# mratsim/laser

Hardware: NVIDIA H100
Metric: sgemm_tflops_m8192_n8192_k8192 (higher is better)
Workload: dtype f32

## Files before the change

### laser_b200/_build.py

```python
import concurrent.futures
import fcntl
import hashlib
import os
import shutil
import subprocess

_HERE = os.path.dirname(os.path.abspath(__file__))
CSRC = os.path.join(_HERE, "csrc")
LIB_DIR = os.path.join(_HERE, "lib")
OBJ_DIR = os.path.join(LIB_DIR, "obj")
LIB_PATH = os.path.join(LIB_DIR, "liblaser_b200.so")
SOURCES = ["capi.cu", "tc_f16x3.cu", "tc_tf32x3.cu", "tc_tf32x1.cu", "tc_bf16.cu"]
HEADERS = ["ptx.cuh", "f16_scale.cuh", "gemm_tc.cuh", "tc_params.h", "tc_launch.h", "tc_launch_impl.cuh", "gemm_simt.cuh", "gemm_dmma.cuh",
           "gemm_simt_kernel.inc", "split.cuh", "layers.cuh", "capi_layers.inc", "capi_multi.inc",
           "../../include/laser_b200.h"]

NVCC_FLAGS = [
    "-O3", "-std=c++17",
    "-gencode", "arch=compute_90a,code=sm_90a",
    "-lineinfo",
    "-Xcompiler", "-fPIC",
]
LINK_FLAGS = ["-shared", "-cudart", "static",
              "-gencode", "arch=compute_90a,code=sm_90a", "-Xcompiler", "-fPIC", "-ldl"]


def _nvcc():
    for cand in (shutil.which("nvcc"), "/usr/local/cuda/bin/nvcc"):
        if cand and os.path.exists(cand):
            return cand
    raise RuntimeError("nvcc not found: cannot build liblaser_b200.so")


def _sources():
    return [s for s in SOURCES if os.path.exists(os.path.join(CSRC, s))]


def _newest_header():
    return max((os.path.getmtime(os.path.join(CSRC, h)) for h in HEADERS if os.path.exists(os.path.join(CSRC, h))), default=0.0)


STAMP_PATH = LIB_PATH + ".srchash"


def _src_digest():
    h = hashlib.sha256(repr((NVCC_FLAGS, LINK_FLAGS)).encode())
    for name in _sources() + HEADERS:
        path = os.path.join(CSRC, name)
        if os.path.exists(path):
            h.update(name.encode() + b"\0")
            with open(path, "rb") as f:
                h.update(f.read())
    return h.hexdigest()


def _stamp():
    try:
        with open(STAMP_PATH) as f:
            return f.read().strip()
    except OSError:
        return None


def _write_stamp():
    tmp = "%s.tmp%d" % (STAMP_PATH, os.getpid())
    with open(tmp, "w") as f:
        f.write(_src_digest() + "\n")
    os.replace(tmp, STAMP_PATH)


def needs_build():
    if not os.path.exists(LIB_PATH):
        return True
    stamp = _stamp()
    if stamp is not None:
        return stamp != _src_digest()
    t = os.path.getmtime(LIB_PATH)
    return _newest_header() > t or any(os.path.getmtime(os.path.join(CSRC, s)) > t for s in _sources())


def build(force=False, verbose=False):
    if not force and not needs_build():
        if _stamp() is None:
            try:
                _write_stamp()
            except OSError:
                pass
        return LIB_PATH
    os.makedirs(OBJ_DIR, exist_ok=True)
    with open(os.path.join(LIB_DIR, ".build.lock"), "w") as lock:
        fcntl.flock(lock, fcntl.LOCK_EX)
        try:
            if not force and not needs_build():
                return LIB_PATH
            return _build_locked(force, verbose)
        finally:
            fcntl.flock(lock, fcntl.LOCK_UN)


def _build_locked(force, verbose):
    env = dict(os.environ)
    env.pop("CC", None)
    env.pop("CXX", None)
    nvcc = _nvcc()
    hdr_t = _newest_header()
    tag = ".tmp%d" % os.getpid()

    def compile_one(src):
        obj = os.path.join(OBJ_DIR, os.path.splitext(src)[0] + ".o")
        path = os.path.join(CSRC, src)
        if not force and os.path.exists(obj) and os.path.getmtime(obj) >= max(hdr_t, os.path.getmtime(path)):
            return obj
        cmd = [nvcc] + NVCC_FLAGS + (["-Xptxas", "-v"] if verbose else []) + ["-c", path, "-o", obj + tag]
        subprocess.check_call(cmd, env=env)
        os.replace(obj + tag, obj)
        return obj

    srcs = _sources()
    with concurrent.futures.ThreadPoolExecutor(max_workers=min(len(srcs), os.cpu_count() or 1)) as pool:
        objs = list(pool.map(compile_one, srcs))
    subprocess.check_call([nvcc] + LINK_FLAGS + ["-o", LIB_PATH + tag] + objs, env=env)
    os.replace(LIB_PATH + tag, LIB_PATH)
    _write_stamp()
    return LIB_PATH


if __name__ == "__main__":
    print(build(force=True, verbose=True))
```

### laser_b200/csrc/capi.cu

```cuda
#include "../../include/laser_b200.h"

#include <cuda.h>
#include <cuda_runtime.h>
#include <cudaTypedefs.h>

#include <atomic>
#include <cstdarg>
#include <cstdio>
#include <cstdlib>
#include <cstring>
#include <map>
#include <mutex>
#include <string>
#include <type_traits>
#include <utility>
#include <vector>

#include "gemm_simt.cuh"
#include "gemm_dmma.cuh"
#include "layers.cuh"
#include "split.cuh"
#include "tc_launch.h"

namespace {

using namespace lb200;

thread_local std::string g_last_error;
thread_local int g_last_path = 0;
std::atomic<int64_t> g_launches{0};
std::atomic<int64_t> g_dmma_launches{0};
std::atomic<int> g_f32_mode{-1};
constexpr int kDefaultF32Mode = LASER_B200_PATH_F16X3;
void multi_shutdown();

int set_error(int code, const char *fmt, ...) {
  char buf[512];
  va_list ap;
  va_start(ap, fmt);
  vsnprintf(buf, sizeof buf, fmt, ap);
  va_end(ap);
  g_last_error = buf;
  return code;
}

#define CUDA_TRY(expr)                                                                      \
  do {                                                                                      \
    cudaError_t _e = (expr);                                                                \
    if (_e != cudaSuccess) {                                                                \
      cudaGetLastError();                                                                   \
      return set_error(_e == cudaErrorMemoryAllocation ? LASER_B200_ENOMEM : LASER_B200_ECUDA, \
                       "%s failed: %s (%s:%d)", #expr, cudaGetErrorString(_e), __FILE__,   \
                       __LINE__);                                                           \
    }                                                                                       \
  } while (0)

struct Buffer {
  void *ptr = nullptr;
  size_t bytes = 0;
};

struct EventPair {
  cudaEvent_t a, b;
  int kind;
  int launches;
};

struct MapKey {
  const void *base;
  int64_t inner, outer, stride;
  int esz, box_inner, box_outer, swz;
  int64_t depth, depth_stride;
  bool operator==(const MapKey &o) const {
    return base == o.base && inner == o.inner && outer == o.outer && stride == o.stride && esz == o.esz &&
           box_inner == o.box_inner && box_outer == o.box_outer && swz == o.swz && depth == o.depth &&
           depth_stride == o.depth_stride;
  }
};
struct MapCacheEntry {
  MapKey key;
  CUtensorMap map;
  bool valid = false;
};
constexpr int kMapCacheSize = 64;

constexpr int kSchedSlots = 256;

struct Ctx {
  MapCacheEntry map_cache[kMapCacheSize];
  int map_cache_next = 0;
  int raster_g = 0;
  bool splitk_enabled = true;
  bool f64_dmma = true;
  bool ring_attr_set = false, dmma_attr_set = false;
  int64_t panel_rows = 1024;
  bool panel_taper = false;
  int kc_faithful = 128;
  bool dyn_sched = true;
  bool pdl = true;
  int64_t batch_ws_bytes = static_cast<int64_t>(1024) << 20;
  bool profiling = false;
  std::vector<EventPair> prof;
  int dev = -1;
  int sm_count = 0;
  cudaStream_t stream = nullptr;
  cudaStream_t up = nullptr, down = nullptr;
  std::vector<cudaEvent_t> panel_ev;
  PFN_cuTensorMapEncodeTiled_v12000 encode = nullptr;
  Buffer ws[4];
  Buffer gather[2];
  Buffer stage[3];
  Buffer splitk;
  Buffer bpanels;
  Buffer layer_ws;
  Buffer tfilt;
  Buffer f16s;
  Buffer sched;
  int sched_next = 0;
  cudaEvent_t ws_free = nullptr;
  std::mutex mu;
  std::mutex host_mu;
  std::mutex tfilt_mu;
  std::atomic<bool> ready{false};
};

constexpr int kMaxDevices = 32;
Ctx g_ctx[kMaxDevices];
std::mutex g_ctx_mu;

int parse_f32_mode(const char *mode) {
  if (!mode) return kDefaultF32Mode;
  if (!strcmp(mode, "f16x3")) return LASER_B200_PATH_F16X3;
  else if (!strcmp(mode, "tf32x3")) return LASER_B200_PATH_TF32X3;
  else if (!strcmp(mode, "tf32x1")) return LASER_B200_PATH_TF32X1;
  else if (!strcmp(mode, "simt")) return LASER_B200_PATH_SIMT;
  return kDefaultF32Mode;
}

int get_ctx(Ctx **out) {
  int dev = 0;
  cudaError_t e = cudaGetDevice(&dev);
  if (e != cudaSuccess) {
    cudaGetLastError();
    return set_error(LASER_B200_ENODEVICE, "no CUDA device: %s", cudaGetErrorString(e));
  }
  if (dev < 0 || dev >= kMaxDevices) return set_error(LASER_B200_ENODEVICE, "device index %d", dev);
  Ctx &c = g_ctx[dev];
  if (!c.ready) {
    std::lock_guard<std::mutex> lk(g_ctx_mu);
    if (!c.ready) {
      cudaDeviceProp prop;
      CUDA_TRY(cudaGetDeviceProperties(&prop, dev));
      if (prop.major != 9 || prop.minor != 0)
        return set_error(LASER_B200_ENODEVICE,
                         "device %d is sm_%d%d; this library is built for sm_90a only (no fallback)",
                         dev, prop.major, prop.minor);
      c.dev = dev;
      c.sm_count = prop.multiProcessorCount;
      CUDA_TRY(cudaStreamCreateWithFlags(&c.stream, cudaStreamNonBlocking));
      CUDA_TRY(cudaStreamCreateWithFlags(&c.up, cudaStreamNonBlocking));
      CUDA_TRY(cudaStreamCreateWithFlags(&c.down, cudaStreamNonBlocking));
      CUDA_TRY(cudaEventCreateWithFlags(&c.ws_free, cudaEventDisableTiming));
      void *fn = nullptr;
      cudaDriverEntryPointQueryResult qres;
      CUDA_TRY(cudaGetDriverEntryPoint("cuTensorMapEncodeTiled", &fn, cudaEnableDefault, &qres));
      if (!fn || qres != cudaDriverEntryPointSuccess)
        return set_error(LASER_B200_ECUDA, "cuTensorMapEncodeTiled not available from the driver");
      c.encode = reinterpret_cast<PFN_cuTensorMapEncodeTiled_v12000>(fn);
      CUDA_TRY(cudaMalloc(&c.sched.ptr, kSchedSlots * 2 * sizeof(unsigned int)));
      c.sched.bytes = kSchedSlots * 2 * sizeof(unsigned int);
      CUDA_TRY(cudaMemset(c.sched.ptr, 0, c.sched.bytes));
      if (const char *kc = getenv("LASER_B200_KC")) {
        const int v = atoi(kc);
        if (v >= 32) c.kc_faithful = v;
      }
      if (const char *rg = getenv("LASER_B200_RASTER")) c.raster_g = atoi(rg);
      if (const char *sk = getenv("LASER_B200_SPLITK")) c.splitk_enabled = atoi(sk) != 0;
      if (const char *dm = getenv("LASER_B200_F64_DMMA")) c.f64_dmma = atoi(dm) != 0;
      if (const char *pt = getenv("LASER_B200_PANEL_TAPER")) c.panel_taper = atoi(pt) != 0;
      if (const char *ds = getenv("LASER_B200_DYNSCHED")) c.dyn_sched = atoi(ds) != 0;
      if (const char *pd = getenv("LASER_B200_PDL")) c.pdl = atoi(pd) != 0;
      if (const char *bw = getenv("LASER_B200_BATCH_WS_MB")) {
        const int64_t v = atoll(bw);
        if (v >= 1) c.batch_ws_bytes = v << 20;
      }
      if (const char *pr = getenv("LASER_B200_PANEL_ROWS")) {
        const int64_t v = atoll(pr) / 256 * 256;
        if (v >= 256) c.panel_rows = v;
      }
      if (g_f32_mode.load() < 0) g_f32_mode.store(parse_f32_mode(getenv("LASER_B200_F32_MODE")));
      c.ready = true;
    }
  }
  *out = &c;
  return LASER_B200_OK;
}

int ensure(Buffer &b, size_t bytes) {
  if (b.bytes >= bytes) return LASER_B200_OK;
  if (b.ptr) CUDA_TRY(cudaFree(b.ptr));
  b.ptr = nullptr;
  b.bytes = 0;
  size_t want = bytes + (bytes >> 3);
  want = (want + 255) & ~static_cast<size_t>(255);
  CUDA_TRY(cudaMalloc(&b.ptr, want));
  b.bytes = want;
  return LASER_B200_OK;
}

struct ProfBracket {
  Ctx *c = nullptr;
  cudaStream_t s = nullptr;
  EventPair ep{};
  int64_t before = 0;

  int open(Ctx &ctx, cudaStream_t stream, int kind) {
    before = g_launches.load();
    if (!ctx.profiling) return LASER_B200_OK;
    c = &ctx;
    s = stream;
    ep.kind = kind;
    CUDA_TRY(cudaEventCreate(&ep.a));
    CUDA_TRY(cudaEventCreate(&ep.b));
    CUDA_TRY(cudaEventRecord(ep.a, s));
    return LASER_B200_OK;
  }
  int launches() const { return static_cast<int>(g_launches.load() - before); }
  int close() {
    if (!c) return LASER_B200_OK;
    ep.launches = launches();
    CUDA_TRY(cudaEventRecord(ep.b, s));
    c->prof.push_back(ep);
    c = nullptr;
    return LASER_B200_OK;
  }
  ~ProfBracket() {
    if (!c) return;
    if (ep.a) cudaEventDestroy(ep.a);
    if (ep.b) cudaEventDestroy(ep.b);
  }
};

inline int64_t round_up(int64_t x, int64_t m) { return (x + m - 1) / m * m; }
inline int grid_for(const Ctx &c, int64_t work_items, int per_sm) {
  int64_t g = static_cast<int64_t>(c.sm_count) * per_sm;
  if (work_items < g) g = work_items > 0 ? work_items : 1;
  return static_cast<int>(g);
}
#define COUNT_LAUNCH() g_launches.fetch_add(1, std::memory_order_relaxed)
#define CHECK_LAUNCH() CUDA_TRY(cudaGetLastError())

template <typename T, int TM, int TN, int BK>
int launch_simt(Ctx &c, int64_t M, int64_t N, int64_t K, T alpha, const T *A, int64_t rsA,
                int64_t csA, const T *B, int64_t rsB, int64_t csB, T beta, T *C, int64_t rsC,
                int64_t csC, cudaStream_t s, const Epilogue &epi, int64_t batch = 1, int64_t bsA = 0, int64_t bsB = 0,
                int64_t bsC = 0) {
  SimtParams<T> p;
  const int64_t tiles = simt_plan<T, TM, TN>(p, M, N, K, alpha, A, rsA, csA, B, rsB, csB, beta, C, rsC, csC);
  if constexpr (std::is_same<T, float>::value) { p.bias = epi.bias; p.bias_per_row = epi.bias_per_row; p.act = epi.act; }
  if (tiles > 0x7fffffff) return set_error(LASER_B200_EINVAL, "too many tiles");
  p.batch = batch; p.bsA = bsA; p.bsB = bsB; p.bsC = bsC;
  const int grid = grid_for(c, tiles * batch, 2);
  if (batch > 1) gemm_simt_batched_kernel<T, TM, TN, BK><<<grid, 256, 0, s>>>(p);
  else gemm_simt_kernel<T, TM, TN, BK><<<grid, 256, 0, s>>>(p);
  COUNT_LAUNCH();
  CHECK_LAUNCH();
  return LASER_B200_OK;
}

template <typename T>
int gemm_simt(Ctx &c, int64_t M, int64_t N, int64_t K, T alpha, const T *A, int64_t rsA,
              int64_t csA, const T *B, int64_t rsB, int64_t csB, T beta, T *C, int64_t rsC,
              int64_t csC, cudaStream_t s, const Epilogue &epi = Epilogue(), int64_t batch = 1, int64_t bsA = 0,
              int64_t bsB = 0, int64_t bsC = 0) {
#ifndef LB200_SIMT_BK
#define LB200_SIMT_BK 16
#endif
  if constexpr (std::is_same<T, double>::value) {
    const int64_t tiles128 = ((M + DMMA_BM - 1) / DMMA_BM) * ((N + DMMA_BN - 1) / DMMA_BN) * batch;
    if (c.f64_dmma && 2 * tiles128 >= c.sm_count) {
      SimtParams<double> p;
      const int64_t tiles = dmma_plan(p, M, N, K, alpha, A, rsA, csA, B, rsB, csB, beta, C, rsC, csC);
      if (tiles * batch > 0x7fffffff) return set_error(LASER_B200_EINVAL, "too many tiles");
      p.batch = batch; p.bsA = bsA; p.bsB = bsB; p.bsC = bsC;
      if (!c.dmma_attr_set) {
        CUDA_TRY(cudaFuncSetAttribute(gemm_dmma_kernel, cudaFuncAttributeMaxDynamicSharedMemorySize, static_cast<int>(DMMA_SMEM_BYTES)));
        c.dmma_attr_set = true;
      }
      gemm_dmma_kernel<<<grid_for(c, tiles * batch, 1), 256, DMMA_SMEM_BYTES, s>>>(p);
      g_dmma_launches.fetch_add(1);
      COUNT_LAUNCH();
      CHECK_LAUNCH();
      return LASER_B200_OK;
    }
  }
  if constexpr (std::is_same<T, float>::value) {
    if (M <= 32 && N >= 1024) {
      SimtParams<float> p;
      simt_plan<float, 8, 8>(p, M, N, K, alpha, A, rsA, csA, B, rsB, csB, beta, C, rsC, csC);
      p.bias = epi.bias; p.bias_per_row = epi.bias_per_row; p.act = epi.act;
      p.batch = batch; p.bsA = bsA; p.bsB = bsB; p.bsC = bsC;
      const bool async_ok = csB == 1 && rsB % 4 == 0 && (batch == 1 || bsB % 4 == 0) && (reinterpret_cast<uintptr_t>(B) & 15) == 0;
      if (async_ok) {
        const int grid = grid_for(c, ((N + 1023) / 1024) * batch, 1);
#define LB200_SKA(MT)                                                                                                  \
  do {                                                                                                                 \
    static std::atomic<uint32_t> attr_set{0};                                                                          \
    if (!(attr_set.load(std::memory_order_acquire) & (1u << c.dev))) {                                                 \
      CUDA_TRY(cudaFuncSetAttribute(gemm_skinny_m_async_kernel<MT>, cudaFuncAttributeMaxDynamicSharedMemorySize,       \
                                    static_cast<int>(ska_smem_bytes<MT>())));                                          \
      attr_set.fetch_or(1u << c.dev, std::memory_order_release);                                                       \
    }                                                                                                                  \
    gemm_skinny_m_async_kernel<MT><<<grid, 256, ska_smem_bytes<MT>(), s>>>(p);                                         \
  } while (0)
        if (M <= 8) LB200_SKA(8); else if (M <= 16) LB200_SKA(16); else if (M <= 24) LB200_SKA(24); else LB200_SKA(32);
#undef LB200_SKA
        COUNT_LAUNCH();
        CHECK_LAUNCH();
        return LASER_B200_OK;
      }
      const int nc = M <= 16 ? 4 : 2;
      const int grid = grid_for(c, ((N + 256 * nc - 1) / (256 * nc)) * batch, 2);
      if (M <= 8) gemm_skinny_m_kernel<8, 4><<<grid, 256, 0, s>>>(p);
      else if (M <= 16) gemm_skinny_m_kernel<16, 4><<<grid, 256, 0, s>>>(p);
      else if (M <= 24) gemm_skinny_m_kernel<24, 2><<<grid, 256, 0, s>>>(p);
      else gemm_skinny_m_kernel<32, 2><<<grid, 256, 0, s>>>(p);
      COUNT_LAUNCH();
      CHECK_LAUNCH();
      return LASER_B200_OK;
    }
  }
  if constexpr (sizeof(T) == 4)
    return launch_simt<T, 8, 8, LB200_SIMT_BK>(c, M, N, K, alpha, A, rsA, csA, B, rsB, csB, beta, C, rsC, csC, s, epi, batch,
                                               bsA, bsB, bsC);
  else
    return launch_simt<T, 4, 4, 16>(c, M, N, K, alpha, A, rsA, csA, B, rsB, csB, beta, C, rsC, csC, s, epi, batch, bsA, bsB,
                                    bsC);
}

struct Operand {
  const void *ptr;
  int64_t mn, k, s_mn, s_k;
  int64_t batch = 0, s_b = 0, aux_sb = 0;
  const ConvGeom *conv = nullptr;
  bool concat = false;
};
enum Major { K_MAJOR = 0, MN_MAJOR = 1, GENERAL = 2 };

Major classify(const Operand &o, int esz) {
  const bool aligned = (reinterpret_cast<uintptr_t>(o.ptr) & 15) == 0;
  if (!aligned) return GENERAL;
  const int64_t lim = (static_cast<int64_t>(1) << 40) / esz;
  if (o.s_k == 1 && o.s_mn > 0 && (o.s_mn * esz) % 16 == 0 && o.s_mn < lim) return K_MAJOR;
  if (o.s_mn == 1 && o.s_k > 0 && (o.s_k * esz) % 16 == 0 && o.s_k < lim) return MN_MAJOR;
  return GENERAL;
}

int encode_map(Ctx &c, CUtensorMap *map, int esz, const void *base, int64_t inner, int64_t outer,
               int64_t outer_stride_elems, int box_inner, int box_outer, CUtensorMapSwizzle swz, int64_t depth = 0,
               int64_t depth_stride = 0) {
  const MapKey key{base, inner, outer, outer_stride_elems, esz, box_inner, box_outer, static_cast<int>(swz), depth, depth_stride};
  for (int i = 0; i < kMapCacheSize; ++i)
    if (c.map_cache[i].valid && c.map_cache[i].key == key) {
      *map = c.map_cache[i].map;
      return LASER_B200_OK;
    }
  const cuuint64_t dims[3] = {static_cast<cuuint64_t>(inner), static_cast<cuuint64_t>(outer), static_cast<cuuint64_t>(depth)};
  const cuuint64_t strides[2] = {static_cast<cuuint64_t>(outer_stride_elems) * esz, static_cast<cuuint64_t>(depth_stride) * esz};
  const cuuint32_t box[3] = {static_cast<cuuint32_t>(box_inner), static_cast<cuuint32_t>(box_outer), 1};
  const cuuint32_t estr[3] = {1, 1, 1};
  const CUtensorMapDataType dt = esz == 4 ? CU_TENSOR_MAP_DATA_TYPE_FLOAT32 : CU_TENSOR_MAP_DATA_TYPE_BFLOAT16;
  CUresult r = c.encode(map, dt, depth > 0 ? 3 : 2, const_cast<void *>(base), dims, strides, box, estr,
                        CU_TENSOR_MAP_INTERLEAVE_NONE, swz,
                        CU_TENSOR_MAP_L2_PROMOTION_L2_256B, CU_TENSOR_MAP_FLOAT_OOB_FILL_NONE);
  if (r != CUDA_SUCCESS)
    return set_error(LASER_B200_ECUDA,
                     "cuTensorMapEncodeTiled failed (%d): base=%p inner=%lld outer=%lld stride=%lld box=%dx%d",
                     static_cast<int>(r), base, (long long)inner, (long long)outer,
                     (long long)outer_stride_elems, box_inner, box_outer);
  MapCacheEntry &e = c.map_cache[c.map_cache_next];
  c.map_cache_next = (c.map_cache_next + 1) % kMapCacheSize;
  e.key = key;
  e.map = *map;
  e.valid = true;
  return LASER_B200_OK;
}

int operand_map(Ctx &c, CUtensorMap *map, int esz, const void *base, Major major, int64_t mn,
                int64_t k, int64_t ld, int block_mn, int64_t depth = 0, int64_t depth_stride = 0) {
  const int block_k = TC_ROW_BYTES / esz;
  const int mn_atom = TC_ROW_BYTES / esz;
  if (major == K_MAJOR)
    return encode_map(c, map, esz, base, k, mn, ld, block_k, block_mn, CU_TENSOR_MAP_SWIZZLE_128B, depth, depth_stride);
  return encode_map(c, map, esz, base, mn, k, ld, mn_atom, block_k,
                    esz == 4 ? CU_TENSOR_MAP_SWIZZLE_128B_ATOM_32B : CU_TENSOR_MAP_SWIZZLE_128B, depth, depth_stride);
}

struct OperandMaps {
  CUtensorMap p0, p1;
  bool mn_major = false;
};
struct OperandWs {
  Buffer *p0, *p1, *gather;
  int64_t amax_off;
};
enum SplitMode {
  SPLIT_NONE = 0,
  SPLIT_TF32 = 1,
  SPLIT_F16X2 = 2,
};

inline OperandOp kernel_op(const OperandOp &op, bool rows_along_k) {
  OperandOp k = op;
  if (rows_along_k) { k.aux_sr = op.aux_sc; k.aux_sc = op.aux_sr; }
  return k;
}
inline bool op_same_layout(const Operand &o, const OperandOp &op) {
  return !op.aux || (op.aux_sr == o.s_mn && op.aux_sc == o.s_k && (reinterpret_cast<uintptr_t>(op.aux) & 15) == 0);
}

template <typename Launch>
int launch_prep(const OperandOp *op, const Batch &bt, Launch launch, bool concat = false) {
  auto with_op = [&](auto batched, auto cat) {
    if (op) launch(std::true_type(), *op, batched, cat);
    else launch(std::false_type(), OperandOp(), batched, cat);
  };
  if (concat) with_op(std::true_type(), std::true_type());
  else if (bt.n > 1) with_op(std::true_type(), std::false_type());
  else with_op(std::false_type(), std::false_type());
  COUNT_LAUNCH();
  CHECK_LAUNCH();
  return LASER_B200_OK;
}
inline Batch batch_of(const Operand &o) { return Batch{o.batch > 1 ? o.batch : 1, o.s_b, o.aux_sb}; }

template <typename T, int MODE = 0>
int gather(Ctx &c, const Operand &o, Buffer &dst, Buffer *lo, cudaStream_t s, const OperandOp *op = nullptr) {
  const Batch bt = batch_of(o);
  const int64_t ld = round_up(o.concat ? bt.n * o.k : o.k, 16 / static_cast<int64_t>(sizeof(T)));
  const size_t bytes = static_cast<size_t>((o.concat ? 1 : bt.n) * o.mn) * ld * sizeof(T);
  int rc;
  if ((rc = ensure(dst, bytes))) return rc;
  if (MODE == 1 && (rc = ensure(*lo, bytes))) return rc;
  const int64_t tiles = ((o.mn + 31) / 32) * ((o.k + 31) / 32) * bt.n;
  const int read_along_r = (llabs(o.s_mn) < llabs(o.s_k)) ? 1 : 0;
  T *d0 = static_cast<T *>(dst.ptr), *d1 = MODE == 1 ? static_cast<T *>(lo->ptr) : nullptr;
  return launch_prep(op, bt, [&](auto has_op, const OperandOp &k, auto batched, auto cat) {
    constexpr bool HAS_OP = decltype(has_op)::value && sizeof(T) == 4, BATCHED = decltype(batched)::value && sizeof(T) == 4,
                   CONCAT = decltype(cat)::value && sizeof(T) == 4;
    pack_general_kernel<T, MODE, HAS_OP, BATCHED, CONCAT><<<grid_for(c, tiles, 8), 256, 0, s>>>(
        static_cast<const T *>(o.ptr), o.mn, o.k, o.s_mn, o.s_k, d0, d1, ld, read_along_r, k, bt);
  }, o.concat);
}

int tf32_split(Ctx &c, const float *src, int64_t R, int64_t Cc, int64_t src_ld, float *hi, float *lo, int64_t ld, cudaStream_t s,
               const OperandOp *op, const Batch &bt = Batch(), bool concat = false) {
  const int64_t items = concat ? R * ((bt.n * Cc + 3) / 4) : bt.n * R * ((Cc + 3) / 4);
  return launch_prep(op, bt, [&](auto has_op, const OperandOp &k, auto batched, auto cat) {
    constexpr bool HAS_OP = decltype(has_op)::value, BATCHED = decltype(batched)::value, CONCAT = decltype(cat)::value;
    split_rows_tf32_kernel<HAS_OP, BATCHED, CONCAT><<<grid_for(c, (items + 255) / 256, 8), 256, 0, s>>>(src, R, Cc, src_ld, hi, lo,
                                                                                                       ld, k, bt);
  }, concat);
}

int f16x2_rows(Ctx &c, const float *src, int64_t R, int64_t Cc, int64_t src_ld, uint16_t *hb, uint16_t *lb, int64_t ld_b,
               uint32_t *words, cudaStream_t s, const OperandOp *op = nullptr, const Batch &bt = Batch(), bool concat = false) {
  const bool ring = !op && bt.n == 1 && f16x2_rows_ring_ok(src, Cc, src_ld);
  if (ring && !c.ring_attr_set) {
    CUDA_TRY(cudaFuncSetAttribute(f16x2_rows_ring_kernel, cudaFuncAttributeMaxDynamicSharedMemorySize,
                                  static_cast<int>(f16x2_rows_ring_smem(4 * 256 * F16ROWS_MAXV))));
    c.ring_attr_set = true;
  }
  const int64_t rows = concat ? R : bt.n * R, row_len = concat ? bt.n * Cc : Cc;
  return launch_prep(op, bt, [&](auto has_op, const OperandOp &k, auto batched, auto cat) {
    constexpr bool HAS_OP = decltype(has_op)::value, BATCHED = decltype(batched)::value, CONCAT = decltype(cat)::value;
    if (row_len <= 4 * 32 * F16ROWS_MAXV)
      f16x2_rows_fused_kernel<32, HAS_OP, BATCHED, CONCAT><<<grid_for(c, (rows + 7) / 8, 4), 256, 0, s>>>(src, R, Cc, src_ld, hb, lb,
                                                                                                     ld_b, words, k, bt);
    else if (ring)
      f16x2_rows_ring_kernel<<<grid_for(c, R, 2), 256, f16x2_rows_ring_smem(Cc), s>>>(src, R, Cc, src_ld, hb, lb, ld_b, words);
    else
      f16x2_rows_fused_kernel<256, HAS_OP, BATCHED, CONCAT><<<grid_for(c, rows, 4), 256, 0, s>>>(src, R, Cc, src_ld, hb, lb, ld_b,
                                                                                                words, k, bt);
  }, concat);
}

int f16x2_col_scales(Ctx &c, const float *src, int64_t R, int64_t Cc, int64_t src_ld, uint32_t *words, cudaStream_t s,
                     const OperandOp *op = nullptr, const Batch &bt = Batch(), bool concat = false) {
  CUDA_TRY(cudaMemsetAsync(words, 0, static_cast<size_t>((concat ? 1 : bt.n) * Cc) * sizeof(uint32_t), s));
  const int64_t items = ((Cc + 3) / 4) * ((R + ABSMAX_COL_ROWS - 1) / ABSMAX_COL_ROWS) * bt.n;
  return launch_prep(op, bt, [&](auto has_op, const OperandOp &k, auto batched, auto cat) {
    constexpr bool HAS_OP = decltype(has_op)::value, BATCHED = decltype(batched)::value, CONCAT = decltype(cat)::value;
    absmax_mn_kernel<true, HAS_OP, BATCHED, CONCAT><<<grid_for(c, (items + 255) / 256, 8), 256, 0, s>>>(src, R, Cc, src_ld, words, k,
                                                                                                       bt);
  }, concat);
}
int f16x2_col_split(Ctx &c, const float *src, int64_t R, int64_t Cc, int64_t src_ld, uint16_t *hb, uint16_t *lb, int64_t ld_b,
                    const uint32_t *words, cudaStream_t s, const OperandOp *op = nullptr, const Batch &bt = Batch(),
                    bool concat = false) {
  const int64_t items = ((Cc + 255) / 256) * ((R + SPLIT_ROWS - 1) / SPLIT_ROWS) * bt.n;
  return launch_prep(op, bt, [&](auto has_op, const OperandOp &k, auto batched, auto cat) {
    constexpr bool HAS_OP = decltype(has_op)::value, BATCHED = decltype(batched)::value, CONCAT = decltype(cat)::value;
    split_rows_f16x2_kernel<true, HAS_OP, BATCHED, CONCAT><<<grid_for(c, items, 8), 256, 0, s>>>(src, R, Cc, src_ld, hb, lb, ld_b,
                                                                                                words, k, bt);
  }, concat);
}

int im2col_rows(Ctx &c, const Operand &o, SplitMode mode, float *dst, float *dst_lo, uint16_t *hb, uint16_t *lb, int64_t ld,
                uint32_t *words, cudaStream_t s, const OperandOp *op = nullptr) {
  const Im2colSrc q = im2col_src(*o.conv);
  const Batch bt = batch_of(o);
  const int64_t images = o.conv->taps ? o.k / q.outHW : o.concat ? bt.n : bt.n * (o.mn / q.outHW), rows = bt.n * o.mn;
  const int64_t tiles = o.conv->taps ? ((o.mn + NHWC_TAPS - 1) / NHWC_TAPS) * ((ld + NHWC_PIX - 1) / NHWC_PIX)
                                     : o.mn * ((ld + TAP_SEG - 1) / TAP_SEG);
  const float *in = static_cast<const float *>(o.ptr);
  const bool dil = o.conv->dH != 1 || o.conv->dW != 1;
  if (o.concat && (dil || op)) return set_error(LASER_B200_ECUDA, "internal: a concatenated im2col source has no dilation or op");
  if (o.conv->nhwc && o.concat) return set_error(LASER_B200_ECUDA, "internal: a channels-last im2col source is not concatenated");
  if (o.conv->taps && (!o.conv->nhwc || dil || op))
    return set_error(LASER_B200_ECUDA, "internal: only a channels-last source without dilation or op has tap rows");
  auto launch = [&](auto m, auto absmax) {
    constexpr int MODE = decltype(m)::value, PER_SM = MODE == IM2COL_F16X2 ? 3 : 4;
    auto rows_kernel = [&](auto d, auto has_op, const auto &src) {
      constexpr bool DIL = decltype(d)::value, HAS_OP = decltype(has_op)::value;
      constexpr bool NHWC = std::is_base_of<Im2colNhwcSrc, typename std::decay<decltype(src)>::type>::value;
      if (ld <= 4 * 32 * F16ROWS_MAXV)
        im2col_rows_kernel<MODE, 32, DIL, HAS_OP, NHWC><<<grid_for(c, (rows + 7) / 8, PER_SM), 256, 0, s>>>(in, src, images, dst,
                                                                                                         dst_lo, hb, lb, ld, words);
      else
        im2col_rows_kernel<MODE, 256, DIL, HAS_OP, NHWC><<<grid_for(c, rows, PER_SM), 256, 0, s>>>(in, src, images, dst, dst_lo, hb,
                                                                                                lb, ld, words);
    };
    if (o.conv->taps) {
      im2col_nhwc_tap_rows_kernel<MODE, decltype(absmax)::value><<<grid_for(c, tiles, NHWC_PER_SM), 256, 0, s>>>(
          in, im2col_nhwc_src(*o.conv, in), images, dst, dst_lo, hb, lb, ld, words);
    } else if (o.conv->nhwc && (dil || op)) {
      Im2colNhwcGradSrc gq{};
      static_cast<Im2colNhwcSrc &>(gq) = im2col_nhwc_src(*o.conv, in);
      gq.vec = gq.vec && (!op || !op->aux || (reinterpret_cast<uintptr_t>(op->aux) & 15) == 0);
      gq.dH = static_cast<int>(o.conv->dH);
      gq.dW = static_cast<int>(o.conv->dW);
      if (op) gq.op = *op;
      if (dil && op) rows_kernel(std::true_type(), std::true_type(), gq);
      else if (dil) rows_kernel(std::true_type(), std::false_type(), gq);
      else rows_kernel(std::false_type(), std::true_type(), gq);
    } else if (o.conv->nhwc) {
      rows_kernel(std::false_type(), std::false_type(), im2col_nhwc_src(*o.conv, in));
    } else if (o.concat) {
      im2col_tap_rows_kernel<MODE, decltype(absmax)::value><<<grid_for(c, tiles, 8), 256, 0, s>>>(in, q, images, dst, dst_lo, hb, lb,
                                                                                                 ld, words);
    } else if (dil || op) {
      Im2colGradSrc gq{};
      static_cast<Im2colSrc &>(gq) = q;
      gq.dH = static_cast<int>(o.conv->dH);
      gq.dW = static_cast<int>(o.conv->dW);
      if (op) gq.op = *op;
      if (dil && op) rows_kernel(std::true_type(), std::true_type(), gq);
      else if (dil) rows_kernel(std::true_type(), std::false_type(), gq);
      else rows_kernel(std::false_type(), std::true_type(), gq);
    } else {
      rows_kernel(std::false_type(), std::false_type(), q);
    }
    COUNT_LAUNCH();
    CHECK_LAUNCH();
    return LASER_B200_OK;
  };
  if (mode == SPLIT_F16X2 && (o.concat || o.conv->taps)) {
    CUDA_TRY(cudaMemsetAsync(words, 0, static_cast<size_t>(o.mn) * sizeof(uint32_t), s));
    const int rc = launch(std::integral_constant<int, IM2COL_F16X2>(), std::true_type());
    if (rc) return rc;
  }
  if (mode == SPLIT_F16X2) return launch(std::integral_constant<int, IM2COL_F16X2>(), std::false_type());
  if (mode == SPLIT_TF32) return launch(std::integral_constant<int, IM2COL_TF32>(), std::false_type());
  return launch(std::integral_constant<int, IM2COL_F32>(), std::false_type());
}

int f32_rows(Ctx &c, const Operand &o, SplitMode mode, Buffer &dst, Buffer *lo, cudaStream_t s, const OperandOp *op) {
  if (!o.conv) return mode == SPLIT_TF32 ? gather<float, 1>(c, o, dst, lo, s, op) : gather<float>(c, o, dst, nullptr, s, op);
  const Batch bt = batch_of(o);
  const int64_t ld = round_up(o.concat ? bt.n * o.k : o.k, 4);
  const size_t bytes = static_cast<size_t>((o.concat ? 1 : bt.n) * o.mn) * ld * sizeof(float);
  int rc;
  if ((rc = ensure(dst, bytes))) return rc;
  if (mode == SPLIT_TF32 && (rc = ensure(*lo, bytes))) return rc;
  return im2col_rows(c, o, mode, static_cast<float *>(dst.ptr), mode == SPLIT_TF32 ? static_cast<float *>(lo->ptr) : nullptr,
                     nullptr, nullptr, ld, nullptr, s, op);
}

template <int ESZ>
int prepare_operand(Ctx &c, const Operand &o, SplitMode mode, const OperandWs &w, int block_mn,
                    OperandMaps *m, bool *used_ws, cudaStream_t s, const OperandOp *op = nullptr) {
  const bool conv = o.conv != nullptr;
  const Major mj = conv ? K_MAJOR : classify(o, ESZ);
  const Batch bt = batch_of(o);
  const bool cat = o.concat;
  const int64_t kk = cat ? bt.n * o.k : o.k;
  const bool rows_ok = bt.n == 1 || ((o.s_b * ESZ) % 16 == 0 && (!op || !op->aux || o.aux_sb % 4 == 0));
  const bool map_ok = bt.n == 1 || (o.s_b > 0 && o.s_b < (static_cast<int64_t>(1) << 40) / ESZ);
  const bool tma_layout = (mj == K_MAJOR || (mj == MN_MAJOR && (ESZ == 2 || mode == SPLIT_F16X2))) && rows_ok;
  const bool in_place = !conv && tma_layout && (mode == SPLIT_NONE ? !op && map_ok && !cat : !op || op_same_layout(o, *op));
  const Major out_mj = in_place ? mj : K_MAJOR;
  const int64_t R = (out_mj == K_MAJOR) ? o.mn : o.k;
  const int64_t Cc = (out_mj == K_MAJOR) ? o.k : o.mn;
  const int64_t src_ld = (mj == K_MAJOR) ? o.s_mn : o.s_k;
  const bool cat_rows = cat && out_mj == K_MAJOR;
  const int64_t rows_p = cat_rows ? R : bt.n * R, row_len = cat_rows ? bt.n * Cc : Cc;
  const int64_t ld = round_up(row_len, 16 / ESZ);
  const int64_t depth = o.batch > 0 && !cat ? bt.n : 0;
  auto d_stride = [&](int64_t pitch) { return bt.n > 1 ? (in_place && mode == SPLIT_NONE ? o.s_b : R * pitch) : R * pitch; };
  m->mn_major = (out_mj == MN_MAJOR);
  int rc;
  if (mode == SPLIT_NONE && in_place) {
    if ((rc = operand_map(c, &m->p0, ESZ, o.ptr, mj, o.mn, o.k, src_ld, block_mn, depth, d_stride(src_ld)))) return rc;
    m->p1 = m->p0;
    return LASER_B200_OK;
  }
  *used_ws = true;
  if constexpr (ESZ == 2) {
    if ((rc = gather<uint16_t>(c, o, *w.p0, nullptr, s))) return rc;
  } else {
    const float *src = static_cast<const float *>(o.ptr);
    const OperandOp kop = op ? kernel_op(*op, out_mj == MN_MAJOR) : OperandOp();
    const OperandOp *on_load = (in_place && op) ? &kop : nullptr;
    if (mode == SPLIT_F16X2) {
      const int64_t ld_b = round_up(row_len, 8);
      const size_t bytes_b = static_cast<size_t>(rows_p) * ld_b * 2;
      if ((rc = ensure(*w.p0, bytes_b))) return rc;
      if ((rc = ensure(*w.p1, bytes_b))) return rc;
      if (c.f16s.bytes < static_cast<size_t>(w.amax_off + (cat ? 1 : bt.n) * o.mn) * sizeof(uint32_t))
        return set_error(LASER_B200_ECUDA, "internal: F16X3 scale buffer not sized for this operand");
      uint16_t *hb = static_cast<uint16_t *>(w.p0->ptr), *lb = static_cast<uint16_t *>(w.p1->ptr);
      uint32_t *words = static_cast<uint32_t *>(c.f16s.ptr) + w.amax_off;
      if (conv) {
        rc = im2col_rows(c, o, mode, nullptr, nullptr, hb, lb, ld_b, words, s, op);
      } else if (!in_place) {
        if ((rc = gather<float>(c, o, *w.gather, nullptr, s, op))) return rc;
        rc = f16x2_rows(c, static_cast<const float *>(w.gather->ptr), rows_p, row_len, ld, hb, lb, ld_b, words, s);
      } else if (out_mj == K_MAJOR) {
        rc = f16x2_rows(c, src, R, Cc, src_ld, hb, lb, ld_b, words, s, on_load, bt, cat);
      } else {
        if ((rc = f16x2_col_scales(c, src, R, Cc, src_ld, words, s, on_load, bt, cat))) return rc;
        rc = f16x2_col_split(c, src, R, Cc, src_ld, hb, lb, ld_b, words, s, on_load, bt, cat);
      }
      if (rc) return rc;
      if ((rc = operand_map(c, &m->p0, 2, w.p0->ptr, out_mj, o.mn, kk, ld_b, block_mn, depth, d_stride(ld_b)))) return rc;
      return operand_map(c, &m->p1, 2, w.p1->ptr, out_mj, o.mn, kk, ld_b, block_mn, depth, d_stride(ld_b));
    }
    if (!in_place || conv) {
      rc = f32_rows(c, o, mode, *w.p0, w.p1, s, op);
    } else {
      const size_t bytes = static_cast<size_t>(rows_p) * ld * sizeof(float);
      if ((rc = ensure(*w.p0, bytes))) return rc;
      if ((rc = ensure(*w.p1, bytes))) return rc;
      rc = tf32_split(c, src, R, Cc, src_ld, static_cast<float *>(w.p0->ptr), static_cast<float *>(w.p1->ptr), ld, s, on_load, bt, cat);
    }
    if (rc) return rc;
  }
  if ((rc = operand_map(c, &m->p0, ESZ, w.p0->ptr, out_mj, o.mn, kk, ld, block_mn, depth, d_stride(ld)))) return rc;
  m->p1 = m->p0;
  if (mode == SPLIT_TF32) return operand_map(c, &m->p1, ESZ, w.p1->ptr, out_mj, o.mn, kk, ld, block_mn, depth, d_stride(ld));
  return LASER_B200_OK;
}

inline OperandWs ws_of_A(Ctx &c) { return OperandWs{&c.ws[0], &c.ws[1], &c.gather[0], 0}; }
inline OperandWs ws_of_B(Ctx &c, int64_t amax_off = 0) { return OperandWs{&c.ws[2], &c.ws[3], &c.gather[1], amax_off}; }
inline int f16_scales(Ctx &c, int64_t M, int64_t N, int64_t *b_off) {
  *b_off = round_up(M, 64);
  return ensure(c.f16s, static_cast<size_t>(*b_off + N) * sizeof(uint32_t));
}
struct F16Scales {
  const uint32_t *a = nullptr, *b = nullptr;
};

enum TcKind { TC_TF32X1, TC_TF32X3, TC_BF16, TC_F16X3 };
inline TcKind tc_kind_of_path(int path) {
  return path == LASER_B200_PATH_TF32X1 ? TC_TF32X1 : path == LASER_B200_PATH_TF32X3 ? TC_TF32X3 : TC_F16X3;
}
inline SplitMode split_mode(TcKind k) { return k == TC_TF32X3 ? SPLIT_TF32 : k == TC_F16X3 ? SPLIT_F16X2 : SPLIT_NONE; }

struct BatchArgs {
  int64_t batch, C, bias = 0;
};

template <typename OutT>
int tc_run(Ctx &c, TcKind kind, int64_t M, int64_t N, int64_t K, float alpha, const OperandMaps &ma,
           const OperandMaps &mb, float beta, OutT *C, int64_t rsC, int64_t csC, cudaStream_t s,
           const Epilogue &epi, const F16Scales *f16 = nullptr, bool after_prep = false, const BatchArgs *bat = nullptr,
           int64_t period_a = 1, int64_t period_b = 1) {
  TcLaunch l;
  l.a0 = ma.p0; l.a1 = ma.p1; l.b0 = mb.p0; l.b1 = mb.p1;
  l.a_mn = ma.mn_major; l.b_mn = mb.mn_major;
  l.pdl = c.pdl && after_prep;
  l.dev = c.dev; l.sm_count = c.sm_count; l.stream = s;
  TcParams &p = l.p;
  p.M = M; p.N = N; p.K = K; p.alpha = alpha; p.beta = beta;
  p.C = C; p.rsC = rsC; p.csC = csC; p.epi = epi;
  if (f16) { p.amax_a = f16->a; p.amax_b = f16->b; }
  if (bat) {
    l.batched = true;
    p.batch = static_cast<int>(bat->batch);
    p.period_a = static_cast<int>(period_a);
    p.period_b = static_cast<int>(period_b);
    p.bsC = bat->C;
    p.amax_bs_a = M;
    p.amax_bs_b = N;
    p.bias_bs = bat->bias;
  }
  const int npass = (kind == TC_TF32X3 || kind == TC_F16X3) ? 3 : 1;
  const TcPlanCfg cfg{c.kc_faithful, c.raster_g, c.splitk_enabled, c.sm_count};
  if (kind == TC_BF16 || kind == TC_F16X3) tc_plan<2, std::is_same<OutT, float>::value>(p, npass, cfg);
  else tc_plan<4, std::is_same<OutT, float>::value>(p, npass, cfg);
  if (c.dyn_sched) {
    p.sched = static_cast<unsigned int *>(c.sched.ptr) + 2 * c.sched_next;
    c.sched_next = (c.sched_next + 1) % kSchedSlots;
  }
  auto launch = [&](const TcLaunch &q) -> int {
    int e;
    switch (kind) {
      case TC_TF32X1: e = launch_tc_tf32x1(q); break;
      case TC_TF32X3: e = launch_tc_tf32x3(q); break;
      case TC_BF16: e = launch_tc_bf16(q); break;
      default: e = launch_tc_f16x3(q); break;
    }
    COUNT_LAUNCH();
    if (e != 0) {
      cudaGetLastError();
      return set_error(e == static_cast<int>(cudaErrorMemoryAllocation) ? LASER_B200_ENOMEM : LASER_B200_ECUDA,
                       "tensor-core kernel launch failed: %s", cudaGetErrorString(static_cast<cudaError_t>(e)));
    }
    CHECK_LAUNCH();
    return LASER_B200_OK;
  };
  ProfBracket prof;
  int rc = prof.open(c, s, 0);
  if (rc) return rc;
  if (p.k_splits > 1) {
    if constexpr (std::is_same<OutT, float>::value) {
      const int64_t ws_floats = tc_split_ws_floats(p);
      if ((rc = ensure(c.splitk, static_cast<size_t>(ws_floats) * sizeof(float)))) return rc;
      p.split_ws = static_cast<float *>(c.splitk.ptr);
      if ((rc = launch(l))) return rc;
      const int n_tail = p.num_m_blocks * p.num_n_blocks * p.batch - p.n_direct;
      const int64_t items = (static_cast<int64_t>(n_tail) * TC_BLOCK_M * (TC_BLOCK_N / 4) + 255) / 256;
      auto reduce = [&](auto batched) {
        splitk_tail_reduce_kernel<decltype(batched)::value><<<grid_for(c, items, 8), 256, 0, s>>>(
            static_cast<const float *>(c.splitk.ptr), p.k_splits, n_tail, p.n_direct, p.num_m_blocks, p.num_n_blocks, p.raster_g,
            M, N, alpha, beta, C, rsC, csC, p.epi.bias, p.epi.bias_per_row, p.epi.act, p.bsC, p.period_a, p.bias_bs);
      };
      if (bat) reduce(std::true_type());
      else reduce(std::false_type());
      COUNT_LAUNCH();
      CHECK_LAUNCH();
      CUDA_TRY(cudaEventRecord(c.ws_free, s));
      return prof.close();
    }
  }
  if ((rc = launch(l))) return rc;
  return prof.close();
}

inline bool batch_shares(int64_t stride, const OperandOp *op, int64_t aux_stride) {
  return stride == 0 && (!op || !op->aux || aux_stride == 0);
}

template <int SRC_ESZ, typename OutT>
int gemm_tc(Ctx &c, TcKind kind, const Operand &oa, const Operand &ob, float alpha, float beta, OutT *C, int64_t rsC, int64_t csC,
            cudaStream_t s, const Epilogue &epi, cudaEvent_t b_ready = nullptr, const OperandOp *opA = nullptr,
            const OperandOp *opB = nullptr, const BatchArgs *bat = nullptr) {
  const int64_t M = oa.mn, N = ob.mn, K = oa.k;
  const bool cat = oa.concat;
  const int64_t Kt = cat ? batch_of(oa).n * K : K;
  if (M > 0x7fffffffLL || N > 0x7fffffffLL || Kt > 0x7fffffffLL)
    return set_error(LASER_B200_EUNSUPPORTED, "tensor-core path: extents must fit in int32");
  std::lock_guard<std::mutex> lk(c.mu);
  const SplitMode mode = split_mode(kind);
  OperandMaps ma, mb;
  bool used_ws = false;
  CUDA_TRY(cudaStreamWaitEvent(s, c.ws_free, 0));
  ProfBracket prep;
  int rc = prep.open(c, s, 1);
  if (rc) return rc;
  int64_t f16_b_off = 0;
  if (mode == SPLIT_F16X2 &&
      (rc = f16_scales(c, (cat ? 1 : batch_of(oa).n) * M, (cat ? 1 : batch_of(ob).n) * N, &f16_b_off)))
    return rc;
  if ((rc = prepare_operand<SRC_ESZ>(c, oa, mode, ws_of_A(c), TC_BLOCK_M, &ma, &used_ws, s, opA))) return rc;
  if (b_ready) CUDA_TRY(cudaStreamWaitEvent(s, b_ready, 0));
  if ((rc = prepare_operand<SRC_ESZ>(c, ob, mode, ws_of_B(c, f16_b_off), TC_BLOCK_N, &mb, &used_ws, s, opB))) return rc;
  const int prep_launches = prep.launches();
  if ((rc = prep.close())) return rc;
  const F16Scales f16{static_cast<const uint32_t *>(c.f16s.ptr), static_cast<const uint32_t *>(c.f16s.ptr) + f16_b_off};
  rc = tc_run<OutT>(c, kind, M, N, Kt, alpha, ma, mb, beta, C, rsC, csC, s, epi, mode == SPLIT_F16X2 ? &f16 : nullptr,
                    prep_launches > 0 && !c.profiling, bat, batch_of(oa).n, batch_of(ob).n);
  if (rc) return rc;
  if (used_ws) CUDA_TRY(cudaEventRecord(c.ws_free, s));
  return LASER_B200_OK;
}

int finish(Ctx &c, cudaStream_t user, cudaStream_t s);

struct PackedLayout {
  int64_t ld_b;
  size_t off_h, off_l, off_amax, bytes;
};
inline PackedLayout packed_layout(int64_t mn, int64_t k) {
  PackedLayout L;
  L.ld_b = round_up(k, 8);
  auto al = [](size_t x) { return (x + 255) & ~static_cast<size_t>(255); };
  L.off_h = 0;
  L.off_l = al(static_cast<size_t>(mn) * L.ld_b * 2);
  L.off_amax = L.off_l + al(static_cast<size_t>(mn) * L.ld_b * 2);
  L.bytes = L.off_amax + al(static_cast<size_t>(mn) * sizeof(uint32_t));
  return L;
}

int prepack_dev(int which, void *dst, int64_t mn, int64_t k, const float *src, int64_t s_mn, int64_t s_k,
                void *stream) {
  if (mn < 0 || k < 0) return set_error(LASER_B200_EINVAL, "negative extent");
  if (mn == 0 || k == 0) return LASER_B200_OK;
  if (!dst || !src) return set_error(LASER_B200_EINVAL, "null pointer");
  if (reinterpret_cast<uintptr_t>(dst) & 255) return set_error(LASER_B200_EINVAL, "packed buffer must be 256-byte aligned");
  Ctx *c;
  int rc = get_ctx(&c);
  if (rc) return rc;
  cudaStream_t s = stream ? static_cast<cudaStream_t>(stream) : c->stream;
  const PackedLayout L = packed_layout(mn, k);
  uint8_t *base = static_cast<uint8_t *>(dst);
  uint16_t *h = reinterpret_cast<uint16_t *>(base + L.off_h), *l = reinterpret_cast<uint16_t *>(base + L.off_l);
  uint32_t *amax = reinterpret_cast<uint32_t *>(base + L.off_amax);
  {
    std::lock_guard<std::mutex> lk(c->mu);
    Operand o{src, mn, k, s_mn, s_k};
    const float *rows = src;
    int64_t rows_ld = s_mn;
    if (classify(o, 4) != K_MAJOR) {
      CUDA_TRY(cudaStreamWaitEvent(s, c->ws_free, 0));
      Buffer &g = c->gather[which];
      if ((rc = gather<float>(*c, o, g, nullptr, s))) return rc;
      rows = static_cast<const float *>(g.ptr);
      rows_ld = round_up(k, 4);
    }
    if ((rc = f16x2_rows(*c, rows, mn, k, rows_ld, h, l, L.ld_b, amax, s))) return rc;
    CUDA_TRY(cudaEventRecord(c->ws_free, s));
  }
  return finish(*c, static_cast<cudaStream_t>(stream), s);
}

int packed_maps(Ctx &c, const void *packed, int64_t mn, int64_t k, int block_mn, OperandMaps *m, const uint32_t **amax) {
  const PackedLayout L = packed_layout(mn, k);
  const uint8_t *base = static_cast<const uint8_t *>(packed);
  int rc;
  m->mn_major = false;
  *amax = reinterpret_cast<const uint32_t *>(base + L.off_amax);
  if ((rc = operand_map(c, &m->p0, 2, base + L.off_h, K_MAJOR, mn, k, L.ld_b, block_mn))) return rc;
  return operand_map(c, &m->p1, 2, base + L.off_l, K_MAJOR, mn, k, L.ld_b, block_mn);
}

int gemm_packed_dev(int64_t M, int64_t N, int64_t K, float alpha, const float *A, int64_t rsA,
                    int64_t csA, const void *packedA, const void *packedB, float beta, float *C,
                    int64_t rsC, int64_t csC, void *stream) {
  if (M < 0 || N < 0 || K < 0) return set_error(LASER_B200_EINVAL, "negative extent");
  if (M == 0 || N == 0 || K == 0) return LASER_B200_OK;
  if ((!A && !packedA) || !packedB || !C) return set_error(LASER_B200_EINVAL, "null pointer");
  if (M > 0x7fffffffLL || N > 0x7fffffffLL || K > 0x7fffffffLL)
    return set_error(LASER_B200_EUNSUPPORTED, "extents must fit in int32");
  Ctx *cp;
  int rc = get_ctx(&cp);
  if (rc) return rc;
  Ctx &c = *cp;
  cudaStream_t s = stream ? static_cast<cudaStream_t>(stream) : c.stream;
  {
    std::lock_guard<std::mutex> lk(c.mu);
    OperandMaps ma, mb;
    F16Scales f16;
    bool used_ws = false;
    int prep_launches = 0;
    CUDA_TRY(cudaStreamWaitEvent(s, c.ws_free, 0));
    if (packedA) {
      if ((rc = packed_maps(c, packedA, M, K, TC_BLOCK_M, &ma, &f16.a))) return rc;
    } else {
      Operand oa{A, M, K, rsA, csA};
      int64_t b_off = 0;
      if ((rc = f16_scales(c, M, 0, &b_off))) return rc;
      ProfBracket prep;
      if ((rc = prep.open(c, s, 1))) return rc;
      if ((rc = prepare_operand<4>(c, oa, SPLIT_F16X2, ws_of_A(c), TC_BLOCK_M, &ma, &used_ws, s))) return rc;
      prep_launches = prep.launches();
      if ((rc = prep.close())) return rc;
      f16.a = static_cast<const uint32_t *>(c.f16s.ptr);
    }
    if ((rc = packed_maps(c, packedB, N, K, TC_BLOCK_N, &mb, &f16.b))) return rc;
    if ((rc = tc_run<float>(c, TC_F16X3, M, N, K, alpha, ma, mb, beta, C, rsC, csC, s, Epilogue(), &f16,
                            prep_launches > 0 && !c.profiling)))
      return rc;
    if (used_ws) CUDA_TRY(cudaEventRecord(c.ws_free, s));
  }
  g_last_path = LASER_B200_PATH_F16X3;
  return finish(c, static_cast<cudaStream_t>(stream), s);
}

int check_args(int64_t M, int64_t N, int64_t K, const void *A, const void *B, const void *C) {
  if (M < 0 || N < 0 || K < 0) return set_error(LASER_B200_EINVAL, "negative extent M=%lld N=%lld K=%lld",
                                                (long long)M, (long long)N, (long long)K);
  if (M == 0 || N == 0 || K == 0) return -1;
  if (!A || !B || !C) return set_error(LASER_B200_EINVAL, "null matrix pointer");
  return LASER_B200_OK;
}

int finish(Ctx &, cudaStream_t user, cudaStream_t s) {
  if (!user) CUDA_TRY(cudaStreamSynchronize(s));
  return LASER_B200_OK;
}

inline bool is_tc_mode(int mode) {
  return mode == LASER_B200_PATH_F16X3 || mode == LASER_B200_PATH_TF32X3 || mode == LASER_B200_PATH_TF32X1;
}
int resolve_auto(int64_t M, int64_t N, int64_t K, const Epilogue &epi, bool operand_op = false) {
  const double work = static_cast<double>(M) * N * K;
  if (work <= 128.0 * 128.0 * 128.0) return LASER_B200_PATH_SIMT;
  const int mode = g_f32_mode.load();
  if (mode == LASER_B200_PATH_SIMT) return LASER_B200_PATH_SIMT;
  if (N <= 4 && M >= 1024 && !epi.bias && !epi.act && !operand_op) return -1;
  if (M <= 32 && N >= 1024) return LASER_B200_PATH_SIMT;
  return mode < 0 ? kDefaultF32Mode : mode;
}

int check_f32_path(int path) {
  if (path == LASER_B200_PATH_AUTO || path == LASER_B200_PATH_SIMT || is_tc_mode(path)) return LASER_B200_OK;
  return set_error(LASER_B200_EINVAL, "unknown path %d for float32", path);
}

int simt_run(Ctx &c, const Operand &oa, const Operand &ob, float alpha, float beta, float *C, int64_t rsC, int64_t csC,
             cudaStream_t s, const Epilogue &epi, const OperandOp *opA, const OperandOp *opB, int64_t batch, int64_t bsC) {
  struct Rows {
    const float *p;
    int64_t s_mn, s_k, s_b;
  };
  const bool copy_a = opA || oa.concat || oa.conv, copy_b = opB || ob.concat || ob.conv;
  std::unique_lock<std::mutex> lk(c.mu, std::defer_lock);
  if (copy_a || copy_b) {
    lk.lock();
    CUDA_TRY(cudaStreamWaitEvent(s, c.ws_free, 0));
  }
  auto rows = [&](const Operand &o, const OperandOp *op, bool copy, Buffer &g, Rows *r) {
    *r = Rows{static_cast<const float *>(o.ptr), o.s_mn, o.s_k, o.s_b};
    if (!copy) return LASER_B200_OK;
    const int rc = f32_rows(c, o, SPLIT_NONE, g, nullptr, s, op);
    const int64_t ld = round_up(o.concat ? batch_of(o).n * o.k : o.k, 4);
    *r = Rows{static_cast<const float *>(g.ptr), ld, 1, !o.concat && !batch_shares(o.s_b, op, o.aux_sb) ? o.mn * ld : 0};
    return rc;
  };
  Rows a, b;
  int rc;
  if ((rc = rows(oa, opA, copy_a, c.gather[0], &a))) return rc;
  if ((rc = rows(ob, opB, copy_b, c.gather[1], &b))) return rc;
  const int64_t K = oa.concat ? batch_of(oa).n * oa.k : oa.k;
  if ((rc = gemm_simt<float>(c, oa.mn, ob.mn, K, alpha, a.p, a.s_mn, a.s_k, b.p, b.s_k, b.s_mn, beta, C, rsC, csC, s, epi, batch,
                             a.s_b, b.s_b, bsC)))
    return rc;
  if (copy_a || copy_b) CUDA_TRY(cudaEventRecord(c.ws_free, s));
  return LASER_B200_OK;
}

int run_f32(Ctx &c, int path, int64_t M, int64_t N, int64_t K, float alpha, const float *A, int64_t rsA, int64_t csA, const float *B,
            int64_t rsB, int64_t csB, float beta, float *C, int64_t rsC, int64_t csC, cudaStream_t s, const Epilogue &epi,
            const OperandOp *opA, const OperandOp *opB, int64_t batch = 0, const laser_b200_batch_strides *bs = nullptr,
            bool concat = false, const ConvGeom *convB = nullptr, cudaEvent_t b_ready = nullptr, const ConvGeom *convA = nullptr,
            int64_t periodA = 0) {
  Operand oa{A, M, K, rsA, csA}, ob{B, N, K, csB, rsB};
  if (batch > 0) {
    oa.batch = periodA > 0 ? periodA : !concat && batch_shares(bs->A, opA, bs->auxA) ? 1 : batch; oa.s_b = bs->A; oa.aux_sb = bs->auxA; oa.concat = concat;
    ob.batch = !concat && batch_shares(bs->B, opB, bs->auxB) ? 1 : batch; ob.s_b = bs->B; ob.aux_sb = bs->auxB; ob.concat = concat;
  }
  oa.conv = convA;
  ob.conv = convB;
  const bool batched = batch > 0 && !concat;
  if (periodA > 0 && (!batched || opA || path == LASER_B200_PATH_SIMT))
    return set_error(LASER_B200_ECUDA, "internal: a periodic A is a batched tensor-core operand without op");
  if (path == LASER_B200_PATH_SIMT)
    return simt_run(c, oa, ob, alpha, beta, C, rsC, csC, s, epi, opA, opB, batched ? batch : 1, batched ? bs->C : 0);
  const BatchArgs bat{batch, batched ? bs->C : 0, periodA > 0 ? M : 0};
  return gemm_tc<4, float>(c, tc_kind_of_path(path), oa, ob, alpha, beta, C, rsC, csC, s, epi, b_ready, opA, opB,
                           batched ? &bat : nullptr);
}

int f32_dev(int64_t M, int64_t N, int64_t K, float alpha, const float *A, int64_t rsA, int64_t csA,
            const float *B, int64_t rsB, int64_t csB, float beta, float *C, int64_t rsC, int64_t csC,
            int path, void *stream, const Epilogue &epi = Epilogue(), cudaEvent_t b_ready = nullptr,
            const OperandOp *opA = nullptr, const OperandOp *opB = nullptr) {
  int rc = check_args(M, N, K, A, B, C);
  if (rc == -1) return LASER_B200_OK;
  if (rc) return rc;
  const bool has_op = opA || opB;
  if ((has_op || path != -1) && (rc = check_f32_path(path))) return rc;
  Ctx *c;
  rc = get_ctx(&c);
  if (rc) return rc;
  cudaStream_t s = stream ? static_cast<cudaStream_t>(stream) : c->stream;
  if (path == LASER_B200_PATH_AUTO) path = resolve_auto(M, N, K, epi, has_op);
  if (b_ready && !is_tc_mode(path)) CUDA_TRY(cudaStreamWaitEvent(s, b_ready, 0));
  switch (path) {
    case -1: {
      const int grid = grid_for(*c, (M + 7) / 8, 8);
      const bool vec = (csA == 1) && (rsA % 4 == 0) && (K % 4 == 0) && ((reinterpret_cast<uintptr_t>(A) & 15) == 0);
      const size_t bsmem = static_cast<size_t>(N) * K * sizeof(float);
      const bool use_smem = vec && bsmem <= 96 * 1024;
#define LB200_GEMV(NV)                                                                                         \
  do {                                                                                                         \
    if (use_smem) {                                                                                            \
      static std::atomic<uint32_t> attr_set{0};                                                                \
      if (!(attr_set.load(std::memory_order_acquire) & (1u << c->dev))) {                                      \
        CUDA_TRY(cudaFuncSetAttribute(gemv_warp_smem_kernel<NV>, cudaFuncAttributeMaxDynamicSharedMemorySize, 96 * 1024)); \
        attr_set.fetch_or(1u << c->dev, std::memory_order_release);                                            \
      }                                                                                                        \
      gemv_warp_smem_kernel<NV><<<grid_for(*c, (M + 7) / 8, 2), 256, bsmem, s>>>(M, K, alpha, A, rsA, B, rsB, csB, beta, C, rsC, csC); \
    } else if (vec) gemv_warp_kernel<NV, true><<<grid, 256, 0, s>>>(M, K, alpha, A, rsA, csA, B, rsB, csB, beta, C, rsC, csC);  \
    else gemv_warp_kernel<NV, false><<<grid, 256, 0, s>>>(M, K, alpha, A, rsA, csA, B, rsB, csB, beta, C, rsC, csC);     \
  } while (0)
      if (N == 1) LB200_GEMV(1); else if (N == 2) LB200_GEMV(2); else if (N == 3) LB200_GEMV(3); else LB200_GEMV(4);
#undef LB200_GEMV
      COUNT_LAUNCH();
      CHECK_LAUNCH();
      g_last_path = LASER_B200_PATH_SIMT;
      break;
    }
    default:
      rc = run_f32(*c, path, M, N, K, alpha, A, rsA, csA, B, rsB, csB, beta, C, rsC, csC, s, epi, opA, opB, 0, nullptr, false,
                   nullptr, b_ready);
      if (rc) return rc;
      g_last_path = path;
      break;
  }
  return finish(*c, static_cast<cudaStream_t>(stream), s);
}

template <typename T>
int simt_dev(int64_t M, int64_t N, int64_t K, T alpha, const T *A, int64_t rsA, int64_t csA,
             const T *B, int64_t rsB, int64_t csB, T beta, T *C, int64_t rsC, int64_t csC,
             void *stream) {
  int rc = check_args(M, N, K, A, B, C);
  if (rc == -1) return LASER_B200_OK;
  if (rc) return rc;
  Ctx *c;
  rc = get_ctx(&c);
  if (rc) return rc;
  cudaStream_t s = stream ? static_cast<cudaStream_t>(stream) : c->stream;
  rc = gemm_simt<T>(*c, M, N, K, alpha, A, rsA, csA, B, rsB, csB, beta, C, rsC, csC, s);
  if (rc) return rc;
  g_last_path = LASER_B200_PATH_SIMT;
  return finish(*c, static_cast<cudaStream_t>(stream), s);
}

int bf16_dev(int64_t M, int64_t N, int64_t K, float alpha, const uint16_t *A, int64_t rsA,
             int64_t csA, const uint16_t *B, int64_t rsB, int64_t csB, float beta, uint16_t *C,
             int64_t rsC, int64_t csC, void *stream) {
  int rc = check_args(M, N, K, A, B, C);
  if (rc == -1) return LASER_B200_OK;
  if (rc) return rc;
  Ctx *c;
  rc = get_ctx(&c);
  if (rc) return rc;
  cudaStream_t s = stream ? static_cast<cudaStream_t>(stream) : c->stream;
  rc = gemm_tc<2, uint16_t>(*c, TC_BF16, Operand{A, M, K, rsA, csA}, Operand{B, N, K, csB, rsB}, alpha, beta, C, rsC, csC, s,
                            Epilogue());
  if (rc) return rc;
  g_last_path = LASER_B200_PATH_BF16;
  return finish(*c, static_cast<cudaStream_t>(stream), s);
}

int epilogue_of(const laser_b200_epilogue *epi, Epilogue *e) {
  if (!epi) return LASER_B200_OK;
  if (epi->activation < 0 || epi->activation > 3) return set_error(LASER_B200_EINVAL, "unknown activation %d", epi->activation);
  e->bias = epi->bias;
  e->bias_per_row = epi->bias_per_row ? 1 : 0;
  e->act = epi->activation;
  return LASER_B200_OK;
}
int operand_op_of(const laser_b200_operand_op *in, bool is_b, OperandOp *op, const OperandOp **out) {
  *out = nullptr;
  if (!in || in->op == LASER_B200_OP_NONE) return LASER_B200_OK;
  if (in->op < LASER_B200_OP_NONE || in->op > LASER_B200_OP_SIGMOID_GRAD)
// ... 886 lines not shown
```

### laser_b200/csrc/f16_scale.cuh

```cuda
#pragma once

#include <stdint.h>
#ifdef LB200_HOST_EMULATION
#include <cmath>
#include <limits>
#endif

namespace lb200 {

__device__ __forceinline__ int f16x2_scale_exp(uint32_t absmax_bits) {
  const int e = static_cast<int>(absmax_bits >> 23);
  if (e == 0) return 0;
  int s = 14 - (e - 127);
  if (s > 126) s = 126;
  if (s < -126) s = -126;
  return s;
}
__device__ __forceinline__ float f16x2_pow2(int s) { return __uint_as_float(static_cast<uint32_t>(127 + s) << 23); }
__device__ __forceinline__ float f16x2_scale(uint32_t absmax_bits) { return f16x2_pow2(f16x2_scale_exp(absmax_bits)); }
__device__ __forceinline__ float f16x2_unscale(uint32_t absmax_bits) { return f16x2_pow2(-f16x2_scale_exp(absmax_bits)); }

#ifndef LB200_HOST_EMULATION
__device__ __forceinline__ uint16_t f16_rn_bits(float x) {
  uint16_t h;
  asm("cvt.rn.f16.f32 %0, %1;" : "=h"(h) : "f"(x));
  return h;
}
__device__ __forceinline__ float f16_bits_to_f32(uint16_t h) {
  float f;
  asm("cvt.f32.f16 %0, %1;" : "=f"(f) : "h"(h));
  return f;
}
#else
inline uint16_t f16_rn_bits(float x) {
  const uint32_t u = __float_as_uint(x);
  const uint16_t sign = static_cast<uint16_t>((u >> 16) & 0x8000u);
  const uint32_t a = u & 0x7fffffffu;
  if (a > 0x7f800000u) return static_cast<uint16_t>(sign | 0x7e00u);
  if (a == 0x7f800000u) return static_cast<uint16_t>(sign | 0x7c00u);
  const double ax = static_cast<double>(__uint_as_float(a));
  if (ax == 0.0) return sign;
  int e;
  std::frexp(ax, &e);
  int E = e - 1;
  if (E < -14) E = -14;
  const double q = std::ldexp(1.0, E - 10);
  const double r = std::nearbyint(ax / q) * q;
  if (r >= 65520.0) return static_cast<uint16_t>(sign | 0x7c00u);
  if (r < std::ldexp(1.0, -14)) return static_cast<uint16_t>(sign | static_cast<uint16_t>(r / std::ldexp(1.0, -24)));
  int e2;
  const double m = std::frexp(r, &e2);
  const uint32_t mant = static_cast<uint32_t>(m * 2048.0) - 1024u;
  return static_cast<uint16_t>(sign | (static_cast<uint32_t>(e2 - 1 + 15) << 10) | mant);
}
inline float f16_bits_to_f32(uint16_t h) {
  const int e = (h >> 10) & 31;
  const int m = h & 1023;
  double v;
  if (e == 0) v = std::ldexp(static_cast<double>(m), -24);
  else if (e == 31) v = m ? std::numeric_limits<double>::quiet_NaN() : std::numeric_limits<double>::infinity();
  else v = std::ldexp(static_cast<double>(1024 + m), e - 25);
  return static_cast<float>((h & 0x8000) ? -v : v);
}
#endif

__device__ __forceinline__ float f16_bits_to_f32_alu(uint32_t v) {
  const uint32_t u = v & 0x7fffu;
  const float normal = __uint_as_float((u << 13) + 0x38000000u);
  const float subnormal = __uint_as_float(0x38800000u + (u << 13)) - __uint_as_float(0x38800000u);
  const float mag = (u < 0x0400u) ? subnormal : normal;
  return (v & 0x8000u) ? -mag : mag;
}
__device__ __forceinline__ void f16x2_pieces2(float x0, float x1, uint32_t &h2, uint32_t &l2) {
#ifndef LB200_HOST_EMULATION
  asm("cvt.rn.f16x2.f32 %0, %1, %2;" : "=r"(h2) : "f"(x1), "f"(x0));
  const uint32_t v0 = h2 & 0xffffu, v1 = h2 >> 16;
  float d0 = __fsub_rn(x0, f16_bits_to_f32_alu(v0)), d1 = __fsub_rn(x1, f16_bits_to_f32_alu(v1));
  if ((v0 & 0x7c00u) == 0x7c00u) d0 = 0.0f;
  if ((v1 & 0x7c00u) == 0x7c00u) d1 = 0.0f;
  asm("cvt.rn.f16x2.f32 %0, %1, %2;" : "=r"(l2) : "f"(d1), "f"(d0));
#else
  const uint16_t a0 = f16_rn_bits(x0), a1 = f16_rn_bits(x1);
  const uint16_t b0 = ((a0 & 0x7c00u) == 0x7c00u) ? static_cast<uint16_t>(0) : f16_rn_bits(__fsub_rn(x0, f16_bits_to_f32_alu(a0)));
  const uint16_t b1 = ((a1 & 0x7c00u) == 0x7c00u) ? static_cast<uint16_t>(0) : f16_rn_bits(__fsub_rn(x1, f16_bits_to_f32_alu(a1)));
  h2 = a0 | (static_cast<uint32_t>(a1) << 16);
  l2 = b0 | (static_cast<uint32_t>(b1) << 16);
#endif
}

}
```

### laser_b200/csrc/gemm_tc.cuh

```cuda
#pragma once

#include <type_traits>

#include "f16_scale.cuh"
#include "ptx.cuh"
#include "tc_params.h"

namespace lb200 {

#ifndef LB200_HOST_EMULATION
static __device__ __noinline__ float epi_act(float v, int act) {
#else
inline float epi_act(float v, int act) {
#endif
  if (act == 1) return fmaxf(v, 0.0f);
  if (act == 2) return tanhf(v);
  if (act == 3) return 1.0f / (1.0f + expf(-v));
  return v;
}

__device__ __forceinline__ float bf16_bits_to_f32(uint16_t h) {
  return __uint_as_float(static_cast<uint32_t>(h) << 16);
}
__device__ __forceinline__ uint16_t f32_to_bf16_bits(float f) {
  uint32_t u = __float_as_uint(f);
  if ((u & 0x7fffffffu) > 0x7f800000u) return static_cast<uint16_t>((u >> 16) | 0x40);
  u += 0x7fffu + ((u >> 16) & 1u);
  return static_cast<uint16_t>(u >> 16);
}

template <int ESZ, uint32_t FMT16, int NPASS, bool A_MN, bool B_MN, typename OutT, bool SCALED, bool BATCHED>
__global__ void __launch_bounds__(TC_THREADS, 1)
gemm_tc_kernel(const __grid_constant__ CUtensorMap mapA0, const __grid_constant__ CUtensorMap mapA1,
               const __grid_constant__ CUtensorMap mapB0, const __grid_constant__ CUtensorMap mapB1,
               const TcParams p) {
  static_assert(NPASS == 1 || NPASS == 3, "one pass, or the three passes of a two-piece product");
  static_assert(ESZ == 2 || (!A_MN && !B_MN), "wgmma reads tf32 operands K-major only (capi.cu transposes MN-major fp32)");
  using Cfg = TcCfg<NPASS>;
  constexpr int STAGES = Cfg::STAGES;
  constexpr int BLOCK_K = TC_ROW_BYTES / ESZ;
  const int sched_id = static_cast<int>(blockIdx.x);
  const int sched_stride = static_cast<int>(gridDim.x);

  LB200_DYN_SMEM(uint8_t, smem_raw);
  uint8_t *smem = reinterpret_cast<uint8_t *>((reinterpret_cast<uintptr_t>(smem_raw) + 1023) &
                                              ~static_cast<uintptr_t>(1023));
  uint64_t *bars = reinterpret_cast<uint64_t *>(smem + STAGES * Cfg::STAGE_BYTES);
  uint64_t *full_bar = bars;
  uint64_t *empty_bar = bars + STAGES;
  uint64_t *sched_full = bars + 2 * STAGES;
  uint64_t *sched_empty = sched_full + 1;
  int *sched_unit = reinterpret_cast<int *>(sched_empty + 1);

  const int warp_idx = threadIdx.x >> 5;
  const int lane = threadIdx.x & 31;
  const int tiles_pp = p.num_m_blocks * p.num_n_blocks;
  const int num_tiles = BATCHED ? tiles_pp * p.batch : tiles_pp;
  const int num_kb = static_cast<int>((p.K + BLOCK_K - 1) / BLOCK_K);
  const int num_units = p.n_direct + (num_tiles - p.n_direct) * p.k_splits;
  auto decode_unit = [&](int u, int &t, int &sp, int &kb_lo, int &kb_hi) {
    if (u < p.n_direct) {
      t = u; sp = -1; kb_lo = 0; kb_hi = num_kb;
    } else {
      const int v = u - p.n_direct;
      const int i = v / p.k_splits;
      t = p.n_direct + i;
      sp = v - i * p.k_splits;
      kb_lo = min(num_kb, sp * p.kb_per_split);
      kb_hi = min(num_kb, kb_lo + p.kb_per_split);
    }
  };
  constexpr int SCHED_CONSUMERS = 1 + TC_EPI_WARPS;
  auto next_unit = [&](uint32_t &ph) -> int {
    ptx::mbar_wait(sched_full, ph);
    const int u = *reinterpret_cast<volatile int *>(sched_unit);
    ptx::mbar_arrive(sched_empty);
    ph ^= 1u;
    return u;
  };

  if (threadIdx.x == 0) {
    ptx::prefetch_tensormap(&mapA0);
    ptx::prefetch_tensormap(&mapB0);
    if constexpr (NPASS == 3) {
      ptx::prefetch_tensormap(&mapA1);
      ptx::prefetch_tensormap(&mapB1);
    }
  }
  if (threadIdx.x == 32) {
    for (int i = 0; i < STAGES; ++i) {
      ptx::mbar_init(&full_bar[i], 1);
      ptx::mbar_init(&empty_bar[i], TC_EPI_WARPS);
    }
    ptx::mbar_init(sched_full, 1);
    ptx::mbar_init(sched_empty, SCHED_CONSUMERS);
    ptx::fence_barrier_init();
  }
  __syncthreads();
  ptx::griddep_wait();

  if (warp_idx < 4) {
    ptx::setmaxnreg_dec<TC_REGS_CTRL>();
    if (warp_idx == 3 && lane == 0) {
      uint32_t phase = 0;
      int next_static = sched_id;
      for (;;) {
        ptx::mbar_wait(sched_empty, phase ^ 1);
        int u;
        if (p.sched) {
          u = static_cast<int>(atomicAdd(p.sched, 1u));
        } else {
          u = next_static;
          next_static += sched_stride;
        }
        if (u >= num_units) u = -1;
        *reinterpret_cast<volatile int *>(sched_unit) = u;
        ptx::mbar_arrive(sched_full);
        phase ^= 1u;
        if (u < 0) {
          if (p.sched) {
            __threadfence();
            if (atomicAdd(p.sched + 1, 1u) == static_cast<unsigned int>(sched_stride - 1)) {
              p.sched[0] = 0u;
              p.sched[1] = 0u;
              __threadfence();
            }
          }
          break;
        }
      }
    } else if (warp_idx == 0 && lane == 0) {
      int stage = 0;
      uint32_t phase = 0, sched_phase = 0;
      constexpr int MN_ATOM = TC_ROW_BYTES / ESZ;
      constexpr int MN_BOX_BYTES = BLOCK_K * TC_ROW_BYTES;
      auto load_a = [&](uint8_t *dst, const CUtensorMap *m, uint64_t *bar, int m0, int k0, int z) {
        if constexpr (!A_MN) {
          if constexpr (BATCHED) ptx::tma_load_3d(dst, m, bar, k0, m0, z);
          else ptx::tma_load_2d(dst, m, bar, k0, m0);
        } else {
#pragma unroll
          for (int c = 0; c < TC_BLOCK_M / MN_ATOM; ++c) {
            if constexpr (BATCHED) ptx::tma_load_3d(dst + c * MN_BOX_BYTES, m, bar, m0 + c * MN_ATOM, k0, z);
            else ptx::tma_load_2d(dst + c * MN_BOX_BYTES, m, bar, m0 + c * MN_ATOM, k0);
          }
        }
      };
      auto load_b = [&](uint8_t *dst, const CUtensorMap *m, uint64_t *bar, int n0, int k0, int z) {
        if constexpr (!B_MN) {
          if constexpr (BATCHED) ptx::tma_load_3d(dst, m, bar, k0, n0, z);
          else ptx::tma_load_2d(dst, m, bar, k0, n0);
        } else {
#pragma unroll
          for (int c = 0; c < TC_BLOCK_N / MN_ATOM; ++c) {
            if constexpr (BATCHED) ptx::tma_load_3d(dst + c * MN_BOX_BYTES, m, bar, n0 + c * MN_ATOM, k0, z);
            else ptx::tma_load_2d(dst + c * MN_BOX_BYTES, m, bar, n0 + c * MN_ATOM, k0);
          }
        }
      };
      for (;;) {
        const int u = next_unit(sched_phase);
        if (u < 0) break;
        int t, sp, mb, nb, kb_lo, kb_hi;
        decode_unit(u, t, sp, kb_lo, kb_hi);
        int za = 0, zb = 0;
        if constexpr (BATCHED) {
          const int bz = t / tiles_pp;
          t -= bz * tiles_pp;
          za = bz % p.period_a;
          zb = bz % p.period_b;
        }
        tile_coords(t, p.num_m_blocks, p.num_n_blocks, p.raster_g, mb, nb);
        const int m0 = mb * TC_BLOCK_M;
        const int n0 = nb * TC_BLOCK_N;
        for (int kb = kb_lo; kb < kb_hi; ++kb) {
          ptx::mbar_wait(&empty_bar[stage], phase ^ 1);
          ptx::mbar_arrive_expect_tx(&full_bar[stage], Cfg::STAGE_BYTES);
          uint8_t *sa = smem + stage * Cfg::STAGE_BYTES;
          uint8_t *sb = sa + Cfg::A_STAGE_BYTES;
          const int k0 = kb * BLOCK_K;
          load_a(sa, &mapA0, &full_bar[stage], m0, k0, za);
          if constexpr (NPASS == 3) load_a(sa + TC_A_TILE_BYTES, &mapA1, &full_bar[stage], m0, k0, za);
          load_b(sb, &mapB0, &full_bar[stage], n0, k0, zb);
          if constexpr (NPASS == 3) load_b(sb + Cfg::B_TILE_BYTES, &mapB1, &full_bar[stage], n0, k0, zb);
          if (++stage == STAGES) { stage = 0; phase ^= 1; }
        }
      }
    }
  } else {
    ptx::setmaxnreg_inc<TC_REGS_EPI>();
    const int g = (warp_idx - 4) >> 2;
    const int wq = warp_idx & 3;
    const int lr = lane >> 2;
    const int lc = 2 * (lane & 3);
    constexpr int MMA_K = 32 / ESZ;
    constexpr int K_STEPS = BLOCK_K / MMA_K;
    constexpr int MN_BOX_BYTES = BLOCK_K * TC_ROW_BYTES;
    constexpr uint32_t A_WG_BYTES = 64 * TC_ROW_BYTES;
    int stage = 0;
    uint32_t phase = 0, sched_phase = 0;
    const bool vec_ok_c = (p.csC == 1) && ((p.rsC & 1) == 0) && ((reinterpret_cast<uintptr_t>(p.C) & (2 * sizeof(OutT) - 1)) == 0) &&
                          (!BATCHED || (p.bsC & 1) == 0);
    float acc[TC_ACC_REGS];
#pragma unroll
    for (int j = 0; j < TC_ACC_REGS; ++j) acc[j] = 0.0f;
    for (;;) {
      int u = 0;
      if (lane == 0) u = next_unit(sched_phase);
      u = __shfl_sync(0xffffffffu, u, 0);
      if (u < 0) break;
      int t, sp, mb, nb, kb_lo, kb_hi;
      decode_unit(u, t, sp, kb_lo, kb_hi);
      int bz = 0, za = 0, zb = 0;
      if constexpr (BATCHED) {
        bz = t / tiles_pp;
        za = bz % p.period_a;
        zb = bz % p.period_b;
        int tl = t - bz * tiles_pp;
        tile_coords(tl, p.num_m_blocks, p.num_n_blocks, p.raster_g, mb, nb);
      } else {
        tile_coords(t, p.num_m_blocks, p.num_n_blocks, p.raster_g, mb, nb);
      }
      const int num_blocks = (kb_hi - kb_lo + p.kb_per_block - 1) / p.kb_per_block;
      const int r_tile = 64 * g + 16 * wq + lr;
      const int64_t row0 = static_cast<int64_t>(mb) * TC_BLOCK_M + r_tile;
      const int64_t col0 = static_cast<int64_t>(nb) * TC_BLOCK_N + lc;
      const bool split_unit = sp >= 0;
      uint32_t amax_row[2] = {0u, 0u}, amax_col[2 * TC_BLOCK_N / 8];
      if constexpr (SCALED) {
#pragma unroll
        for (int h = 0; h < 2; ++h)
          if (row0 + 8 * h < p.M) amax_row[h] = p.amax_a[(BATCHED ? za * p.amax_bs_a : 0) + row0 + 8 * h];
#pragma unroll
        for (int j = 0; j < 2 * TC_BLOCK_N / 8; ++j) {
          const int64_t c = col0 + 8 * (j >> 1) + (j & 1);
          amax_col[j] = c < p.N ? p.amax_b[(BATCHED ? zb * p.amax_bs_b : 0) + c] : 0u;
        }
      }
      float run[TC_ACC_REGS];
#pragma unroll
      for (int j = 0; j < TC_ACC_REGS; ++j) run[j] = 0.0f;
      for (int blk = 0; blk < num_blocks; ++blk) {
        const int kb0 = kb_lo + blk * p.kb_per_block;
        const int kb1 = min(kb_hi, kb0 + p.kb_per_block);
        int prev_stage = -1;
        for (int kb = kb0; kb < kb1; ++kb) {
          ptx::mbar_wait(&full_bar[stage], phase);
          ptx::wgmma_fence();
          const uint32_t a_addr = ptx::smem_u32(smem + stage * Cfg::STAGE_BYTES) + g * A_WG_BYTES;
          const uint32_t b_addr = ptx::smem_u32(smem + stage * Cfg::STAGE_BYTES + Cfg::A_STAGE_BYTES);
#pragma unroll
          for (int pass = 0; pass < NPASS; ++pass) {
            const uint32_t a_tile = a_addr + ((NPASS == 3 && pass == 1) ? TC_A_TILE_BYTES : 0);
            const uint32_t b_tile = b_addr + ((NPASS == 3 && pass == 0) ? Cfg::B_TILE_BYTES : 0);
#pragma unroll
            for (int k = 0; k < K_STEPS; ++k) {
              const uint64_t ad = A_MN ? ptx::make_smem_desc(a_tile + k * MMA_K * TC_ROW_BYTES, MN_BOX_BYTES, 1024, ptx::kLayoutSw128)
                                       : ptx::make_smem_desc(a_tile + k * 32, 0, 1024, ptx::kLayoutSw128);
              const uint64_t bd = B_MN ? ptx::make_smem_desc(b_tile + k * MMA_K * TC_ROW_BYTES, MN_BOX_BYTES, 1024, ptx::kLayoutSw128)
                                       : ptx::make_smem_desc(b_tile + k * 32, 0, 1024, ptx::kLayoutSw128);
              const uint32_t accum = (kb == kb0 && pass == 0 && k == 0) ? 0u : 1u;
              if constexpr (ESZ == 4) ptx::wgmma_m64n128k8_tf32(acc, ad, bd, accum);
              else if constexpr (FMT16 == ptx::kFmtF16) ptx::wgmma_m64n128k16_f16<A_MN ? 1 : 0, B_MN ? 1 : 0>(acc, ad, bd, accum);
              else ptx::wgmma_m64n128k16_bf16<A_MN ? 1 : 0, B_MN ? 1 : 0>(acc, ad, bd, accum);
            }
          }
          ptx::wgmma_commit();
          ptx::wgmma_wait<1>();
          if (prev_stage >= 0 && lane == 0) ptx::mbar_arrive(&empty_bar[prev_stage]);
          prev_stage = stage;
          if (++stage == STAGES) { stage = 0; phase ^= 1; }
        }
        ptx::wgmma_wait<0>();
        ptx::wgmma_hold(acc);
        if (prev_stage >= 0 && lane == 0) ptx::mbar_arrive(&empty_bar[prev_stage]);
#pragma unroll
        for (int j = 0; j < TC_ACC_REGS; ++j) run[j] = __fadd_rn(run[j], acc[j]);
      }
      float alpha_r[2] = {split_unit ? 1.0f : p.alpha, split_unit ? 1.0f : p.alpha};
      if constexpr (SCALED) {
#pragma unroll
        for (int h = 0; h < 2; ++h) alpha_r[h] *= f16x2_unscale(amax_row[h]);
      }
      const float beta_u = split_unit ? 0.0f : p.beta;
      const bool has_epi = !split_unit && ((p.epi.bias != nullptr) || (p.epi.act != 0));
      float *ws_base = nullptr;
      if (split_unit) {
        const int64_t plane = static_cast<int64_t>(sp) * (num_tiles - p.n_direct) + (t - p.n_direct);
        ws_base = p.split_ws + (plane * TC_BLOCK_M + r_tile) * TC_BLOCK_N + lc;
      }
#pragma unroll
      for (int h = 0; h < 2; ++h) {
        const int64_t row = row0 + 8 * h;
        if (!split_unit && row >= p.M) continue;
        const float row_bias =
            (has_epi && p.epi.bias && p.epi.bias_per_row) ? p.epi.bias[(BATCHED ? za * p.bias_bs : 0) + row] : 0.0f;
        OutT *crow = split_unit ? nullptr : reinterpret_cast<OutT *>(p.C) + (BATCHED ? bz * p.bsC : 0) + row * p.rsC;
#pragma unroll
        for (int i = 0; i < TC_BLOCK_N / 8; ++i) {
          float v[2];
#pragma unroll
          for (int e = 0; e < 2; ++e) {
            v[e] = alpha_r[h] * run[4 * i + 2 * h + e];
            if constexpr (SCALED) v[e] *= f16x2_unscale(amax_col[2 * i + e]);
          }
          if (split_unit) {
            *reinterpret_cast<float2 *>(ws_base + 8 * h * TC_BLOCK_N + 8 * i) = make_float2(v[0], v[1]);
            continue;
          }
          const int64_t c = col0 + 8 * i;
          if (c >= p.N) continue;
          const bool pair_ok = vec_ok_c && c + 1 < p.N;
          OutT *dst = crow + c * p.csC;
          if (beta_u != 0.0f) {
            float o[2] = {0.0f, 0.0f};
            if constexpr (sizeof(OutT) == 4) {
              if (pair_ok) { const float2 w = *reinterpret_cast<const float2 *>(dst); o[0] = w.x; o[1] = w.y; }
              else { o[0] = dst[0]; if (c + 1 < p.N) o[1] = dst[p.csC]; }
            } else {
              o[0] = bf16_bits_to_f32(dst[0]);
              if (c + 1 < p.N) o[1] = bf16_bits_to_f32(dst[pair_ok ? 1 : p.csC]);
            }
#pragma unroll
            for (int e = 0; e < 2; ++e) v[e] = fmaf(beta_u, o[e], v[e]);
          }
          if (has_epi) {
#pragma unroll
            for (int e = 0; e < 2; ++e) {
              const float bv = (p.epi.bias && !p.epi.bias_per_row) ? (c + e < p.N ? p.epi.bias[c + e] : 0.0f) : row_bias;
              v[e] = epi_act(v[e] + bv, p.epi.act);
            }
          }
          if constexpr (sizeof(OutT) == 4) {
            if (pair_ok) *reinterpret_cast<float2 *>(dst) = make_float2(v[0], v[1]);
            else { dst[0] = v[0]; if (c + 1 < p.N) dst[p.csC] = v[1]; }
          } else {
            if (pair_ok) *reinterpret_cast<uint32_t *>(dst) = f32_to_bf16_bits(v[0]) | (static_cast<uint32_t>(f32_to_bf16_bits(v[1])) << 16);
            else { dst[0] = f32_to_bf16_bits(v[0]); if (c + 1 < p.N) dst[p.csC] = f32_to_bf16_bits(v[1]); }
          }
        }
      }
    }
  }

  __syncthreads();
}

}
```

### laser_b200/csrc/ptx.cuh

```cuda
#pragma once

#include <cuda.h>
#include <cuda_runtime.h>
#include <stdint.h>

#ifdef LB200_HOST_EMULATION
#include "ptx_emu.h"
#else

#define LB200_DYN_SMEM(T, name) extern __shared__ T name[]

namespace lb200 {
namespace ptx {

__device__ __forceinline__ uint32_t smem_u32(const void *p) {
  return static_cast<uint32_t>(__cvta_generic_to_shared(p));
}

__device__ __forceinline__ bool elect_one() {
  uint32_t pred = 0;
  asm volatile(
      "{\n\t"
      ".reg .pred P;\n\t"
      "elect.sync _|P, 0xffffffff;\n\t"
      "selp.u32 %0, 1, 0, P;\n\t"
      "}\n"
      : "=r"(pred));
  return pred != 0;
}

__device__ __forceinline__ void mbar_init(uint64_t *bar, uint32_t count) {
  asm volatile("mbarrier.init.shared::cta.b64 [%0], %1;" ::"r"(smem_u32(bar)), "r"(count));
}
__device__ __forceinline__ void fence_barrier_init() {
  asm volatile("fence.mbarrier_init.release.cluster;" ::: "memory");
}
__device__ __forceinline__ void fence_proxy_async_smem() {
  asm volatile("fence.proxy.async.shared::cta;" ::: "memory");
}
__device__ __forceinline__ void mbar_arrive_expect_tx(uint64_t *bar, uint32_t bytes) {
  asm volatile("mbarrier.arrive.expect_tx.shared::cta.b64 _, [%0], %1;" ::"r"(smem_u32(bar)),
               "r"(bytes)
               : "memory");
}
__device__ __forceinline__ void mbar_arrive(uint64_t *bar) {
  asm volatile("mbarrier.arrive.shared::cta.b64 _, [%0];" ::"r"(smem_u32(bar)) : "memory");
}
__device__ __forceinline__ bool mbar_try_wait(uint64_t *bar, uint32_t parity) {
  uint32_t ok;
  asm volatile(
      "{\n\t"
      ".reg .pred P;\n\t"
      "mbarrier.try_wait.parity.shared::cta.b64 P, [%1], %2;\n\t"
      "selp.u32 %0, 1, 0, P;\n\t"
      "}\n"
      : "=r"(ok)
      : "r"(smem_u32(bar)), "r"(parity)
      : "memory");
  return ok != 0;
}
__device__ __forceinline__ void mbar_wait(uint64_t *bar, uint32_t parity) {
  while (!mbar_try_wait(bar, parity)) {
  }
}

__device__ __forceinline__ void prefetch_tensormap(const CUtensorMap *m) {
  asm volatile("prefetch.tensormap [%0];" ::"l"(reinterpret_cast<uint64_t>(m)) : "memory");
}
__device__ __forceinline__ void tma_load_2d(void *smem_dst, const CUtensorMap *map, uint64_t *bar,
                                            int32_t c0, int32_t c1) {
  asm volatile(
      "cp.async.bulk.tensor.2d.shared::cluster.global.mbarrier::complete_tx::bytes"
      " [%0], [%1, {%3, %4}], [%2];"
      ::"r"(smem_u32(smem_dst)), "l"(reinterpret_cast<uint64_t>(map)), "r"(smem_u32(bar)),
        "r"(c0), "r"(c1)
      : "memory");
}
__device__ __forceinline__ void tma_load_3d(void *smem_dst, const CUtensorMap *map, uint64_t *bar,
                                            int32_t c0, int32_t c1, int32_t c2) {
  asm volatile(
      "cp.async.bulk.tensor.3d.shared::cluster.global.mbarrier::complete_tx::bytes"
      " [%0], [%1, {%3, %4, %5}], [%2];"
      ::"r"(smem_u32(smem_dst)), "l"(reinterpret_cast<uint64_t>(map)), "r"(smem_u32(bar)),
        "r"(c0), "r"(c1), "r"(c2)
      : "memory");
}
__device__ __forceinline__ void cp_async_8(void *smem_dst, const void *gsrc, bool valid) {
  asm volatile("cp.async.ca.shared.global [%0], [%1], 8, %2;"
               ::"r"(smem_u32(smem_dst)), "l"(reinterpret_cast<uint64_t>(gsrc)), "r"(valid ? 8u : 0u) : "memory");
}
__device__ __forceinline__ void cp_async_16(void *smem_dst, const void *gsrc, uint32_t src_bytes) {
  asm volatile("cp.async.cg.shared.global [%0], [%1], 16, %2;"
               ::"r"(smem_u32(smem_dst)), "l"(reinterpret_cast<uint64_t>(gsrc)), "r"(src_bytes) : "memory");
}
__device__ __forceinline__ void cp_async_commit() { asm volatile("cp.async.commit_group;" ::: "memory"); }
template <int N>
__device__ __forceinline__ void cp_async_wait() { asm volatile("cp.async.wait_group %0;" ::"n"(N) : "memory"); }
__device__ __forceinline__ void bulk_load_1d(void *smem_dst, const void *gsrc, uint32_t bytes, uint64_t *bar) {
  asm volatile("cp.async.bulk.shared::cluster.global.mbarrier::complete_tx::bytes [%0], [%1], %2, [%3];"
               ::"r"(smem_u32(smem_dst)), "l"(reinterpret_cast<uint64_t>(gsrc)), "r"(bytes), "r"(smem_u32(bar))
               : "memory");
}
__device__ __forceinline__ void prefetch_l2(const void *p) {
  asm volatile("prefetch.global.L2 [%0];" ::"l"(p));
}
template <int N>
__device__ __forceinline__ void setmaxnreg_inc() {
  asm volatile("setmaxnreg.inc.sync.aligned.u32 %0;" ::"n"(N));
}
template <int N>
__device__ __forceinline__ void setmaxnreg_dec() {
  asm volatile("setmaxnreg.dec.sync.aligned.u32 %0;" ::"n"(N));
}

__device__ __forceinline__ void wgmma_fence() { asm volatile("wgmma.fence.sync.aligned;" ::: "memory"); }
__device__ __forceinline__ void wgmma_commit() { asm volatile("wgmma.commit_group.sync.aligned;" ::: "memory"); }
template <int N>
__device__ __forceinline__ void wgmma_wait() { asm volatile("wgmma.wait_group.sync.aligned %0;" ::"n"(N) : "memory"); }
__device__ __forceinline__ void wgmma_hold(float (&d)[64]) {
#pragma unroll
  for (int i = 0; i < 64; ++i) asm volatile("" : "+f"(d[i])::"memory");
}
template <int TA, int TB>
__device__ __forceinline__ void wgmma_m64n128k16_f16(float (&d)[64], uint64_t a_desc, uint64_t b_desc, uint32_t scale_d) {
  asm volatile(
      "{\n\t"
      ".reg .pred p;\n\t"
      "setp.ne.b32 p, %66, 0;\n\t"
      "wgmma.mma_async.sync.aligned.m64n128k16.f32.f16.f16 "
      "{%0, %1, %2, %3, %4, %5, %6, %7, %8, %9, %10, %11, %12, %13, %14, %15, %16, %17, %18, %19, %20, %21, %22, %23, %24, %25, %26, %27, %28, %29, %30, %31, %32, %33, %34, %35, %36, %37, %38, %39, %40, %41, %42, %43, %44, %45, %46, %47, %48, %49, %50, %51, %52, %53, %54, %55, %56, %57, %58, %59, %60, %61, %62, %63}, "
      "%64, %65, p, 1, 1, %67, %68;\n\t"
      "}\n"
      : "+f"(d[0]), "+f"(d[1]), "+f"(d[2]), "+f"(d[3]), "+f"(d[4]), "+f"(d[5]), "+f"(d[6]), "+f"(d[7]),
        "+f"(d[8]), "+f"(d[9]), "+f"(d[10]), "+f"(d[11]), "+f"(d[12]), "+f"(d[13]), "+f"(d[14]), "+f"(d[15]),
        "+f"(d[16]), "+f"(d[17]), "+f"(d[18]), "+f"(d[19]), "+f"(d[20]), "+f"(d[21]), "+f"(d[22]), "+f"(d[23]),
        "+f"(d[24]), "+f"(d[25]), "+f"(d[26]), "+f"(d[27]), "+f"(d[28]), "+f"(d[29]), "+f"(d[30]), "+f"(d[31]),
        "+f"(d[32]), "+f"(d[33]), "+f"(d[34]), "+f"(d[35]), "+f"(d[36]), "+f"(d[37]), "+f"(d[38]), "+f"(d[39]),
        "+f"(d[40]), "+f"(d[41]), "+f"(d[42]), "+f"(d[43]), "+f"(d[44]), "+f"(d[45]), "+f"(d[46]), "+f"(d[47]),
        "+f"(d[48]), "+f"(d[49]), "+f"(d[50]), "+f"(d[51]), "+f"(d[52]), "+f"(d[53]), "+f"(d[54]), "+f"(d[55]),
        "+f"(d[56]), "+f"(d[57]), "+f"(d[58]), "+f"(d[59]), "+f"(d[60]), "+f"(d[61]), "+f"(d[62]), "+f"(d[63])
      : "l"(a_desc), "l"(b_desc), "r"(scale_d), "n"(TA), "n"(TB));
}
template <int TA, int TB>
__device__ __forceinline__ void wgmma_m64n128k16_bf16(float (&d)[64], uint64_t a_desc, uint64_t b_desc, uint32_t scale_d) {
  asm volatile(
      "{\n\t"
      ".reg .pred p;\n\t"
      "setp.ne.b32 p, %66, 0;\n\t"
      "wgmma.mma_async.sync.aligned.m64n128k16.f32.bf16.bf16 "
      "{%0, %1, %2, %3, %4, %5, %6, %7, %8, %9, %10, %11, %12, %13, %14, %15, %16, %17, %18, %19, %20, %21, %22, %23, %24, %25, %26, %27, %28, %29, %30, %31, %32, %33, %34, %35, %36, %37, %38, %39, %40, %41, %42, %43, %44, %45, %46, %47, %48, %49, %50, %51, %52, %53, %54, %55, %56, %57, %58, %59, %60, %61, %62, %63}, "
      "%64, %65, p, 1, 1, %67, %68;\n\t"
      "}\n"
      : "+f"(d[0]), "+f"(d[1]), "+f"(d[2]), "+f"(d[3]), "+f"(d[4]), "+f"(d[5]), "+f"(d[6]), "+f"(d[7]),
        "+f"(d[8]), "+f"(d[9]), "+f"(d[10]), "+f"(d[11]), "+f"(d[12]), "+f"(d[13]), "+f"(d[14]), "+f"(d[15]),
        "+f"(d[16]), "+f"(d[17]), "+f"(d[18]), "+f"(d[19]), "+f"(d[20]), "+f"(d[21]), "+f"(d[22]), "+f"(d[23]),
        "+f"(d[24]), "+f"(d[25]), "+f"(d[26]), "+f"(d[27]), "+f"(d[28]), "+f"(d[29]), "+f"(d[30]), "+f"(d[31]),
        "+f"(d[32]), "+f"(d[33]), "+f"(d[34]), "+f"(d[35]), "+f"(d[36]), "+f"(d[37]), "+f"(d[38]), "+f"(d[39]),
        "+f"(d[40]), "+f"(d[41]), "+f"(d[42]), "+f"(d[43]), "+f"(d[44]), "+f"(d[45]), "+f"(d[46]), "+f"(d[47]),
        "+f"(d[48]), "+f"(d[49]), "+f"(d[50]), "+f"(d[51]), "+f"(d[52]), "+f"(d[53]), "+f"(d[54]), "+f"(d[55]),
        "+f"(d[56]), "+f"(d[57]), "+f"(d[58]), "+f"(d[59]), "+f"(d[60]), "+f"(d[61]), "+f"(d[62]), "+f"(d[63])
      : "l"(a_desc), "l"(b_desc), "r"(scale_d), "n"(TA), "n"(TB));
}
__device__ __forceinline__ void wgmma_m64n128k8_tf32(float (&d)[64], uint64_t a_desc, uint64_t b_desc, uint32_t scale_d) {
  asm volatile(
      "{\n\t"
      ".reg .pred p;\n\t"
      "setp.ne.b32 p, %66, 0;\n\t"
      "wgmma.mma_async.sync.aligned.m64n128k8.f32.tf32.tf32 "
      "{%0, %1, %2, %3, %4, %5, %6, %7, %8, %9, %10, %11, %12, %13, %14, %15, %16, %17, %18, %19, %20, %21, %22, %23, %24, %25, %26, %27, %28, %29, %30, %31, %32, %33, %34, %35, %36, %37, %38, %39, %40, %41, %42, %43, %44, %45, %46, %47, %48, %49, %50, %51, %52, %53, %54, %55, %56, %57, %58, %59, %60, %61, %62, %63}, "
      "%64, %65, p, 1, 1;\n\t"
      "}\n"
      : "+f"(d[0]), "+f"(d[1]), "+f"(d[2]), "+f"(d[3]), "+f"(d[4]), "+f"(d[5]), "+f"(d[6]), "+f"(d[7]),
        "+f"(d[8]), "+f"(d[9]), "+f"(d[10]), "+f"(d[11]), "+f"(d[12]), "+f"(d[13]), "+f"(d[14]), "+f"(d[15]),
        "+f"(d[16]), "+f"(d[17]), "+f"(d[18]), "+f"(d[19]), "+f"(d[20]), "+f"(d[21]), "+f"(d[22]), "+f"(d[23]),
        "+f"(d[24]), "+f"(d[25]), "+f"(d[26]), "+f"(d[27]), "+f"(d[28]), "+f"(d[29]), "+f"(d[30]), "+f"(d[31]),
        "+f"(d[32]), "+f"(d[33]), "+f"(d[34]), "+f"(d[35]), "+f"(d[36]), "+f"(d[37]), "+f"(d[38]), "+f"(d[39]),
        "+f"(d[40]), "+f"(d[41]), "+f"(d[42]), "+f"(d[43]), "+f"(d[44]), "+f"(d[45]), "+f"(d[46]), "+f"(d[47]),
        "+f"(d[48]), "+f"(d[49]), "+f"(d[50]), "+f"(d[51]), "+f"(d[52]), "+f"(d[53]), "+f"(d[54]), "+f"(d[55]),
        "+f"(d[56]), "+f"(d[57]), "+f"(d[58]), "+f"(d[59]), "+f"(d[60]), "+f"(d[61]), "+f"(d[62]), "+f"(d[63])
      : "l"(a_desc), "l"(b_desc), "r"(scale_d));
}

__device__ __forceinline__ void griddep_wait() { asm volatile("griddepcontrol.wait;" ::: "memory"); }
__device__ __forceinline__ void griddep_launch_dependents() { asm volatile("griddepcontrol.launch_dependents;" ::: "memory"); }
constexpr uint32_t kLayoutSw128 = 1;
__device__ __forceinline__ uint64_t make_smem_desc(uint32_t smem_addr, uint32_t lbo_bytes, uint32_t sbo_bytes, uint32_t layout) {
  uint64_t d = 0;
  d |= static_cast<uint64_t>((smem_addr & 0x3FFFF) >> 4);
  d |= static_cast<uint64_t>((lbo_bytes >> 4) & 0x3FFF) << 16;
  d |= static_cast<uint64_t>((sbo_bytes >> 4) & 0x3FFF) << 32;
  d |= static_cast<uint64_t>(layout) << 62;
  return d;
}
constexpr uint32_t kFmtF16 = 0, kFmtBF16 = 1, kFmtTF32 = 2;

}
}

#endif
```

### laser_b200/csrc/split.cuh

```cuda
#pragma once

#include <cuda_runtime.h>
#include <stdint.h>

#include <type_traits>

#include "f16_scale.cuh"
#include "layers.cuh"
#include "ptx.cuh"
#include "tc_params.h"

namespace lb200 {

#ifndef LB200_HOST_EMULATION
__device__ __forceinline__ float tf32_rna(float x) {
  uint32_t u;
  asm("cvt.rna.tf32.f32 %0, %1;" : "=r"(u) : "f"(x));
  return __uint_as_float(u);
}
#else
inline float tf32_rna(float x) {
  uint32_t u = __float_as_uint(x);
  if ((u & 0x7f800000u) != 0x7f800000u) u = (u + 0x1000u) & 0xffffe000u;
  return __uint_as_float(u);
}
#endif

__device__ __forceinline__ float tf32_lo(float x, float hi) {
  return ((__float_as_uint(hi) & 0x7f800000u) == 0x7f800000u) ? 0.0f : tf32_rna(x - hi);
}

struct OperandOp {
  int op = 0;
  const float *aux = nullptr;
  int64_t aux_sr = 0, aux_sc = 0;
};
#ifndef LB200_HOST_EMULATION
static __device__ __noinline__ float operand_act(int op, float x) {
#else
inline float operand_act(int op, float x) {
#endif
  return op == 2 ? tanhf(x) : 1.0f / (1.0f + expf(-x));
}
__device__ __forceinline__ float operand_op(int op, float x, float y) {
  switch (op) {
    case 1: return fmaxf(x, 0.0f);
    case 2:
    case 3: return operand_act(op, x);
    case 4: return y > 0.0f ? x : 0.0f;
    case 5: return __fmul_rn(x, __fsub_rn(1.0f, __fmul_rn(y, y)));
    case 6: return __fmul_rn(x, __fmul_rn(y, __fsub_rn(1.0f, y)));
    default: return x;
  }
}
__device__ __forceinline__ float4 load_row_vec(const float *row, int64_t c, int64_t Cc) {
  float4 v;
  if (c + 4 <= Cc) {
    v = *reinterpret_cast<const float4 *>(row + c);
  } else {
    v.x = row[c];
    v.y = (c + 1 < Cc) ? row[c + 1] : 0.0f;
    v.z = (c + 2 < Cc) ? row[c + 2] : 0.0f;
    v.w = 0.0f;
  }
  return v;
}
__device__ __forceinline__ float4 op_vec(const OperandOp &op, float4 v, int64_t r, int64_t c, int64_t Cc) {
  const float4 y = op.aux ? load_row_vec(op.aux + r * op.aux_sr, c, Cc) : make_float4(0.0f, 0.0f, 0.0f, 0.0f);
  v.x = operand_op(op.op, v.x, y.x);
  v.y = (c + 1 < Cc) ? operand_op(op.op, v.y, y.y) : 0.0f;
  v.z = (c + 2 < Cc) ? operand_op(op.op, v.z, y.z) : 0.0f;
  v.w = (c + 3 < Cc) ? operand_op(op.op, v.w, y.w) : 0.0f;
  return v;
}

struct Batch {
  int64_t n = 1;
  int64_t bs = 0, aux_bs = 0;
};
template <bool BATCHED>
__device__ __forceinline__ int64_t batch_row(int64_t g, int64_t R, const Batch &bt, const float *&src, OperandOp &op) {
  if constexpr (BATCHED) {
    const int64_t b = g / R;
    src += b * bt.bs;
    if (op.aux) op.aux += b * bt.aux_bs;
    return g - b * R;
  } else {
    return g;
  }
}

template <bool HAS_OP>
__device__ __forceinline__ float4 concat_vec(const float *src, int64_t src_ld, const OperandOp &op, const Batch &bt, int64_t r,
                                             int64_t c, int64_t Cc) {
  const int seg = static_cast<int>(Cc);
  int b = static_cast<int>(c) / seg;
  int k = static_cast<int>(c) - b * seg;
  if ((k & 3) == 0 && k + 4 <= seg) {
    float4 v = *reinterpret_cast<const float4 *>(src + b * bt.bs + r * src_ld + k);
    if constexpr (HAS_OP) {
      float4 y = make_float4(0.0f, 0.0f, 0.0f, 0.0f);
      if (op.aux) y = *reinterpret_cast<const float4 *>(op.aux + b * bt.aux_bs + r * op.aux_sr + k);
      v.x = operand_op(op.op, v.x, y.x); v.y = operand_op(op.op, v.y, y.y);
      v.z = operand_op(op.op, v.z, y.z); v.w = operand_op(op.op, v.w, y.w);
    }
    return v;
  }
  float e[4];
#pragma unroll
  for (int i = 0; i < 4; ++i) {
    while (k >= seg) { k -= seg; ++b; }
    float x = 0.0f;
    if (b < bt.n) {
      x = src[b * bt.bs + r * src_ld + k];
      if constexpr (HAS_OP) x = operand_op(op.op, x, op.aux ? op.aux[b * bt.aux_bs + r * op.aux_sr + k] : 0.0f);
    }
    e[i] = x;
    ++k;
  }
  return make_float4(e[0], e[1], e[2], e[3]);
}

template <bool HAS_OP = false, bool BATCHED = false, bool CONCAT = false>
__global__ void __launch_bounds__(256)
split_rows_tf32_kernel(const float *__restrict__ src, int64_t R, int64_t Cc, int64_t src_ld,
                       float *__restrict__ hi, float *__restrict__ lo, int64_t dst_ld, OperandOp op = OperandOp(),
                       Batch bt = Batch()) {
  static_assert(!CONCAT || BATCHED, "a concatenation is of a batch");
  ptx::griddep_launch_dependents();
  const int64_t vec_per_row = ((CONCAT ? bt.n * Cc : Cc) + 3) >> 2;
  const int64_t total = (BATCHED && !CONCAT ? bt.n * R : R) * vec_per_row;
  for (int64_t i = blockIdx.x * static_cast<int64_t>(blockDim.x) + threadIdx.x; i < total;
       i += static_cast<int64_t>(gridDim.x) * blockDim.x) {
    const int64_t r = i / vec_per_row;
    const int64_t c = (i - r * vec_per_row) << 2;
    float4 v;
    if constexpr (CONCAT) {
      v = concat_vec<HAS_OP>(src, src_ld, op, bt, r, c, Cc);
    } else {
      const float *sp = src;
      OperandOp o = op;
      const int64_t rl = batch_row<BATCHED>(r, R, bt, sp, o);
      const float *s = sp + rl * src_ld + c;
      if (c + 4 <= Cc) {
        v = *reinterpret_cast<const float4 *>(s);
      } else {
        v.x = s[0];
        v.y = (c + 1 < Cc) ? s[1] : 0.0f;
        v.z = (c + 2 < Cc) ? s[2] : 0.0f;
        v.w = 0.0f;
      }
      if constexpr (HAS_OP && BATCHED) v = op_vec(o, v, rl, c, Cc);
      else if constexpr (HAS_OP) v = op_vec(op, v, r, c, Cc);
    }
    float4 h, l;
    h.x = tf32_rna(v.x); l.x = tf32_lo(v.x, h.x);
    h.y = tf32_rna(v.y); l.y = tf32_lo(v.y, h.y);
    h.z = tf32_rna(v.z); l.z = tf32_lo(v.z, h.z);
    h.w = tf32_rna(v.w); l.w = tf32_lo(v.w, h.w);
    *reinterpret_cast<float4 *>(hi + r * dst_ld + c) = h;
    *reinterpret_cast<float4 *>(lo + r * dst_ld + c) = l;
  }
}

__device__ __forceinline__ uint32_t finite_abs_bits(float f) {
  const uint32_t a = __float_as_uint(f) & 0x7fffffffu;
  return a < 0x7f800000u ? a : 0u;
}
constexpr int ABSMAX_ROW_CHUNK = 1024;
constexpr int ABSMAX_COL_ROWS = 64;
template <bool PER_COL, bool HAS_OP = false, bool BATCHED = false, bool CONCAT = false>
__global__ void __launch_bounds__(256)
absmax_mn_kernel(const float *__restrict__ src, int64_t R, int64_t Cc, int64_t src_ld, uint32_t *__restrict__ out,
                 OperandOp op = OperandOp(), Batch bt = Batch()) {
  static_assert(PER_COL || !HAS_OP, "a K-major operand with an op takes the fused row kernel");
  static_assert(PER_COL || !BATCHED, "a K-major operand takes the fused row kernel");
  static_assert(!CONCAT || BATCHED, "a concatenation is of a batch");
  if constexpr (!PER_COL) {
    const int lane = threadIdx.x & 31;
    const int64_t chunks = (Cc + ABSMAX_ROW_CHUNK - 1) / ABSMAX_ROW_CHUNK;
    const int64_t items = R * chunks;
    const int64_t warps = (static_cast<int64_t>(gridDim.x) * blockDim.x) >> 5;
    for (int64_t it = (blockIdx.x * static_cast<int64_t>(blockDim.x) + threadIdx.x) >> 5; it < items; it += warps) {
      const int64_t r = it / chunks;
      const int64_t c0 = (it - r * chunks) * ABSMAX_ROW_CHUNK;
      const float *row = src + r * src_ld;
      uint32_t m = 0u;
#pragma unroll
      for (int i = 0; i < ABSMAX_ROW_CHUNK / 128; ++i) {
        const int64_t c = c0 + i * 128 + lane * 4;
        if (c + 4 <= Cc) {
          const float4 v = *reinterpret_cast<const float4 *>(row + c);
          m = max(max(m, finite_abs_bits(v.x)), max(finite_abs_bits(v.y), max(finite_abs_bits(v.z), finite_abs_bits(v.w))));
        } else if (c < Cc) {
          m = max(m, finite_abs_bits(row[c]));
          if (c + 1 < Cc) m = max(m, finite_abs_bits(row[c + 1]));
          if (c + 2 < Cc) m = max(m, finite_abs_bits(row[c + 2]));
        }
      }
      float mf = __uint_as_float(m);
#pragma unroll
      for (int o = 16; o > 0; o >>= 1) mf = fmaxf(mf, __shfl_xor_sync(0xffffffffu, mf, o));
      if (lane == 0) atomicMax(out + r, __float_as_uint(mf));
    }
  } else {
    const int64_t strips = (Cc + 3) >> 2;
    const int64_t rblocks = (R + ABSMAX_COL_ROWS - 1) / ABSMAX_COL_ROWS;
    const int64_t items = strips * (BATCHED ? bt.n * rblocks : rblocks);
    for (int64_t it = blockIdx.x * static_cast<int64_t>(blockDim.x) + threadIdx.x; it < items;
         it += static_cast<int64_t>(gridDim.x) * blockDim.x) {
      int64_t rb = it / strips;
      const int64_t c = (it - rb * strips) << 2;
      const float *src_b = src;
      OperandOp o = op;
      uint32_t *out_b = out;
      if constexpr (BATCHED) {
        const int64_t b = rb / rblocks;
        rb -= b * rblocks;
        batch_row<true>(b * R, R, bt, src_b, o);
        if constexpr (!CONCAT) out_b += b * Cc;
      }
      const int64_t r1 = (rb + 1) * ABSMAX_COL_ROWS < R ? (rb + 1) * ABSMAX_COL_ROWS : R;
      uint32_t m0 = 0u, m1 = 0u, m2 = 0u, m3 = 0u;
      for (int64_t r = rb * ABSMAX_COL_ROWS; r < r1; ++r) {
        const float *s = src_b + r * src_ld + c;
        if constexpr (HAS_OP) {
          const float4 v = op_vec(BATCHED ? o : op, load_row_vec(src_b + r * src_ld, c, Cc), r, c, Cc);
          m0 = max(m0, finite_abs_bits(v.x)); m1 = max(m1, finite_abs_bits(v.y));
          m2 = max(m2, finite_abs_bits(v.z)); m3 = max(m3, finite_abs_bits(v.w));
        } else if (c + 4 <= Cc) {
          const float4 v = *reinterpret_cast<const float4 *>(s);
          m0 = max(m0, finite_abs_bits(v.x)); m1 = max(m1, finite_abs_bits(v.y));
          m2 = max(m2, finite_abs_bits(v.z)); m3 = max(m3, finite_abs_bits(v.w));
        } else {
          m0 = max(m0, finite_abs_bits(s[0]));
          if (c + 1 < Cc) m1 = max(m1, finite_abs_bits(s[1]));
          if (c + 2 < Cc) m2 = max(m2, finite_abs_bits(s[2]));
        }
      }
      atomicMax(out_b + c, m0);
      if (c + 1 < Cc) atomicMax(out_b + c + 1, m1);
      if (c + 2 < Cc) atomicMax(out_b + c + 2, m2);
      if (c + 3 < Cc) atomicMax(out_b + c + 3, m3);
    }
  }
}

__device__ __forceinline__ void store_f16x2_vec4(float4 v, float sx, float sy, float sz, float sw, uint16_t *hrow, uint16_t *lrow,
                                                 int64_t c) {
  uint2 h, l;
  f16x2_pieces2(__fmul_rn(v.x, sx), __fmul_rn(v.y, sy), h.x, l.x);
  f16x2_pieces2(__fmul_rn(v.z, sz), __fmul_rn(v.w, sw), h.y, l.y);
  *reinterpret_cast<uint2 *>(hrow + c) = h;
  *reinterpret_cast<uint2 *>(lrow + c) = l;
}
__device__ __forceinline__ void store_f16x2_vec(float4 v, float s, uint16_t *hrow, uint16_t *lrow, int64_t c) {
  store_f16x2_vec4(v, s, s, s, s, hrow, lrow, c);
}

constexpr int F16ROWS_MAXV = 8;
template <int GROUP, bool HAS_OP = false, bool BATCHED = false, bool CONCAT = false>
__global__ void __launch_bounds__(256, 4)
f16x2_rows_fused_kernel(const float *__restrict__ src, int64_t R, int64_t Cc, int64_t src_ld, uint16_t *__restrict__ hb,
                        uint16_t *__restrict__ lb, int64_t ld_b, uint32_t *__restrict__ absmax, OperandOp op = OperandOp(),
                        Batch bt = Batch()) {
  static_assert(GROUP == 32 || GROUP == 256, "a warp or the CTA per row");
  static_assert(!CONCAT || BATCHED, "a concatenation is of a batch");
  __shared__ uint32_t red[2][8];
  ptx::griddep_launch_dependents();
  const int tid = static_cast<int>(threadIdx.x) % GROUP;
  const int64_t per_cta = 256 / GROUP;
  const int64_t first = static_cast<int64_t>(blockIdx.x) * per_cta + static_cast<int64_t>(threadIdx.x) / GROUP;
  const int64_t step = static_cast<int64_t>(gridDim.x) * per_cta;
  const int64_t nvec = ((CONCAT ? bt.n * Cc : Cc) + 3) >> 2;
  int parity = 0;
  const int64_t rows = BATCHED && !CONCAT ? bt.n * R : R;
  for (int64_t r = first; r < rows; r += step) {
    const float *sp = src;
    OperandOp o = op;
    const int64_t rl = batch_row<BATCHED && !CONCAT>(r, R, bt, sp, o);
    const float *row = sp + rl * src_ld;
    float4 v[F16ROWS_MAXV];
    uint32_t m = 0u;
#pragma unroll
    for (int i = 0; i < F16ROWS_MAXV; ++i) {
      const int64_t idx = tid + static_cast<int64_t>(i) * GROUP;
      if (idx < nvec) {
        if constexpr (CONCAT) {
          v[i] = concat_vec<HAS_OP>(src, src_ld, op, bt, r, idx << 2, Cc);
        } else {
          v[i] = load_row_vec(row, idx << 2, Cc);
          if constexpr (HAS_OP) v[i] = op_vec(o, v[i], rl, idx << 2, Cc);
        }
        m = max(max(m, finite_abs_bits(v[i].x)), max(finite_abs_bits(v[i].y), max(finite_abs_bits(v[i].z), finite_abs_bits(v[i].w))));
      }
    }
    for (int64_t idx = tid + static_cast<int64_t>(F16ROWS_MAXV) * GROUP; idx < nvec; idx += GROUP) {
      float4 t;
      if constexpr (CONCAT) {
        t = concat_vec<HAS_OP>(src, src_ld, op, bt, r, idx << 2, Cc);
      } else {
        t = load_row_vec(row, idx << 2, Cc);
        if constexpr (HAS_OP) t = op_vec(o, t, rl, idx << 2, Cc);
      }
      m = max(max(m, finite_abs_bits(t.x)), max(finite_abs_bits(t.y), max(finite_abs_bits(t.z), finite_abs_bits(t.w))));
    }
    float mf = __uint_as_float(m);
#pragma unroll
    for (int o = 16; o > 0; o >>= 1) mf = fmaxf(mf, __shfl_xor_sync(0xffffffffu, mf, o));
    m = __float_as_uint(mf);
    if constexpr (GROUP == 256) {
      if ((threadIdx.x & 31) == 0) red[parity][threadIdx.x >> 5] = m;
      __syncthreads();
#pragma unroll
      for (int w = 0; w < 8; ++w) m = max(m, red[parity][w]);
      parity ^= 1;
    }
    if (tid == 0) absmax[r] = m;
    const float s = f16x2_scale(m);
    uint16_t *hrow = hb + r * ld_b, *lrow = lb + r * ld_b;
#pragma unroll
    for (int i = 0; i < F16ROWS_MAXV; ++i) {
      const int64_t idx = tid + static_cast<int64_t>(i) * GROUP;
      if (idx < nvec) store_f16x2_vec(v[i], s, hrow, lrow, idx << 2);
    }
    for (int64_t idx = tid + static_cast<int64_t>(F16ROWS_MAXV) * GROUP; idx < nvec; idx += GROUP) {
      if constexpr (CONCAT) store_f16x2_vec(concat_vec<HAS_OP>(src, src_ld, op, bt, r, idx << 2, Cc), s, hrow, lrow, idx << 2);
      else if constexpr (HAS_OP) store_f16x2_vec(op_vec(o, load_row_vec(row, idx << 2, Cc), rl, idx << 2, Cc), s, hrow, lrow, idx << 2);
      else store_f16x2_vec(load_row_vec(row, idx << 2, Cc), s, hrow, lrow, idx << 2);
    }
  }
}

constexpr int F16RING_BUFS = 3;
__global__ void __launch_bounds__(256, 2)
f16x2_rows_ring_kernel(const float *__restrict__ src, int64_t R, int64_t Cc, int64_t src_ld, uint16_t *__restrict__ hb,
                       uint16_t *__restrict__ lb, int64_t ld_b, uint32_t *__restrict__ absmax) {
  LB200_DYN_SMEM(uint8_t, ring_raw);
  __shared__ uint32_t red[2][8];
  __shared__ uint64_t full[F16RING_BUFS];
  ptx::griddep_launch_dependents();
  uint8_t *ring = reinterpret_cast<uint8_t *>((reinterpret_cast<uintptr_t>(ring_raw) + 127) & ~static_cast<uintptr_t>(127));
  const uint32_t row_bytes = static_cast<uint32_t>(Cc) * 4u;
  const uint32_t buf_bytes = (row_bytes + 127u) & ~127u;
  const int tid = static_cast<int>(threadIdx.x);
  const int64_t first = blockIdx.x, step = gridDim.x;
  const int nvec = static_cast<int>(Cc >> 2);
  if (tid == 0) {
    for (int i = 0; i < F16RING_BUFS; ++i) ptx::mbar_init(&full[i], 1);
    ptx::fence_barrier_init();
    for (int i = 0; i < F16RING_BUFS; ++i) {
      const int64_t r = first + i * step;
      if (r < R) {
        ptx::mbar_arrive_expect_tx(&full[i], row_bytes);
        ptx::bulk_load_1d(ring + i * buf_bytes, src + r * src_ld, row_bytes, &full[i]);
      }
    }
  }
  __syncthreads();
  int b = 0, parity = 0;
  uint32_t phase = 0;
  for (int64_t r = first; r < R; r += step) {
    ptx::mbar_wait(&full[b], phase);
    const float4 *row = reinterpret_cast<const float4 *>(ring + b * buf_bytes);
    float4 v[F16ROWS_MAXV];
    uint32_t m = 0u;
#pragma unroll
    for (int i = 0; i < F16ROWS_MAXV; ++i) {
      const int idx = tid + i * 256;
      if (idx < nvec) {
        v[i] = row[idx];
        m = max(max(m, finite_abs_bits(v[i].x)), max(finite_abs_bits(v[i].y), max(finite_abs_bits(v[i].z), finite_abs_bits(v[i].w))));
      }
    }
    float mf = __uint_as_float(m);
#pragma unroll
    for (int o = 16; o > 0; o >>= 1) mf = fmaxf(mf, __shfl_xor_sync(0xffffffffu, mf, o));
    if ((tid & 31) == 0) red[parity][tid >> 5] = __float_as_uint(mf);
    __syncthreads();
    if (tid == 0) {
      const int64_t rn = r + F16RING_BUFS * step;
      if (rn < R) {
        ptx::mbar_arrive_expect_tx(&full[b], row_bytes);
        ptx::bulk_load_1d(ring + b * buf_bytes, src + rn * src_ld, row_bytes, &full[b]);
      }
    }
    m = 0u;
#pragma unroll
    for (int w = 0; w < 8; ++w) m = max(m, red[parity][w]);
    parity ^= 1;
    if (tid == 0) absmax[r] = m;
    const float s = f16x2_scale(m);
    uint16_t *hrow = hb + r * ld_b, *lrow = lb + r * ld_b;
#pragma unroll
    for (int i = 0; i < F16ROWS_MAXV; ++i) {
      const int idx = tid + i * 256;
      if (idx < nvec) store_f16x2_vec(v[i], s, hrow, lrow, static_cast<int64_t>(idx) << 2);
    }
    if (++b == F16RING_BUFS) { b = 0; phase ^= 1u; }
  }
}
inline size_t f16x2_rows_ring_smem(int64_t Cc) { return static_cast<size_t>(F16RING_BUFS) * ((Cc * 4 + 127) / 128 * 128) + 128; }
inline bool f16x2_rows_ring_ok(const float *src, int64_t Cc, int64_t src_ld) {
  return Cc % 4 == 0 && src_ld % 4 == 0 && Cc > 4 * 32 * F16ROWS_MAXV && Cc <= 4 * 256 * F16ROWS_MAXV &&
         (reinterpret_cast<uintptr_t>(src) & 15) == 0;
}

constexpr int SPLIT_ROWS = 64;
template <bool PER_COL, bool HAS_OP = false, bool BATCHED = false, bool CONCAT = false>
__global__ void __launch_bounds__(256)
split_rows_f16x2_kernel(const float *__restrict__ src, int64_t R, int64_t Cc, int64_t src_ld,
                        uint16_t *__restrict__ hb, uint16_t *__restrict__ lb, int64_t ld_b,
                        const uint32_t *__restrict__ absmax, OperandOp op = OperandOp(), Batch bt = Batch()) {
  static_assert(PER_COL || !BATCHED, "a K-major operand takes the fused row kernel");
  static_assert(!CONCAT || BATCHED, "a concatenation is of a batch");
  ptx::griddep_launch_dependents();
  const int tx = static_cast<int>(threadIdx.x) & 63, ty = static_cast<int>(threadIdx.x) >> 6;
  const int64_t strips = (Cc + 255) >> 8;
  const int64_t rblocks = (R + SPLIT_ROWS - 1) / SPLIT_ROWS;
  for (int64_t it = blockIdx.x; it < strips * (BATCHED ? bt.n * rblocks : rblocks); it += gridDim.x) {
    int64_t rb = it / strips;
    const int64_t c = ((it - rb * strips) << 8) + (tx << 2);
    if (c >= Cc) continue;
    const float *src_b = src;
    OperandOp o = op;
    const uint32_t *absmax_b = absmax;
    uint16_t *hb_b = hb, *lb_b = lb;
    if constexpr (BATCHED) {
      const int64_t b = rb / rblocks;
      rb -= b * rblocks;
      batch_row<true>(b * R, R, bt, src_b, o);
      if constexpr (!CONCAT) absmax_b += b * Cc;
      hb_b += b * R * ld_b;
      lb_b += b * R * ld_b;
    }
    float sx = 1.0f, sy = 1.0f, sz = 1.0f, sw = 1.0f;
    if constexpr (PER_COL) {
      sx = f16x2_scale(absmax_b[c]);
      sy = (c + 1 < Cc) ? f16x2_scale(absmax_b[c + 1]) : 1.0f;
      sz = (c + 2 < Cc) ? f16x2_scale(absmax_b[c + 2]) : 1.0f;
      sw = (c + 3 < Cc) ? f16x2_scale(absmax_b[c + 3]) : 1.0f;
    }
    const int64_t r1 = (rb + 1) * SPLIT_ROWS < R ? (rb + 1) * SPLIT_ROWS : R;
#pragma unroll 4
    for (int64_t r = rb * SPLIT_ROWS + ty; r < r1; r += 4) {
      float4 v = load_row_vec(src_b + r * src_ld, c, Cc);
      if constexpr (HAS_OP) v = op_vec(o, v, r, c, Cc);
      if constexpr (!PER_COL) sx = sy = sz = sw = f16x2_scale(absmax_b[r]);
      store_f16x2_vec4(v, sx, sy, sz, sw, hb_b + r * ld_b, lb_b + r * ld_b, c);
    }
  }
}

enum Im2colMode { IM2COL_F32 = 0, IM2COL_TF32 = 1, IM2COL_F16X2 = 2 };
struct Im2colSrc {
  int C, H, W, kH, kW, pH, pW, sH, sW, outW, K;
  int64_t outHW, image;
};
inline Im2colSrc im2col_src(const ConvGeom &g) {
  return Im2colSrc{static_cast<int>(g.C), static_cast<int>(g.H), static_cast<int>(g.W), static_cast<int>(g.kH),
                   static_cast<int>(g.kW), static_cast<int>(g.pH), static_cast<int>(g.pW), static_cast<int>(g.sH),
                   static_cast<int>(g.sW), static_cast<int>(g.outW), static_cast<int>(g.K()), g.outHW(), g.C * g.H * g.W};
}
__device__ __forceinline__ float4 window_vec(const float *__restrict__ img, const Im2colSrc &q, int oh, int ow, int k) {
  const int khw = q.kH * q.kW;
  int c = k / khw;
  int kr = (k - c * khw) / q.kW;
  int kc = k - c * khw - kr * q.kW;
  float v[4];
#pragma unroll
  for (int e = 0; e < 4; ++e) {
    const int h = oh * q.sH - q.pH + kr, w = ow * q.sW - q.pW + kc;
    const bool inside = k + e < q.K && static_cast<unsigned>(h) < static_cast<unsigned>(q.H) &&
                        static_cast<unsigned>(w) < static_cast<unsigned>(q.W);
    v[e] = inside ? img[(static_cast<int64_t>(c) * q.H + h) * q.W + w] : 0.0f;
    if (++kc == q.kW) { kc = 0; if (++kr == q.kH) { kr = 0; ++c; } }
  }
  return make_float4(v[0], v[1], v[2], v[3]);
}

struct Im2colGradSrc : Im2colSrc {
  int dH, dW;
  OperandOp op;
};
struct Im2colNhwcSrc : Im2colSrc {
  int vec;
};
inline Im2colNhwcSrc im2col_nhwc_src(const ConvGeom &g, const float *in) {
  Im2colNhwcSrc q{};
  static_cast<Im2colSrc &>(q) = im2col_src(g);
  q.vec = g.C % 4 == 0 && (reinterpret_cast<uintptr_t>(in) & 15) == 0;
  return q;
}
__device__ __forceinline__ float4 nhwc_window_vec(const float *__restrict__ img, const Im2colNhwcSrc &q, int oh, int ow, int k) {
  const int tap = k / q.C;
  int ci = k - tap * q.C;
  int kr = tap / q.kW, kc = tap - kr * q.kW;
  if (q.vec) {
    const int h = oh * q.sH - q.pH + kr, w = ow * q.sW - q.pW + kc;
    if (k < q.K && static_cast<unsigned>(h) < static_cast<unsigned>(q.H) && static_cast<unsigned>(w) < static_cast<unsigned>(q.W))
      return *reinterpret_cast<const float4 *>(img + (static_cast<int64_t>(h) * q.W + w) * q.C + ci);
    return make_float4(0.0f, 0.0f, 0.0f, 0.0f);
  }
  float v[4];
#pragma unroll
  for (int e = 0; e < 4; ++e) {
    const int h = oh * q.sH - q.pH + kr, w = ow * q.sW - q.pW + kc;
    const bool inside = k + e < q.K && static_cast<unsigned>(h) < static_cast<unsigned>(q.H) &&
                        static_cast<unsigned>(w) < static_cast<unsigned>(q.W);
    v[e] = inside ? img[(static_cast<int64_t>(h) * q.W + w) * q.C + ci] : 0.0f;
    if (++ci == q.C) { ci = 0; if (++kc == q.kW) { kc = 0; ++kr; } }
  }
  return make_float4(v[0], v[1], v[2], v[3]);
}

struct Im2colNhwcGradSrc : Im2colNhwcSrc {
  int dH, dW;
  OperandOp op;
};
template <bool DIL>
__device__ __forceinline__ bool dilated_source(const Im2colNhwcGradSrc &q, int &h, int &w) {
  if constexpr (DIL) {
    const unsigned hq = static_cast<unsigned>(h) / static_cast<unsigned>(q.dH), wq = static_cast<unsigned>(w) / static_cast<unsigned>(q.dW);
    const bool inside = h >= 0 && w >= 0 && hq * q.dH == static_cast<unsigned>(h) && wq * q.dW == static_cast<unsigned>(w) &&
                        hq < static_cast<unsigned>(q.H) && wq < static_cast<unsigned>(q.W);
    h = static_cast<int>(hq);
    w = static_cast<int>(wq);
    return inside;
  } else {
    return static_cast<unsigned>(h) < static_cast<unsigned>(q.H) && static_cast<unsigned>(w) < static_cast<unsigned>(q.W);
  }
}
template <bool DIL, bool HAS_OP>
__device__ __forceinline__ float4 nhwc_grad_window_vec(const float *__restrict__ img, const float *__restrict__ aux,
                                                       const Im2colNhwcGradSrc &q, int oh, int ow, int k) {
  const int tap = k / q.C;
  int co = k - tap * q.C;
  int kr = tap / q.kW, kc = tap - kr * q.kW;
  if (q.vec) {
    int h = oh - q.pH + kr, w = ow - q.pW + kc;
    if (k < q.K && dilated_source<DIL>(q, h, w)) {
      const int64_t off = (static_cast<int64_t>(h) * q.W + w) * q.C + co;
      float4 v = *reinterpret_cast<const float4 *>(img + off);
      if constexpr (HAS_OP) {
        const float4 y = aux ? *reinterpret_cast<const float4 *>(aux + off) : make_float4(0.0f, 0.0f, 0.0f, 0.0f);
        v = make_float4(operand_op(q.op.op, v.x, y.x), operand_op(q.op.op, v.y, y.y), operand_op(q.op.op, v.z, y.z),
                        operand_op(q.op.op, v.w, y.w));
      }
      return v;
    }
    return make_float4(0.0f, 0.0f, 0.0f, 0.0f);
  }
  float v[4];
#pragma unroll
  for (int e = 0; e < 4; ++e) {
    int h = oh - q.pH + kr, w = ow - q.pW + kc;
    float x = 0.0f;
    if (k + e < q.K && dilated_source<DIL>(q, h, w)) {
// ... 451 lines not shown
```

### laser_b200/csrc/tc_launch.h

```cpp
#pragma once

#include <cuda.h>
#include <cuda_runtime.h>

#include "tc_params.h"

namespace lb200 {

struct TcLaunch {
  CUtensorMap a0, a1, b0, b1;
  TcParams p;
  bool a_mn = false, b_mn = false;
  bool batched = false;
  bool pdl = false;
  int dev = 0, sm_count = 0;
  cudaStream_t stream = nullptr;
};

int launch_tc_tf32x1(const TcLaunch &l);
int launch_tc_tf32x3(const TcLaunch &l);
int launch_tc_bf16(const TcLaunch &l);
int launch_tc_f16x3(const TcLaunch &l);

}
```

### laser_b200/csrc/tc_launch_impl.cuh

```cuda
#pragma once

#include <atomic>

#include "gemm_tc.cuh"
#include "tc_launch.h"

#ifndef LB200_LAUNCH_EX
#define LB200_LAUNCH_EX cudaLaunchKernelEx
#endif

namespace lb200 {

template <int ESZ, uint32_t FMT16, int NPASS, typename OutT, bool SCALED, bool A_MN, bool B_MN, bool BATCHED>
int launch_tc_one(const TcLaunch &l) {
  using Cfg = TcCfg<NPASS>;
  const int64_t units_total = tc_units(l.p);
  cudaLaunchConfig_t cfg{};
  cfg.gridDim = dim3(static_cast<int>(units_total < l.sm_count ? units_total : l.sm_count));
  cfg.blockDim = dim3(TC_THREADS);
  cfg.dynamicSmemBytes = Cfg::SMEM_BYTES;
  cfg.stream = l.stream;
  cudaLaunchAttribute attr[1];
  if (l.pdl) {
    attr[0].id = cudaLaunchAttributeProgrammaticStreamSerialization;
    attr[0].val.programmaticStreamSerializationAllowed = 1;
    cfg.attrs = attr;
    cfg.numAttrs = 1;
  }
  auto kfn = gemm_tc_kernel<ESZ, FMT16, NPASS, A_MN, B_MN, OutT, SCALED, BATCHED>;
  static std::atomic<uint32_t> attr_set{0};
  if (!(attr_set.load(std::memory_order_acquire) & (1u << l.dev))) {
    const cudaError_t e = cudaFuncSetAttribute(kfn, cudaFuncAttributeMaxDynamicSharedMemorySize, Cfg::SMEM_BYTES);
    if (e != cudaSuccess) return static_cast<int>(e);
    attr_set.fetch_or(1u << l.dev, std::memory_order_release);
  }
  return static_cast<int>(LB200_LAUNCH_EX(&cfg, kfn, l.a0, l.a1, l.b0, l.b1, l.p));
}

template <int ESZ, uint32_t FMT16, int NPASS, typename OutT, bool SCALED>
int launch_tc_family(const TcLaunch &l) {
  if constexpr (ESZ == 4) {
    if (l.a_mn || l.b_mn) return static_cast<int>(cudaErrorNotSupported);
    if (l.batched) return launch_tc_one<ESZ, FMT16, NPASS, OutT, SCALED, false, false, true>(l);
    return launch_tc_one<ESZ, FMT16, NPASS, OutT, SCALED, false, false, false>(l);
  }
#define LB200_MAJORS(BATCHED)                                                                                  \
  do {                                                                                                         \
    if (!l.a_mn && !l.b_mn) return launch_tc_one<ESZ, FMT16, NPASS, OutT, SCALED, false, false, BATCHED>(l);   \
    if (!l.a_mn && l.b_mn) return launch_tc_one<ESZ, FMT16, NPASS, OutT, SCALED, false, true, BATCHED>(l);     \
    if (l.a_mn && !l.b_mn) return launch_tc_one<ESZ, FMT16, NPASS, OutT, SCALED, true, false, BATCHED>(l);     \
    return launch_tc_one<ESZ, FMT16, NPASS, OutT, SCALED, true, true, BATCHED>(l);                             \
  } while (0)
  if constexpr (ESZ == 2) {
    if constexpr (SCALED) {
      if (l.batched) LB200_MAJORS(true);
    }
    if (l.batched) return static_cast<int>(cudaErrorNotSupported);
    LB200_MAJORS(false);
  }
#undef LB200_MAJORS
}

}
```

### laser_b200/csrc/tc_params.h

```cpp
#pragma once

#include <stdint.h>

#if defined(__CUDACC__) || defined(LB200_HOST_EMULATION)
#define LB200_HD __host__ __device__
#else
#define LB200_HD
#endif

namespace lb200 {

constexpr int TC_BLOCK_M = 128;
constexpr int TC_BLOCK_N = 128;
constexpr int TC_ROW_BYTES = 128;
constexpr int TC_A_TILE_BYTES = TC_BLOCK_M * TC_ROW_BYTES;
template <int NPASS> struct TcCfg {
  static constexpr int PIECES = (NPASS == 3) ? 2 : 1;
  static constexpr int B_TILE_BYTES = TC_BLOCK_N * TC_ROW_BYTES;
  static constexpr int A_STAGE_BYTES = PIECES * TC_A_TILE_BYTES;
  static constexpr int B_STAGE_BYTES = PIECES * B_TILE_BYTES;
  static constexpr int STAGE_BYTES = A_STAGE_BYTES + B_STAGE_BYTES;
#ifdef TC_STAGES_OVERRIDE
  static constexpr int STAGES = TC_STAGES_OVERRIDE;
#else
  static constexpr int STAGES = (NPASS == 3) ? 3 : 6;
#endif
  static constexpr int SMEM_BYTES = STAGES * STAGE_BYTES + 1024  + 512 ;
};
constexpr int TC_THREADS = 384;
constexpr int TC_EPI_THREADS = 256;
constexpr int TC_EPI_WARPS = TC_EPI_THREADS / 32;
constexpr int TC_ACC_REGS = 64 * TC_BLOCK_N / 128;
constexpr int TC_REGS_CTRL = 40;
constexpr int TC_REGS_EPI = 232;

struct Epilogue {
  const float *bias = nullptr;
  int bias_per_row = 0;
  int act = 0;
};
struct TcParams {
  int64_t M, N, K;
  float alpha, beta;
  void *C;
  int64_t rsC, csC;
  int kb_per_block;
  int raster_g;
  Epilogue epi;
  int n_direct;
  int k_splits;
  int kb_per_split;
  float *split_ws = nullptr;
  int num_m_blocks, num_n_blocks;
  const uint32_t *amax_a = nullptr, *amax_b = nullptr;
  unsigned int *sched = nullptr;
  int batch = 1;
  int period_a = 1, period_b = 1;
  int64_t bsC = 0;
  int64_t amax_bs_a = 0, amax_bs_b = 0;
  int64_t bias_bs = 0;
};

LB200_HD inline void tile_coords(int t, int num_m, int num_n, int G, int &mb, int &nb) {
  const int per_group = G * num_n;
  const int g = t / per_group;
  const int first_m = g * G;
  const int gsz = (G < num_m - first_m) ? G : (num_m - first_m);
  const int r = t - g * per_group;
  mb = first_m + r % gsz;
  nb = r / gsz;
}

struct TcPlanCfg {
  int kc_faithful;
  int raster_g;
  bool splitk_enabled;
  int sm_count;
  int tail_min_k = 2048;
};
template <int ESZ, bool OUT_F32>
inline void tc_plan(TcParams &p, int npass, const TcPlanCfg &cfg) {
  const int block_k = TC_ROW_BYTES / ESZ;
  const int num_kb = static_cast<int>((p.K + block_k - 1) / block_k);
  {
    const int kc = (npass == 3) ? cfg.kc_faithful : 0;
    p.kb_per_block = (kc > 0) ? (kc + block_k - 1) / block_k : num_kb;
    if (p.kb_per_block < 1) p.kb_per_block = 1;
    if (p.kb_per_block > num_kb) p.kb_per_block = num_kb;
  }
  p.raster_g = cfg.raster_g > 0 ? cfg.raster_g : 16;
  p.num_m_blocks = static_cast<int>((p.M + TC_BLOCK_M - 1) / TC_BLOCK_M);
  p.num_n_blocks = static_cast<int>((p.N + TC_BLOCK_N - 1) / TC_BLOCK_N);
  const int64_t tiles = static_cast<int64_t>(p.num_m_blocks) * p.num_n_blocks * p.batch;
  p.k_splits = 1;
  p.kb_per_split = num_kb;
  p.n_direct = static_cast<int>(tiles);
  p.split_ws = nullptr;
  const int units = cfg.sm_count;
  if constexpr (OUT_F32) {
    const int blocks = (num_kb + p.kb_per_block - 1) / p.kb_per_block;
    const int min_tiles = 512 / block_k;
    const int min_blocks = (min_tiles + p.kb_per_block - 1) / p.kb_per_block;
    const int max_s = blocks / min_blocks < 16 ? blocks / min_blocks : 16;
    const int64_t rem = tiles < units ? tiles : tiles % units;
    int S = rem > 0 ? static_cast<int>(units / rem) : 1;
    if (S > max_s) S = max_s;
    const bool worth = S >= 2 && (tiles < units || p.K >= cfg.tail_min_k);
    if (cfg.splitk_enabled && worth && units > 0) {
      const int blocks_per_split = (blocks + S - 1) / S;
      p.k_splits = (blocks + blocks_per_split - 1) / blocks_per_split;
      p.kb_per_split = blocks_per_split * p.kb_per_block;
      if (p.k_splits >= 2) p.n_direct = static_cast<int>(tiles - rem);
      else { p.k_splits = 1; p.kb_per_split = num_kb; }
    }
  }
}
inline int64_t tc_units(const TcParams &p) {
  const int64_t tiles = static_cast<int64_t>(p.num_m_blocks) * p.num_n_blocks * p.batch;
  return p.n_direct + (tiles - p.n_direct) * p.k_splits;
}
inline int64_t tc_split_ws_floats(const TcParams &p) {
  const int64_t tiles = static_cast<int64_t>(p.num_m_blocks) * p.num_n_blocks * p.batch;
  return (tiles - p.n_direct) * p.k_splits * TC_BLOCK_M * TC_BLOCK_N;
}

}
```

Baseline: 209.1.

## Fuse f16x3 operand preparation into the persistent GEMM kernel via panel work units

Adds a fused path for fp32 f16x3 GEMMs in which the persistent tensor-core kernel also does the operand preparation. Panel-prep units (absmax scaling and hi/lo f16 splitting of A/B row or column panels) are interleaved into the dynamic schedule, and consumers wait on per-panel global ready flags using acquire/release. The aim is to remove the separate prep kernels and their extra global memory round trip and launch serialization, letting the prep overlap with the GEMM. In exchange it adds cross-CTA flag spinning, a host-computed unit sequence, and extra shared memory, which risks stalls if panels are not ready when tiles need them.

Result: slower. 188.1 (median of 6 runs) (-10.0%).

```diff
diff --git a/laser_b200/_build.py b/laser_b200/_build.py
--- a/laser_b200/_build.py
+++ b/laser_b200/_build.py
@@ -11,7 +11,7 @@
 OBJ_DIR = os.path.join(LIB_DIR, "obj")
 LIB_PATH = os.path.join(LIB_DIR, "liblaser_b200.so")
 SOURCES = ["capi.cu", "tc_f16x3.cu", "tc_tf32x3.cu", "tc_tf32x1.cu", "tc_bf16.cu"]
-HEADERS = ["ptx.cuh", "f16_scale.cuh", "gemm_tc.cuh", "tc_params.h", "tc_launch.h", "tc_launch_impl.cuh", "gemm_simt.cuh", "gemm_dmma.cuh",
+HEADERS = ["ptx.cuh", "f16_scale.cuh", "gemm_tc.cuh", "gemm_tc_kernel.inc", "tc_params.h", "tc_launch.h", "tc_launch_impl.cuh", "gemm_simt.cuh", "gemm_dmma.cuh",
            "gemm_simt_kernel.inc", "split.cuh", "layers.cuh", "capi_layers.inc", "capi_multi.inc",
            "../../include/laser_b200.h"]
 
diff --git a/laser_b200/csrc/capi.cu b/laser_b200/csrc/capi.cu
--- a/laser_b200/csrc/capi.cu
+++ b/laser_b200/csrc/capi.cu
@@ -98,6 +98,7 @@
   int kc_faithful = 128;
   bool dyn_sched = true;
   bool pdl = true;
+  bool fused_prep = true;
   int64_t batch_ws_bytes = static_cast<int64_t>(1024) << 20;
   bool profiling = false;
   std::vector<EventPair> prof;
@@ -117,6 +118,10 @@
   Buffer f16s;
   Buffer sched;
   int sched_next = 0;
+  Buffer prep_ready;
+  uint32_t prep_seq = 0;
+  Buffer prep_units;
+  int64_t prep_units_key[6] = {};
   cudaEvent_t ws_free = nullptr;
   std::mutex mu;
   std::mutex host_mu;
@@ -180,6 +185,7 @@
       if (const char *pt = getenv("LASER_B200_PANEL_TAPER")) c.panel_taper = atoi(pt) != 0;
       if (const char *ds = getenv("LASER_B200_DYNSCHED")) c.dyn_sched = atoi(ds) != 0;
       if (const char *pd = getenv("LASER_B200_PDL")) c.pdl = atoi(pd) != 0;
+      if (const char *fp = getenv("LASER_B200_FUSED_PREP")) c.fused_prep = atoi(fp) != 0;
       if (const char *bw = getenv("LASER_B200_BATCH_WS_MB")) {
         const int64_t v = atoll(bw);
         if (v >= 1) c.batch_ws_bytes = v << 20;
@@ -682,11 +688,16 @@
   int64_t batch, C, bias = 0;
 };
 
+struct FusedPrep {
+  CUtensorMap sa, sb;
+  TcParams::PrepOperand a, b;
+};
+
 template <typename OutT>
 int tc_run(Ctx &c, TcKind kind, int64_t M, int64_t N, int64_t K, float alpha, const OperandMaps &ma,
            const OperandMaps &mb, float beta, OutT *C, int64_t rsC, int64_t csC, cudaStream_t s,
            const Epilogue &epi, const F16Scales *f16 = nullptr, bool after_prep = false, const BatchArgs *bat = nullptr,
-           int64_t period_a = 1, int64_t period_b = 1) {
+           int64_t period_a = 1, int64_t period_b = 1, const FusedPrep *fused = nullptr) {
   TcLaunch l;
   l.a0 = ma.p0; l.a1 = ma.p1; l.b0 = mb.p0; l.b1 = mb.p1;
   l.a_mn = ma.mn_major; l.b_mn = mb.mn_major;
@@ -713,6 +724,34 @@
   if (c.dyn_sched) {
     p.sched = static_cast<unsigned int *>(c.sched.ptr) + 2 * c.sched_next;
     c.sched_next = (c.sched_next + 1) % kSchedSlots;
+  }
+  if (fused) {
+    if (!p.sched) return set_error(LASER_B200_ECUDA, "internal: the fused preparation needs the dynamic scheduler");
+    l.prep = true;
+    l.sa = fused->sa;
+    l.sb = fused->sb;
+    p.prep_a = fused->a;
+    p.prep_b = fused->b;
+    p.n_prep = p.num_m_blocks + p.num_n_blocks;
+    const size_t ready_bytes = static_cast<size_t>(p.n_prep) * sizeof(uint32_t);
+    if (c.prep_ready.bytes < ready_bytes) {
+      int rc;
+      if ((rc = ensure(c.prep_ready, ready_bytes))) return rc;
+      CUDA_TRY(cudaMemsetAsync(c.prep_ready.ptr, 0, c.prep_ready.bytes, s));
+    }
+    if (++c.prep_seq == 0) c.prep_seq = 1;
+    p.ready = static_cast<uint32_t *>(c.prep_ready.ptr);
+    p.ready_seq = c.prep_seq;
+    const int64_t key[6] = {p.num_m_blocks, p.num_n_blocks, p.raster_g, p.n_direct, p.k_splits, c.sm_count};
+    if (memcmp(key, c.prep_units_key, sizeof key) != 0) {
+      std::vector<int> seq(static_cast<size_t>(tc_units(p) + p.n_prep));
+      tc_prep_sequence(p, c.sm_count, seq.data());
+      int rc;
+      if ((rc = ensure(c.prep_units, seq.size() * sizeof(int)))) return rc;
+      CUDA_TRY(cudaMemcpyAsync(c.prep_units.ptr, seq.data(), seq.size() * sizeof(int), cudaMemcpyHostToDevice, s));
+      memcpy(c.prep_units_key, key, sizeof key);
+    }
+    p.unit_seq = static_cast<const int *>(c.prep_units.ptr);
   }
   auto launch = [&](const TcLaunch &q) -> int {
     int e;
@@ -763,6 +802,48 @@
   return stride == 0 && (!op || !op->aux || aux_stride == 0);
 }
 
+int gemm_tc_fused(Ctx &c, const Operand &oa, const Operand &ob, float alpha, float beta, float *C, int64_t rsC, int64_t csC,
+                  cudaStream_t s, const Epilogue &epi) {
+  int64_t f16_b_off = 0;
+  int rc;
+  if ((rc = f16_scales(c, oa.mn, ob.mn, &f16_b_off))) return rc;
+  FusedPrep fp;
+  OperandMaps ma, mb;
+  auto operand = [&](const Operand &o, const OperandWs &w, int block_mn, OperandMaps *m, CUtensorMap *src,
+                     TcParams::PrepOperand *po) {
+    const Major mj = classify(o, 4);
+    const int64_t R = mj == K_MAJOR ? o.mn : o.k, Cc = mj == K_MAJOR ? o.k : o.mn;
+    const int64_t ld_b = round_up(Cc, 8);
+    const size_t bytes_b = static_cast<size_t>(R) * ld_b * 2;
+    int e;
+    if ((e = ensure(*w.p0, bytes_b)) || (e = ensure(*w.p1, bytes_b))) return e;
+    m->mn_major = mj == MN_MAJOR;
+    if ((e = operand_map(c, &m->p0, 2, w.p0->ptr, mj, o.mn, o.k, ld_b, block_mn))) return e;
+    if ((e = operand_map(c, &m->p1, 2, w.p1->ptr, mj, o.mn, o.k, ld_b, block_mn))) return e;
+    if ((e = encode_map(c, src, 4, o.ptr, Cc, R, mj == K_MAJOR ? o.s_mn : o.s_k, TC_PREP_STRIP, TC_PREP_BOX,
+                        CU_TENSOR_MAP_SWIZZLE_NONE)))
+      return e;
+    po->h = static_cast<uint16_t *>(w.p0->ptr);
+    po->l = static_cast<uint16_t *>(w.p1->ptr);
+    po->ld = ld_b;
+    po->words = static_cast<uint32_t *>(c.f16s.ptr) + w.amax_off;
+    po->R = R;
+    po->Cc = Cc;
+    po->mn_major = mj == MN_MAJOR;
+    return LASER_B200_OK;
+  };
+  if ((rc = operand(oa, ws_of_A(c), TC_BLOCK_M, &ma, &fp.sa, &fp.a))) return rc;
+  if ((rc = operand(ob, ws_of_B(c, f16_b_off), TC_BLOCK_N, &mb, &fp.sb, &fp.b))) return rc;
+  ProfBracket prep;
+  if ((rc = prep.open(c, s, 1)) || (rc = prep.close())) return rc;
+  const F16Scales f16{static_cast<const uint32_t *>(c.f16s.ptr), static_cast<const uint32_t *>(c.f16s.ptr) + f16_b_off};
+  if ((rc = tc_run<float>(c, TC_F16X3, oa.mn, ob.mn, oa.k, alpha, ma, mb, beta, C, rsC, csC, s, epi, &f16, false, nullptr, 1, 1,
+                          &fp)))
+    return rc;
+  CUDA_TRY(cudaEventRecord(c.ws_free, s));
+  return LASER_B200_OK;
+}
+
 template <int SRC_ESZ, typename OutT>
 int gemm_tc(Ctx &c, TcKind kind, const Operand &oa, const Operand &ob, float alpha, float beta, OutT *C, int64_t rsC, int64_t csC,
             cudaStream_t s, const Epilogue &epi, cudaEvent_t b_ready = nullptr, const OperandOp *opA = nullptr,
@@ -777,6 +858,13 @@
   OperandMaps ma, mb;
   bool used_ws = false;
   CUDA_TRY(cudaStreamWaitEvent(s, c.ws_free, 0));
+  if constexpr (SRC_ESZ == 4 && std::is_same<OutT, float>::value) {
+    const int64_t tiles = ((M + TC_BLOCK_M - 1) / TC_BLOCK_M) * ((N + TC_BLOCK_N - 1) / TC_BLOCK_N);
+    if (kind == TC_F16X3 && c.fused_prep && c.dyn_sched && !bat && !b_ready && !opA && !opB && !oa.conv && !ob.conv &&
+        oa.batch == 0 && ob.batch == 0 && !cat && classify(oa, 4) != GENERAL && classify(ob, 4) != GENERAL &&
+        tiles >= 2 * static_cast<int64_t>(c.sm_count))
+      return gemm_tc_fused(c, oa, ob, alpha, beta, C, rsC, csC, s, epi);
+  }
   ProfBracket prep;
   int rc = prep.open(c, s, 1);
   if (rc) return rc;
diff --git a/laser_b200/csrc/f16_scale.cuh b/laser_b200/csrc/f16_scale.cuh
--- a/laser_b200/csrc/f16_scale.cuh
+++ b/laser_b200/csrc/f16_scale.cuh
@@ -88,4 +88,17 @@
 #endif
 }
 
+__device__ __forceinline__ uint32_t finite_abs_bits(float f) {
+  const uint32_t a = __float_as_uint(f) & 0x7fffffffu;
+  return a < 0x7f800000u ? a : 0u;
 }
+__device__ __forceinline__ void store_f16x2_vec4(float4 v, float sx, float sy, float sz, float sw, uint16_t *hrow, uint16_t *lrow,
+                                                 int64_t c) {
+  uint2 h, l;
+  f16x2_pieces2(__fmul_rn(v.x, sx), __fmul_rn(v.y, sy), h.x, l.x);
+  f16x2_pieces2(__fmul_rn(v.z, sz), __fmul_rn(v.w, sw), h.y, l.y);
+  *reinterpret_cast<uint2 *>(hrow + c) = h;
+  *reinterpret_cast<uint2 *>(lrow + c) = l;
+}
+
+}
diff --git a/laser_b200/csrc/gemm_tc.cuh b/laser_b200/csrc/gemm_tc.cuh
--- a/laser_b200/csrc/gemm_tc.cuh
+++ b/laser_b200/csrc/gemm_tc.cuh
@@ -29,321 +29,110 @@
   return static_cast<uint16_t>(u >> 16);
 }
 
-template <int ESZ, uint32_t FMT16, int NPASS, bool A_MN, bool B_MN, typename OutT, bool SCALED, bool BATCHED>
-__global__ void __launch_bounds__(TC_THREADS, 1)
-gemm_tc_kernel(const __grid_constant__ CUtensorMap mapA0, const __grid_constant__ CUtensorMap mapA1,
-               const __grid_constant__ CUtensorMap mapB0, const __grid_constant__ CUtensorMap mapB1,
-               const TcParams p) {
-  static_assert(NPASS == 1 || NPASS == 3, "one pass, or the three passes of a two-piece product");
-  static_assert(ESZ == 2 || (!A_MN && !B_MN), "wgmma reads tf32 operands K-major only (capi.cu transposes MN-major fp32)");
-  using Cfg = TcCfg<NPASS>;
-  constexpr int STAGES = Cfg::STAGES;
-  constexpr int BLOCK_K = TC_ROW_BYTES / ESZ;
-  const int sched_id = static_cast<int>(blockIdx.x);
-  const int sched_stride = static_cast<int>(gridDim.x);
-
-  LB200_DYN_SMEM(uint8_t, smem_raw);
-  uint8_t *smem = reinterpret_cast<uint8_t *>((reinterpret_cast<uintptr_t>(smem_raw) + 1023) &
-                                              ~static_cast<uintptr_t>(1023));
-  uint64_t *bars = reinterpret_cast<uint64_t *>(smem + STAGES * Cfg::STAGE_BYTES);
-  uint64_t *full_bar = bars;
-  uint64_t *empty_bar = bars + STAGES;
-  uint64_t *sched_full = bars + 2 * STAGES;
-  uint64_t *sched_empty = sched_full + 1;
-  int *sched_unit = reinterpret_cast<int *>(sched_empty + 1);
-
-  const int warp_idx = threadIdx.x >> 5;
-  const int lane = threadIdx.x & 31;
-  const int tiles_pp = p.num_m_blocks * p.num_n_blocks;
-  const int num_tiles = BATCHED ? tiles_pp * p.batch : tiles_pp;
-  const int num_kb = static_cast<int>((p.K + BLOCK_K - 1) / BLOCK_K);
-  const int num_units = p.n_direct + (num_tiles - p.n_direct) * p.k_splits;
-  auto decode_unit = [&](int u, int &t, int &sp, int &kb_lo, int &kb_hi) {
-    if (u < p.n_direct) {
-      t = u; sp = -1; kb_lo = 0; kb_hi = num_kb;
+template <int STAGES, int STAGE_BYTES>
+__device__ __forceinline__ void prep_panel(const TcParams &p, int i, uint8_t *smem, uint64_t *full_bar, uint64_t *empty_bar,
+                                           uint64_t *prep_bar, uint32_t *red, int &stage, uint32_t &phase, uint32_t &prep_phase) {
+  constexpr int V = TC_PREP_STRIP / 4;
+  const int ct = static_cast<int>(threadIdx.x) - (TC_THREADS - TC_EPI_THREADS);
+  const int w = ct >> 5, lane = ct & 31;
+  const bool is_a = i < p.num_m_blocks;
+  uint16_t *const hb = is_a ? p.prep_a.h : p.prep_b.h;
+  uint16_t *const lb = is_a ? p.prep_a.l : p.prep_b.l;
+  uint32_t *const words = is_a ? p.prep_a.words : p.prep_b.words;
+  const int64_t ld = is_a ? p.prep_a.ld : p.prep_b.ld;
+  const int64_t R = is_a ? p.prep_a.R : p.prep_b.R, Cc = is_a ? p.prep_a.Cc : p.prep_b.Cc;
+  const bool per_col = is_a ? p.prep_a.mn_major : p.prep_b.mn_major;
+  const int64_t panel0 = static_cast<int64_t>(is_a ? i : i - p.num_m_blocks) * TC_PREP_BOX;
+  const int chunks = static_cast<int>(((per_col ? R : Cc) + TC_PREP_BOX - 1) / TC_PREP_BOX);
+  auto consumers_sync = [&]() {
+    ptx::mbar_arrive(prep_bar);
+    ptx::mbar_wait(prep_bar, prep_phase);
+    prep_phase ^= 1u;
+  };
+  auto release_stage = [&]() {
+    __syncwarp();
+    if (lane == 0) ptx::mbar_arrive(&empty_bar[stage]);
+    if (++stage == STAGES) { stage = 0; phase ^= 1u; }
+  };
+  const int lane_off = (lane / V) * TC_PREP_BOX * V + lane % V;
+  uint32_t m[16];
+#pragma unroll
+  for (int k = 0; k < 16; ++k) m[k] = 0u;
+  for (int q = 0; q < chunks; ++q) {
+    ptx::mbar_wait(&full_bar[stage], phase);
+    const float4 *box = reinterpret_cast<const float4 *>(smem + stage * STAGE_BYTES) + lane_off + 16 * w * V;
+    if (per_col) {
+#pragma unroll
+      for (int k = 0; k < 16; ++k) {
+        const float4 v = box[k * V];
+        m[0] = max(m[0], finite_abs_bits(v.x)); m[1] = max(m[1], finite_abs_bits(v.y));
+        m[2] = max(m[2], finite_abs_bits(v.z)); m[3] = max(m[3], finite_abs_bits(v.w));
+      }
     } else {
-      const int v = u - p.n_direct;
-      const int i = v / p.k_splits;
-      t = p.n_direct + i;
-      sp = v - i * p.k_splits;
-      kb_lo = min(num_kb, sp * p.kb_per_split);
-      kb_hi = min(num_kb, kb_lo + p.kb_per_split);
+#pragma unroll
+      for (int k = 0; k < 16; ++k) {
+        const float4 v = box[k * V];
+        m[k] = max(max(m[k], finite_abs_bits(v.x)), max(finite_abs_bits(v.y), max(finite_abs_bits(v.z), finite_abs_bits(v.w))));
+      }
     }
-  };
-  constexpr int SCHED_CONSUMERS = 1 + TC_EPI_WARPS;
-  auto next_unit = [&](uint32_t &ph) -> int {
-    ptx::mbar_wait(sched_full, ph);
-    const int u = *reinterpret_cast<volatile int *>(sched_unit);
-    ptx::mbar_arrive(sched_empty);
-    ph ^= 1u;
-    return u;
-  };
-
-  if (threadIdx.x == 0) {
-    ptx::prefetch_tensormap(&mapA0);
-    ptx::prefetch_tensormap(&mapB0);
-    if constexpr (NPASS == 3) {
-      ptx::prefetch_tensormap(&mapA1);
-      ptx::prefetch_tensormap(&mapB1);
+    release_stage();
+  }
+  float s[16];
+  if (per_col) {
+#pragma unroll
+    for (int e = 0; e < 4; ++e) red[w * TC_PREP_BOX + 4 * lane + e] = m[e];
+    consumers_sync();
+    const int64_t c = panel0 + 4 * lane;
+#pragma unroll
+    for (int e = 0; e < 4; ++e) {
+      uint32_t mm = 0u;
+#pragma unroll
+      for (int v = 0; v < TC_EPI_WARPS; ++v) mm = max(mm, red[v * TC_PREP_BOX + 4 * lane + e]);
+      if (w == 0 && c + e < Cc) words[c + e] = mm;
+      s[e] = f16x2_scale(mm);
+    }
+  } else {
+#pragma unroll
+    for (int k = 0; k < 16; ++k) {
+      float mf = __uint_as_float(m[k]);
+#pragma unroll
+      for (int o = 16; o > 0; o >>= 1) mf = fmaxf(mf, __shfl_xor_sync(0xffffffffu, mf, o));
+      const int64_t r = panel0 + 16 * w + k;
+      if (lane == 0 && r < R) words[r] = __float_as_uint(mf);
+      s[k] = f16x2_scale(__float_as_uint(mf));
     }
   }
-  if (threadIdx.x == 32) {
-    for (int i = 0; i < STAGES; ++i) {
-      ptx::mbar_init(&full_bar[i], 1);
-      ptx::mbar_init(&empty_bar[i], TC_EPI_WARPS);
-    }
-    ptx::mbar_init(sched_full, 1);
-    ptx::mbar_init(sched_empty, SCHED_CONSUMERS);
-    ptx::fence_barrier_init();
-  }
-  __syncthreads();
-  ptx::griddep_wait();
-
-  if (warp_idx < 4) {
-    ptx::setmaxnreg_dec<TC_REGS_CTRL>();
-    if (warp_idx == 3 && lane == 0) {
-      uint32_t phase = 0;
-      int next_static = sched_id;
-      for (;;) {
-        ptx::mbar_wait(sched_empty, phase ^ 1);
-        int u;
-        if (p.sched) {
-          u = static_cast<int>(atomicAdd(p.sched, 1u));
-        } else {
-          u = next_static;
-          next_static += sched_stride;
-        }
-        if (u >= num_units) u = -1;
-        *reinterpret_cast<volatile int *>(sched_unit) = u;
-        ptx::mbar_arrive(sched_full);
-        phase ^= 1u;
-        if (u < 0) {
-          if (p.sched) {
-            __threadfence();
-            if (atomicAdd(p.sched + 1, 1u) == static_cast<unsigned int>(sched_stride - 1)) {
-              p.sched[0] = 0u;
-              p.sched[1] = 0u;
-              __threadfence();
-            }
-          }
-          break;
-        }
-      }
-    } else if (warp_idx == 0 && lane == 0) {
-      int stage = 0;
-      uint32_t phase = 0, sched_phase = 0;
-      constexpr int MN_ATOM = TC_ROW_BYTES / ESZ;
-      constexpr int MN_BOX_BYTES = BLOCK_K * TC_ROW_BYTES;
-      auto load_a = [&](uint8_t *dst, const CUtensorMap *m, uint64_t *bar, int m0, int k0, int z) {
-        if constexpr (!A_MN) {
-          if constexpr (BATCHED) ptx::tma_load_3d(dst, m, bar, k0, m0, z);
-          else ptx::tma_load_2d(dst, m, bar, k0, m0);
-        } else {
+  for (int q = 0; q < chunks; ++q) {
+    ptx::mbar_wait(&full_bar[stage], phase);
+    const float4 *box = reinterpret_cast<const float4 *>(smem + stage * STAGE_BYTES) + lane_off + 16 * w * V;
+    const int64_t r0 = per_col ? static_cast<int64_t>(q) * TC_PREP_BOX + 16 * w : panel0 + 16 * w;
+    const int64_t c = (per_col ? panel0 : static_cast<int64_t>(q) * TC_PREP_BOX) + 4 * lane;
+    if (c < Cc) {
+      if (per_col) {
 #pragma unroll
-          for (int c = 0; c < TC_BLOCK_M / MN_ATOM; ++c) {
-            if constexpr (BATCHED) ptx::tma_load_3d(dst + c * MN_BOX_BYTES, m, bar, m0 + c * MN_ATOM, k0, z);
-            else ptx::tma_load_2d(dst + c * MN_BOX_BYTES, m, bar, m0 + c * MN_ATOM, k0);
-          }
-        }
-      };
-      auto load_b = [&](uint8_t *dst, const CUtensorMap *m, uint64_t *bar, int n0, int k0, int z) {
-        if constexpr (!B_MN) {
-          if constexpr (BATCHED) ptx::tma_load_3d(dst, m, bar, k0, n0, z);
-          else ptx::tma_load_2d(dst, m, bar, k0, n0);
-        } else {
+        for (int k = 0; k < 16; ++k)
+          if (r0 + k < R) store_f16x2_vec4(box[k * V], s[0], s[1], s[2], s[3], hb + (r0 + k) * ld, lb + (r0 + k) * ld, c);
+      } else {
 #pragma unroll
-          for (int c = 0; c < TC_BLOCK_N / MN_ATOM; ++c) {
-            if constexpr (BATCHED) ptx::tma_load_3d(dst + c * MN_BOX_BYTES, m, bar, n0 + c * MN_ATOM, k0, z);
-            else ptx::tma_load_2d(dst + c * MN_BOX_BYTES, m, bar, n0 + c * MN_ATOM, k0);
-          }
-        }
-      };
-      for (;;) {
-        const int u = next_unit(sched_phase);
-        if (u < 0) break;
-        int t, sp, mb, nb, kb_lo, kb_hi;
-        decode_unit(u, t, sp, kb_lo, kb_hi);
-        int za = 0, zb = 0;
-        if constexpr (BATCHED) {
-          const int bz = t / tiles_pp;
-          t -= bz * tiles_pp;
-          za = bz % p.period_a;
-          zb = bz % p.period_b;
-        }
-        tile_coords(t, p.num_m_blocks, p.num_n_blocks, p.raster_g, mb, nb);
-        const int m0 = mb * TC_BLOCK_M;
-        const int n0 = nb * TC_BLOCK_N;
-        for (int kb = kb_lo; kb < kb_hi; ++kb) {
-          ptx::mbar_wait(&empty_bar[stage], phase ^ 1);
-          ptx::mbar_arrive_expect_tx(&full_bar[stage], Cfg::STAGE_BYTES);
-          uint8_t *sa = smem + stage * Cfg::STAGE_BYTES;
-          uint8_t *sb = sa + Cfg::A_STAGE_BYTES;
-          const int k0 = kb * BLOCK_K;
-          load_a(sa, &mapA0, &full_bar[stage], m0, k0, za);
-          if constexpr (NPASS == 3) load_a(sa + TC_A_TILE_BYTES, &mapA1, &full_bar[stage], m0, k0, za);
-          load_b(sb, &mapB0, &full_bar[stage], n0, k0, zb);
-          if constexpr (NPASS == 3) load_b(sb + Cfg::B_TILE_BYTES, &mapB1, &full_bar[stage], n0, k0, zb);
-          if (++stage == STAGES) { stage = 0; phase ^= 1; }
-        }
+        for (int k = 0; k < 16; ++k)
+          if (r0 + k < R) store_f16x2_vec4(box[k * V], s[k], s[k], s[k], s[k], hb + (r0 + k) * ld, lb + (r0 + k) * ld, c);
       }
     }
-  } else {
-    ptx::setmaxnreg_inc<TC_REGS_EPI>();
-    const int g = (warp_idx - 4) >> 2;
-    const int wq = warp_idx & 3;
-    const int lr = lane >> 2;
-    const int lc = 2 * (lane & 3);
-    constexpr int MMA_K = 32 / ESZ;
-    constexpr int K_STEPS = BLOCK_K / MMA_K;
-    constexpr int MN_BOX_BYTES = BLOCK_K * TC_ROW_BYTES;
-    constexpr uint32_t A_WG_BYTES = 64 * TC_ROW_BYTES;
-    int stage = 0;
-    uint32_t phase = 0, sched_phase = 0;
-    const bool vec_ok_c = (p.csC == 1) && ((p.rsC & 1) == 0) && ((reinterpret_cast<uintptr_t>(p.C) & (2 * sizeof(OutT) - 1)) == 0) &&
-                          (!BATCHED || (p.bsC & 1) == 0);
-    float acc[TC_ACC_REGS];
-#pragma unroll
-    for (int j = 0; j < TC_ACC_REGS; ++j) acc[j] = 0.0f;
-    for (;;) {
-      int u = 0;
-      if (lane == 0) u = next_unit(sched_phase);
-      u = __shfl_sync(0xffffffffu, u, 0);
-      if (u < 0) break;
-      int t, sp, mb, nb, kb_lo, kb_hi;
-      decode_unit(u, t, sp, kb_lo, kb_hi);
-      int bz = 0, za = 0, zb = 0;
-      if constexpr (BATCHED) {
-        bz = t / tiles_pp;
-        za = bz % p.period_a;
-        zb = bz % p.period_b;
-        int tl = t - bz * tiles_pp;
-        tile_coords(tl, p.num_m_blocks, p.num_n_blocks, p.raster_g, mb, nb);
-      } else {
-        tile_coords(t, p.num_m_blocks, p.num_n_blocks, p.raster_g, mb, nb);
-      }
-      const int num_blocks = (kb_hi - kb_lo + p.kb_per_block - 1) / p.kb_per_block;
-      const int r_tile = 64 * g + 16 * wq + lr;
-      const int64_t row0 = static_cast<int64_t>(mb) * TC_BLOCK_M + r_tile;
-      const int64_t col0 = static_cast<int64_t>(nb) * TC_BLOCK_N + lc;
-      const bool split_unit = sp >= 0;
-      uint32_t amax_row[2] = {0u, 0u}, amax_col[2 * TC_BLOCK_N / 8];
-      if constexpr (SCALED) {
-#pragma unroll
-        for (int h = 0; h < 2; ++h)
-          if (row0 + 8 * h < p.M) amax_row[h] = p.amax_a[(BATCHED ? za * p.amax_bs_a : 0) + row0 + 8 * h];
-#pragma unroll
-        for (int j = 0; j < 2 * TC_BLOCK_N / 8; ++j) {
-          const int64_t c = col0 + 8 * (j >> 1) + (j & 1);
-          amax_col[j] = c < p.N ? p.amax_b[(BATCHED ? zb * p.amax_bs_b : 0) + c] : 0u;
-        }
-      }
-      float run[TC_ACC_REGS];
-#pragma unroll
-      for (int j = 0; j < TC_ACC_REGS; ++j) run[j] = 0.0f;
-      for (int blk = 0; blk < num_blocks; ++blk) {
-        const int kb0 = kb_lo + blk * p.kb_per_block;
-        const int kb1 = min(kb_hi, kb0 + p.kb_per_block);
-        int prev_stage = -1;
-        for (int kb = kb0; kb < kb1; ++kb) {
-          ptx::mbar_wait(&full_bar[stage], phase);
-          ptx::wgmma_fence();
-          const uint32_t a_addr = ptx::smem_u32(smem + stage * Cfg::STAGE_BYTES) + g * A_WG_BYTES;
-          const uint32_t b_addr = ptx::smem_u32(smem + stage * Cfg::STAGE_BYTES + Cfg::A_STAGE_BYTES);
-#pragma unroll
-          for (int pass = 0; pass < NPASS; ++pass) {
-            const uint32_t a_tile = a_addr + ((NPASS == 3 && pass == 1) ? TC_A_TILE_BYTES : 0);
-            const uint32_t b_tile = b_addr + ((NPASS == 3 && pass == 0) ? Cfg::B_TILE_BYTES : 0);
-#pragma unroll
-            for (int k = 0; k < K_STEPS; ++k) {
-              const uint64_t ad = A_MN ? ptx::make_smem_desc(a_tile + k * MMA_K * TC_ROW_BYTES, MN_BOX_BYTES, 1024, ptx::kLayoutSw128)
-                                       : ptx::make_smem_desc(a_tile + k * 32, 0, 1024, ptx::kLayoutSw128);
-              const uint64_t bd = B_MN ? ptx::make_smem_desc(b_tile + k * MMA_K * TC_ROW_BYTES, MN_BOX_BYTES, 1024, ptx::kLayoutSw128)
-                                       : ptx::make_smem_desc(b_tile + k * 32, 0, 1024, ptx::kLayoutSw128);
-              const uint32_t accum = (kb == kb0 && pass == 0 && k == 0) ? 0u : 1u;
-              if constexpr (ESZ == 4) ptx::wgmma_m64n128k8_tf32(acc, ad, bd, accum);
-              else if constexpr (FMT16 == ptx::kFmtF16) ptx::wgmma_m64n128k16_f16<A_MN ? 1 : 0, B_MN ? 1 : 0>(acc, ad, bd, accum);
-              else ptx::wgmma_m64n128k16_bf16<A_MN ? 1 : 0, B_MN ? 1 : 0>(acc, ad, bd, accum);
-            }
-          }
-          ptx::wgmma_commit();
-          ptx::wgmma_wait<1>();
-          if (prev_stage >= 0 && lane == 0) ptx::mbar_arrive(&empty_bar[prev_stage]);
-          prev_stage = stage;
-          if (++stage == STAGES) { stage = 0; phase ^= 1; }
-        }
-        ptx::wgmma_wait<0>();
-        ptx::wgmma_hold(acc);
-        if (prev_stage >= 0 && lane == 0) ptx::mbar_arrive(&empty_bar[prev_stage]);
-#pragma unroll
-        for (int j = 0; j < TC_ACC_REGS; ++j) run[j] = __fadd_rn(run[j], acc[j]);
-      }
-      float alpha_r[2] = {split_unit ? 1.0f : p.alpha, split_unit ? 1.0f : p.alpha};
-      if constexpr (SCALED) {
-#pragma unroll
-        for (int h = 0; h < 2; ++h) alpha_r[h] *= f16x2_unscale(amax_row[h]);
-      }
-      const float beta_u = split_unit ? 0.0f : p.beta;
-      const bool has_epi = !split_unit && ((p.epi.bias != nullptr) || (p.epi.act != 0));
-      float *ws_base = nullptr;
-      if (split_unit) {
-        const int64_t plane = static_cast<int64_t>(sp) * (num_tiles - p.n_direct) + (t - p.n_direct);
-        ws_base = p.split_ws + (plane * TC_BLOCK_M + r_tile) * TC_BLOCK_N + lc;
-      }
-#pragma unroll
-      for (int h = 0; h < 2; ++h) {
-        const int64_t row = row0 + 8 * h;
-        if (!split_unit && row >= p.M) continue;
-        const float row_bias =
-            (has_epi && p.epi.bias && p.epi.bias_per_row) ? p.epi.bias[(BATCHED ? za * p.bias_bs : 0) + row] : 0.0f;
-        OutT *crow = split_unit ? nullptr : reinterpret_cast<OutT *>(p.C) + (BATCHED ? bz * p.bsC : 0) + row * p.rsC;
-#pragma unroll
-        for (int i = 0; i < TC_BLOCK_N / 8; ++i) {
-          float v[2];
-#pragma unroll
-          for (int e = 0; e < 2; ++e) {
-            v[e] = alpha_r[h] * run[4 * i + 2 * h + e];
-            if constexpr (SCALED) v[e] *= f16x2_unscale(amax_col[2 * i + e]);
-          }
-          if (split_unit) {
-            *reinterpret_cast<float2 *>(ws_base + 8 * h * TC_BLOCK_N + 8 * i) = make_float2(v[0], v[1]);
-            continue;
-          }
-          const int64_t c = col0 + 8 * i;
-          if (c >= p.N) continue;
-          const bool pair_ok = vec_ok_c && c + 1 < p.N;
-          OutT *dst = crow + c * p.csC;
-          if (beta_u != 0.0f) {
-            float o[2] = {0.0f, 0.0f};
-            if constexpr (sizeof(OutT) == 4) {
-              if (pair_ok) { const float2 w = *reinterpret_cast<const float2 *>(dst); o[0] = w.x; o[1] = w.y; }
-              else { o[0] = dst[0]; if (c + 1 < p.N) o[1] = dst[p.csC]; }
-            } else {
-              o[0] = bf16_bits_to_f32(dst[0]);
-              if (c + 1 < p.N) o[1] = bf16_bits_to_f32(dst[pair_ok ? 1 : p.csC]);
-            }
-#pragma unroll
-            for (int e = 0; e < 2; ++e) v[e] = fmaf(beta_u, o[e], v[e]);
-          }
-          if (has_epi) {
-#pragma unroll
-            for (int e = 0; e < 2; ++e) {
-              const float bv = (p.epi.bias && !p.epi.bias_per_row) ? (c + e < p.N ? p.epi.bias[c + e] : 0.0f) : row_bias;
-              v[e] = epi_act(v[e] + bv, p.epi.act);
-            }
-          }
-          if constexpr (sizeof(OutT) == 4) {
-            if (pair_ok) *reinterpret_cast<float2 *>(dst) = make_float2(v[0], v[1]);
-            else { dst[0] = v[0]; if (c + 1 < p.N) dst[p.csC] = v[1]; }
-          } else {
-            if (pair_ok) *reinterpret_cast<uint32_t *>(dst) = f32_to_bf16_bits(v[0]) | (static_cast<uint32_t>(f32_to_bf16_bits(v[1])) << 16);
-            else { dst[0] = f32_to_bf16_bits(v[0]); if (c + 1 < p.N) dst[p.csC] = f32_to_bf16_bits(v[1]); }
-          }
-        }
-      }
-    }
+    release_stage();
   }
-
-  __syncthreads();
+  consumers_sync();
+  if (ct == 0) {
+    __threadfence();
+    ptx::fence_proxy_async_global();
+    ptx::st_release_gpu(p.ready + i, p.ready_seq);
+  }
 }
 
+#define LB200_TC_PREP 0
+#include "gemm_tc_kernel.inc"
+#undef LB200_TC_PREP
+#define LB200_TC_PREP 1
+#include "gemm_tc_kernel.inc"
+#undef LB200_TC_PREP
+
 }
diff --git a/laser_b200/csrc/gemm_tc_kernel.inc b/laser_b200/csrc/gemm_tc_kernel.inc
--- /dev/null
+++ b/laser_b200/csrc/gemm_tc_kernel.inc
@@ -0,0 +1,394 @@
+#if LB200_TC_PREP
+template <bool A_MN, bool B_MN>
+__global__ void __launch_bounds__(TC_THREADS, 1)
+gemm_tc_prep_kernel(const __grid_constant__ CUtensorMap mapA0, const __grid_constant__ CUtensorMap mapA1,
+                    const __grid_constant__ CUtensorMap mapB0, const __grid_constant__ CUtensorMap mapB1,
+                    const TcParams p, const __grid_constant__ CUtensorMap srcA, const __grid_constant__ CUtensorMap srcB) {
+  constexpr int ESZ = 2, NPASS = 3;
+  constexpr uint32_t FMT16 = ptx::kFmtF16;
+  using OutT = float;
+  constexpr bool SCALED = true, BATCHED = false;
+#else
+template <int ESZ, uint32_t FMT16, int NPASS, bool A_MN, bool B_MN, typename OutT, bool SCALED, bool BATCHED>
+__global__ void __launch_bounds__(TC_THREADS, 1)
+gemm_tc_kernel(const __grid_constant__ CUtensorMap mapA0, const __grid_constant__ CUtensorMap mapA1,
+               const __grid_constant__ CUtensorMap mapB0, const __grid_constant__ CUtensorMap mapB1,
+               const TcParams p) {
+#endif
+  static_assert(NPASS == 1 || NPASS == 3, "one pass, or the three passes of a two-piece product");
+#if LB200_TC_PREP
+  static_assert(SCALED && !BATCHED && NPASS == 3 && TcCfg<NPASS>::STAGE_BYTES == TC_PREP_BOX * TC_PREP_BOX * 4,
+                "one fp32 source box per stage");
+#endif
+  static_assert(ESZ == 2 || (!A_MN && !B_MN), "wgmma reads tf32 operands K-major only (capi.cu transposes MN-major fp32)");
+  using Cfg = TcCfg<NPASS>;
+  constexpr int STAGES = Cfg::STAGES;
+  constexpr int BLOCK_K = TC_ROW_BYTES / ESZ;
+  const int sched_id = static_cast<int>(blockIdx.x);
+  const int sched_stride = static_cast<int>(gridDim.x);
+
+  LB200_DYN_SMEM(uint8_t, smem_raw);
+  uint8_t *smem = reinterpret_cast<uint8_t *>((reinterpret_cast<uintptr_t>(smem_raw) + 1023) &
+                                              ~static_cast<uintptr_t>(1023));
+  uint64_t *bars = reinterpret_cast<uint64_t *>(smem + STAGES * Cfg::STAGE_BYTES);
+  uint64_t *full_bar = bars;
+  uint64_t *empty_bar = bars + STAGES;
+  uint64_t *sched_full = bars + 2 * STAGES;
+  uint64_t *sched_empty = sched_full + 1;
+  int *sched_unit = reinterpret_cast<int *>(sched_empty + 1);
+#if LB200_TC_PREP
+  uint64_t *prep_bar = sched_empty + 2;
+  uint32_t *prep_red = reinterpret_cast<uint32_t *>(smem + STAGES * Cfg::STAGE_BYTES + 512);
+#endif
+
+  const int warp_idx = threadIdx.x >> 5;
+  const int lane = threadIdx.x & 31;
+  const int tiles_pp = p.num_m_blocks * p.num_n_blocks;
+  const int num_tiles = BATCHED ? tiles_pp * p.batch : tiles_pp;
+  const int num_kb = static_cast<int>((p.K + BLOCK_K - 1) / BLOCK_K);
+#if LB200_TC_PREP
+  const int num_units = p.n_direct + (num_tiles - p.n_direct) * p.k_splits + p.n_prep;
+#define LB200_TC_NO_MORE(u) ((u) == -1)
+#else
+  const int num_units = p.n_direct + (num_tiles - p.n_direct) * p.k_splits;
+#define LB200_TC_NO_MORE(u) ((u) < 0)
+#endif
+  auto decode_unit = [&](int u, int &t, int &sp, int &kb_lo, int &kb_hi) {
+    if (u < p.n_direct) {
+      t = u; sp = -1; kb_lo = 0; kb_hi = num_kb;
+    } else {
+      const int v = u - p.n_direct;
+      const int i = v / p.k_splits;
+      t = p.n_direct + i;
+      sp = v - i * p.k_splits;
+      kb_lo = min(num_kb, sp * p.kb_per_split);
+      kb_hi = min(num_kb, kb_lo + p.kb_per_split);
+    }
+  };
+  constexpr int SCHED_CONSUMERS = 1 + TC_EPI_WARPS;
+  auto next_unit = [&](uint32_t &ph) -> int {
+    ptx::mbar_wait(sched_full, ph);
+    const int u = *reinterpret_cast<volatile int *>(sched_unit);
+    ptx::mbar_arrive(sched_empty);
+    ph ^= 1u;
+    return u;
+  };
+
+  if (threadIdx.x == 0) {
+    ptx::prefetch_tensormap(&mapA0);
+    ptx::prefetch_tensormap(&mapB0);
+    if constexpr (NPASS == 3) {
+      ptx::prefetch_tensormap(&mapA1);
+      ptx::prefetch_tensormap(&mapB1);
+    }
+#if LB200_TC_PREP
+    ptx::prefetch_tensormap(&srcA);
+    ptx::prefetch_tensormap(&srcB);
+#endif
+  }
+  if (threadIdx.x == 32) {
+    for (int i = 0; i < STAGES; ++i) {
+      ptx::mbar_init(&full_bar[i], 1);
+      ptx::mbar_init(&empty_bar[i], TC_EPI_WARPS);
+    }
+    ptx::mbar_init(sched_full, 1);
+    ptx::mbar_init(sched_empty, SCHED_CONSUMERS);
+#if LB200_TC_PREP
+    ptx::mbar_init(prep_bar, TC_EPI_THREADS);
+#endif
+    ptx::fence_barrier_init();
+  }
+  __syncthreads();
+  ptx::griddep_wait();
+
+  if (warp_idx < 4) {
+    ptx::setmaxnreg_dec<TC_REGS_CTRL>();
+    if (warp_idx == 3 && lane == 0) {
+      uint32_t phase = 0;
+      int next_static = sched_id;
+      for (;;) {
+        ptx::mbar_wait(sched_empty, phase ^ 1);
+        int u;
+        if (p.sched) {
+          u = static_cast<int>(atomicAdd(p.sched, 1u));
+        } else {
+          u = next_static;
+          next_static += sched_stride;
+        }
+        if (u >= num_units) u = -1;
+#if LB200_TC_PREP
+        else u = p.unit_seq[u];
+#endif
+        *reinterpret_cast<volatile int *>(sched_unit) = u;
+        ptx::mbar_arrive(sched_full);
+        phase ^= 1u;
+        if (LB200_TC_NO_MORE(u)) {
+          if (p.sched) {
+            __threadfence();
+            if (atomicAdd(p.sched + 1, 1u) == static_cast<unsigned int>(sched_stride - 1)) {
+              p.sched[0] = 0u;
+              p.sched[1] = 0u;
+              __threadfence();
+            }
+          }
+          break;
+        }
+      }
+    } else if (warp_idx == 0 && lane == 0) {
+      int stage = 0;
+      uint32_t phase = 0, sched_phase = 0;
+      constexpr int MN_ATOM = TC_ROW_BYTES / ESZ;
+      constexpr int MN_BOX_BYTES = BLOCK_K * TC_ROW_BYTES;
+      auto load_a = [&](uint8_t *dst, const CUtensorMap *m, uint64_t *bar, int m0, int k0, int z) {
+        if constexpr (!A_MN) {
+          if constexpr (BATCHED) ptx::tma_load_3d(dst, m, bar, k0, m0, z);
+          else ptx::tma_load_2d(dst, m, bar, k0, m0);
+        } else {
+#pragma unroll
+          for (int c = 0; c < TC_BLOCK_M / MN_ATOM; ++c) {
+            if constexpr (BATCHED) ptx::tma_load_3d(dst + c * MN_BOX_BYTES, m, bar, m0 + c * MN_ATOM, k0, z);
+            else ptx::tma_load_2d(dst + c * MN_BOX_BYTES, m, bar, m0 + c * MN_ATOM, k0);
+          }
+        }
+      };
+      auto load_b = [&](uint8_t *dst, const CUtensorMap *m, uint64_t *bar, int n0, int k0, int z) {
+        if constexpr (!B_MN) {
+          if constexpr (BATCHED) ptx::tma_load_3d(dst, m, bar, k0, n0, z);
+          else ptx::tma_load_2d(dst, m, bar, k0, n0);
+        } else {
+#pragma unroll
+          for (int c = 0; c < TC_BLOCK_N / MN_ATOM; ++c) {
+            if constexpr (BATCHED) ptx::tma_load_3d(dst + c * MN_BOX_BYTES, m, bar, n0 + c * MN_ATOM, k0, z);
+            else ptx::tma_load_2d(dst + c * MN_BOX_BYTES, m, bar, n0 + c * MN_ATOM, k0);
+          }
+        }
+      };
+      for (;;) {
+        const int u = next_unit(sched_phase);
+        if (LB200_TC_NO_MORE(u)) break;
+#if LB200_TC_PREP
+        {
+          if (u < 0) {
+            const int i = -2 - u;
+            const bool is_a = i < p.num_m_blocks;
+            const CUtensorMap *src = is_a ? &srcA : &srcB;
+            const int panel = (is_a ? i : i - p.num_m_blocks) * TC_PREP_BOX;
+            const bool per_col = is_a ? p.prep_a.mn_major : p.prep_b.mn_major;
+            const int64_t along = per_col ? (is_a ? p.prep_a.R : p.prep_b.R) : (is_a ? p.prep_a.Cc : p.prep_b.Cc);
+            const int chunks = static_cast<int>((along + TC_PREP_BOX - 1) / TC_PREP_BOX);
+            for (int q = 0; q < 2 * chunks; ++q) {
+              const int ch = (q < chunks ? q : q - chunks) * TC_PREP_BOX;
+              ptx::mbar_wait(&empty_bar[stage], phase ^ 1);
+              ptx::mbar_arrive_expect_tx(&full_bar[stage], Cfg::STAGE_BYTES);
+              for (int j = 0; j < TC_PREP_STRIPS; ++j)
+                ptx::tma_load_2d(smem + stage * Cfg::STAGE_BYTES + j * TC_PREP_BOX * TC_PREP_STRIP * 4, src, &full_bar[stage],
+                                 (per_col ? panel : ch) + j * TC_PREP_STRIP, per_col ? ch : panel);
+              if (++stage == STAGES) { stage = 0; phase ^= 1; }
+            }
+            continue;
+          }
+        }
+#endif
+        int t, sp, mb, nb, kb_lo, kb_hi;
+        decode_unit(u, t, sp, kb_lo, kb_hi);
+        int za = 0, zb = 0;
+        if constexpr (BATCHED) {
+          const int bz = t / tiles_pp;
+          t -= bz * tiles_pp;
+          za = bz % p.period_a;
+          zb = bz % p.period_b;
+        }
+        tile_coords(t, p.num_m_blocks, p.num_n_blocks, p.raster_g, mb, nb);
+        const int m0 = mb * TC_BLOCK_M;
+        const int n0 = nb * TC_BLOCK_N;
+#if LB200_TC_PREP
+        ptx::wait_flag(p.ready + mb, p.ready_seq);
+        ptx::wait_flag(p.ready + p.num_m_blocks + nb, p.ready_seq);
+        ptx::fence_proxy_async_global();
+#endif
+        for (int kb = kb_lo; kb < kb_hi; ++kb) {
+          ptx::mbar_wait(&empty_bar[stage], phase ^ 1);
+          ptx::mbar_arrive_expect_tx(&full_bar[stage], Cfg::STAGE_BYTES);
+          uint8_t *sa = smem + stage * Cfg::STAGE_BYTES;
+          uint8_t *sb = sa + Cfg::A_STAGE_BYTES;
+          const int k0 = kb * BLOCK_K;
+          load_a(sa, &mapA0, &full_bar[stage], m0, k0, za);
+          if constexpr (NPASS == 3) load_a(sa + TC_A_TILE_BYTES, &mapA1, &full_bar[stage], m0, k0, za);
+          load_b(sb, &mapB0, &full_bar[stage], n0, k0, zb);
+          if constexpr (NPASS == 3) load_b(sb + Cfg::B_TILE_BYTES, &mapB1, &full_bar[stage], n0, k0, zb);
+          if (++stage == STAGES) { stage = 0; phase ^= 1; }
+        }
+      }
+    }
+  } else {
+    ptx::setmaxnreg_inc<TC_REGS_EPI>();
+    const int g = (warp_idx - 4) >> 2;
+    const int wq = warp_idx & 3;
+    const int lr = lane >> 2;
+    const int lc = 2 * (lane & 3);
+    constexpr int MMA_K = 32 / ESZ;
+    constexpr int K_STEPS = BLOCK_K / MMA_K;
+    constexpr int MN_BOX_BYTES = BLOCK_K * TC_ROW_BYTES;
+    constexpr uint32_t A_WG_BYTES = 64 * TC_ROW_BYTES;
+    int stage = 0;
+    uint32_t phase = 0, sched_phase = 0;
+    const bool vec_ok_c = (p.csC == 1) && ((p.rsC & 1) == 0) && ((reinterpret_cast<uintptr_t>(p.C) & (2 * sizeof(OutT) - 1)) == 0) &&
+                          (!BATCHED || (p.bsC & 1) == 0);
+    float acc[TC_ACC_REGS];
+#pragma unroll
+    for (int j = 0; j < TC_ACC_REGS; ++j) acc[j] = 0.0f;
+#if LB200_TC_PREP
+    uint32_t prep_phase = 0;
+#endif
+    for (;;) {
+      int u = 0;
+      if (lane == 0) u = next_unit(sched_phase);
+      u = __shfl_sync(0xffffffffu, u, 0);
+      if (LB200_TC_NO_MORE(u)) break;
+#if LB200_TC_PREP
+      if (u < 0) {
+        prep_panel<STAGES, Cfg::STAGE_BYTES>(p, -2 - u, smem, full_bar, empty_bar, prep_bar, prep_red, stage, phase, prep_phase);
+        continue;
+      }
+#endif
+      int t, sp, mb, nb, kb_lo, kb_hi;
+      decode_unit(u, t, sp, kb_lo, kb_hi);
+      int bz = 0, za = 0, zb = 0;
+      if constexpr (BATCHED) {
+        bz = t / tiles_pp;
+        za = bz % p.period_a;
+        zb = bz % p.period_b;
+        int tl = t - bz * tiles_pp;
+        tile_coords(tl, p.num_m_blocks, p.num_n_blocks, p.raster_g, mb, nb);
+      } else {
+        tile_coords(t, p.num_m_blocks, p.num_n_blocks, p.raster_g, mb, nb);
+      }
+      const int num_blocks = (kb_hi - kb_lo + p.kb_per_block - 1) / p.kb_per_block;
+      const int r_tile = 64 * g + 16 * wq + lr;
+      const int64_t row0 = static_cast<int64_t>(mb) * TC_BLOCK_M + r_tile;
+      const int64_t col0 = static_cast<int64_t>(nb) * TC_BLOCK_N + lc;
+      const bool split_unit = sp >= 0;
+      uint32_t amax_row[2] = {0u, 0u}, amax_col[2 * TC_BLOCK_N / 8];
+#if LB200_TC_PREP
+      ptx::wait_flag(p.ready + mb, p.ready_seq);
+      ptx::wait_flag(p.ready + p.num_m_blocks + nb, p.ready_seq);
+#endif
+      if constexpr (SCALED) {
+#pragma unroll
+        for (int h = 0; h < 2; ++h)
+          if (row0 + 8 * h < p.M) amax_row[h] = p.amax_a[(BATCHED ? za * p.amax_bs_a : 0) + row0 + 8 * h];
+#pragma unroll
+        for (int j = 0; j < 2 * TC_BLOCK_N / 8; ++j) {
+          const int64_t c = col0 + 8 * (j >> 1) + (j & 1);
+          amax_col[j] = c < p.N ? p.amax_b[(BATCHED ? zb * p.amax_bs_b : 0) + c] : 0u;
+        }
+      }
+      float run[TC_ACC_REGS];
+#pragma unroll
+      for (int j = 0; j < TC_ACC_REGS; ++j) run[j] = 0.0f;
+      for (int blk = 0; blk < num_blocks; ++blk) {
+        const int kb0 = kb_lo + blk * p.kb_per_block;
+        const int kb1 = min(kb_hi, kb0 + p.kb_per_block);
+        int prev_stage = -1;
+        for (int kb = kb0; kb < kb1; ++kb) {
+          ptx::mbar_wait(&full_bar[stage], phase);
+          ptx::wgmma_fence();
+          const uint32_t a_addr = ptx::smem_u32(smem + stage * Cfg::STAGE_BYTES) + g * A_WG_BYTES;
+          const uint32_t b_addr = ptx::smem_u32(smem + stage * Cfg::STAGE_BYTES + Cfg::A_STAGE_BYTES);
+#pragma unroll
+          for (int pass = 0; pass < NPASS; ++pass) {
+            const uint32_t a_tile = a_addr + ((NPASS == 3 && pass == 1) ? TC_A_TILE_BYTES : 0);
+            const uint32_t b_tile = b_addr + ((NPASS == 3 && pass == 0) ? Cfg::B_TILE_BYTES : 0);
+#pragma unroll
+            for (int k = 0; k < K_STEPS; ++k) {
+              const uint64_t ad = A_MN ? ptx::make_smem_desc(a_tile + k * MMA_K * TC_ROW_BYTES, MN_BOX_BYTES, 1024, ptx::kLayoutSw128)
+                                       : ptx::make_smem_desc(a_tile + k * 32, 0, 1024, ptx::kLayoutSw128);
+              const uint64_t bd = B_MN ? ptx::make_smem_desc(b_tile + k * MMA_K * TC_ROW_BYTES, MN_BOX_BYTES, 1024, ptx::kLayoutSw128)
+                                       : ptx::make_smem_desc(b_tile + k * 32, 0, 1024, ptx::kLayoutSw128);
+              const uint32_t accum = (kb == kb0 && pass == 0 && k == 0) ? 0u : 1u;
+              if constexpr (ESZ == 4) ptx::wgmma_m64n128k8_tf32(acc, ad, bd, accum);
+              else if constexpr (FMT16 == ptx::kFmtF16) ptx::wgmma_m64n128k16_f16<A_MN ? 1 : 0, B_MN ? 1 : 0>(acc, ad, bd, accum);
+              else ptx::wgmma_m64n128k16_bf16<A_MN ? 1 : 0, B_MN ? 1 : 0>(acc, ad, bd, accum);
+            }
+          }
+          ptx::wgmma_commit();
+          ptx::wgmma_wait<1>();
+          if (prev_stage >= 0 && lane == 0) ptx::mbar_arrive(&empty_bar[prev_stage]);
+          prev_stage = stage;
+          if (++stage == STAGES) { stage = 0; phase ^= 1; }
+        }
+        ptx::wgmma_wait<0>();
+        ptx::wgmma_hold(acc);
+        if (prev_stage >= 0 && lane == 0) ptx::mbar_arrive(&empty_bar[prev_stage]);
+#pragma unroll
+        for (int j = 0; j < TC_ACC_REGS; ++j) run[j] = __fadd_rn(run[j], acc[j]);
+      }
+      float alpha_r[2] = {split_unit ? 1.0f : p.alpha, split_unit ? 1.0f : p.alpha};
+      if constexpr (SCALED) {
+#pragma unroll
+        for (int h = 0; h < 2; ++h) alpha_r[h] *= f16x2_unscale(amax_row[h]);
+      }
+      const float beta_u = split_unit ? 0.0f : p.beta;
+      const bool has_epi = !split_unit && ((p.epi.bias != nullptr) || (p.epi.act != 0));
+      float *ws_base = nullptr;
+      if (split_unit) {
+        const int64_t plane = static_cast<int64_t>(sp) * (num_tiles - p.n_direct) + (t - p.n_direct);
+        ws_base = p.split_ws + (plane * TC_BLOCK_M + r_tile) * TC_BLOCK_N + lc;
+      }
+#pragma unroll
+      for (int h = 0; h < 2; ++h) {
+        const int64_t row = row0 + 8 * h;
+        if (!split_unit && row >= p.M) continue;
+        const float row_bias =
+            (has_epi && p.epi.bias && p.epi.bias_per_row) ? p.epi.bias[(BATCHED ? za * p.bias_bs : 0) + row] : 0.0f;
+        OutT *crow = split_unit ? nullptr : reinterpret_cast<OutT *>(p.C) + (BATCHED ? bz * p.bsC : 0) + row * p.rsC;
+#pragma unroll
+        for (int i = 0; i < TC_BLOCK_N / 8; ++i) {
+          float v[2];
+#pragma unroll
+          for (int e = 0; e < 2; ++e) {
+            v[e] = alpha_r[h] * run[4 * i + 2 * h + e];
+            if constexpr (SCALED) v[e] *= f16x2_unscale(amax_col[2 * i + e]);
+          }
+          if (split_unit) {
+            *reinterpret_cast<float2 *>(ws_base + 8 * h * TC_BLOCK_N + 8 * i) = make_float2(v[0], v[1]);
+            continue;
+          }
+          const int64_t c = col0 + 8 * i;
+          if (c >= p.N) continue;
+          const bool pair_ok = vec_ok_c && c + 1 < p.N;
+          OutT *dst = crow + c * p.csC;
+          if (beta_u != 0.0f) {
+            float o[2] = {0.0f, 0.0f};
+            if constexpr (sizeof(OutT) == 4) {
+              if (pair_ok) { const float2 w = *reinterpret_cast<const float2 *>(dst); o[0] = w.x; o[1] = w.y; }
+              else { o[0] = dst[0]; if (c + 1 < p.N) o[1] = dst[p.csC]; }
+            } else {
+              o[0] = bf16_bits_to_f32(dst[0]);
+              if (c + 1 < p.N) o[1] = bf16_bits_to_f32(dst[pair_ok ? 1 : p.csC]);
+            }
+#pragma unroll
+            for (int e = 0; e < 2; ++e) v[e] = fmaf(beta_u, o[e], v[e]);
+          }
+          if (has_epi) {
+#pragma unroll
+            for (int e = 0; e < 2; ++e) {
+              const float bv = (p.epi.bias && !p.epi.bias_per_row) ? (c + e < p.N ? p.epi.bias[c + e] : 0.0f) : row_bias;
+              v[e] = epi_act(v[e] + bv, p.epi.act);
+            }
+          }
+          if constexpr (sizeof(OutT) == 4) {
+            if (pair_ok) *reinterpret_cast<float2 *>(dst) = make_float2(v[0], v[1]);
+            else { dst[0] = v[0]; if (c + 1 < p.N) dst[p.csC] = v[1]; }
+          } else {
+            if (pair_ok) *reinterpret_cast<uint32_t *>(dst) = f32_to_bf16_bits(v[0]) | (static_cast<uint32_t>(f32_to_bf16_bits(v[1])) << 16);
+            else { dst[0] = f32_to_bf16_bits(v[0]); if (c + 1 < p.N) dst[p.csC] = f32_to_bf16_bits(v[1]); }
+          }
+        }
+      }
+    }
+  }
+
+  __syncthreads();
+}
+#undef LB200_TC_NO_MORE
diff --git a/laser_b200/csrc/ptx.cuh b/laser_b200/csrc/ptx.cuh
--- a/laser_b200/csrc/ptx.cuh
+++ b/laser_b200/csrc/ptx.cuh
@@ -6,6 +6,29 @@
 
 #ifdef LB200_HOST_EMULATION
 #include "ptx_emu.h"
+#include <sched.h>
+
+#include <atomic>
+#include <chrono>
+
+namespace lb200 {
+namespace ptx {
+inline uint32_t ld_acquire_gpu(const uint32_t *p) { return __atomic_load_n(p, __ATOMIC_ACQUIRE); }
+inline void st_release_gpu(uint32_t *p, uint32_t v) { __atomic_store_n(p, v, __ATOMIC_RELEASE); }
+inline void fence_proxy_async_global() {}
+inline void wait_flag(const uint32_t *p, uint32_t want) {
+  const auto t0 = std::chrono::steady_clock::now();
+  while (ld_acquire_gpu(p) != want) {
+    if (std::chrono::steady_clock::now() - t0 > std::chrono::seconds(mbar_wait_limit_s())) {
+      std::fprintf(stderr, "emu: deadlock: thread %u of CTA %u waits for flag %p to read %u (it reads %u)\n", emu::t_idx.x,
+                   emu::b_idx.x, static_cast<const void *>(p), want, ld_acquire_gpu(p));
+      std::abort();
+    }
+    sched_yield();
+  }
+}
+}
+}
 #else
 
 #define LB200_DYN_SMEM(T, name) extern __shared__ T name[]
@@ -103,6 +126,24 @@
 }
 __device__ __forceinline__ void prefetch_l2(const void *p) {
   asm volatile("prefetch.global.L2 [%0];" ::"l"(p));
+}
+__device__ __forceinline__ uint32_t ld_acquire_gpu(const uint32_t *p) {
+  uint32_t v;
+  asm volatile("ld.acquire.gpu.global.u32 %0, [%1];" : "=r"(v) : "l"(p) : "memory");
+  return v;
+}
+__device__ __forceinline__ void st_release_gpu(uint32_t *p, uint32_t v) {
+  asm volatile("st.release.gpu.global.u32 [%0], %1;" ::"l"(p), "r"(v) : "memory");
+}
+__device__ __forceinline__ void fence_proxy_async_global() {
+  asm volatile("fence.proxy.async.global;" ::: "memory");
+}
+__device__ __forceinline__ void wait_flag(const uint32_t *p, uint32_t want) {
+  uint32_t ns = 32;
+  while (ld_acquire_gpu(p) != want) {
+    __nanosleep(ns);
+    if (ns < 1024) ns <<= 1;
+  }
 }
 template <int N>
 __device__ __forceinline__ void setmaxnreg_inc() {
diff --git a/laser_b200/csrc/split.cuh b/laser_b200/csrc/split.cuh
--- a/laser_b200/csrc/split.cuh
+++ b/laser_b200/csrc/split.cuh
@@ -163,10 +163,6 @@
   }
 }
 
-__device__ __forceinline__ uint32_t finite_abs_bits(float f) {
-  const uint32_t a = __float_as_uint(f) & 0x7fffffffu;
-  return a < 0x7f800000u ? a : 0u;
-}
 constexpr int ABSMAX_ROW_CHUNK = 1024;
 constexpr int ABSMAX_COL_ROWS = 64;
 template <bool PER_COL, bool HAS_OP = false, bool BATCHED = false, bool CONCAT = false>
@@ -246,14 +242,6 @@
   }
 }
 
-__device__ __forceinline__ void store_f16x2_vec4(float4 v, float sx, float sy, float sz, float sw, uint16_t *hrow, uint16_t *lrow,
-                                                 int64_t c) {
-  uint2 h, l;
-  f16x2_pieces2(__fmul_rn(v.x, sx), __fmul_rn(v.y, sy), h.x, l.x);
-  f16x2_pieces2(__fmul_rn(v.z, sz), __fmul_rn(v.w, sw), h.y, l.y);
-  *reinterpret_cast<uint2 *>(hrow + c) = h;
-  *reinterpret_cast<uint2 *>(lrow + c) = l;
-}
 __device__ __forceinline__ void store_f16x2_vec(float4 v, float s, uint16_t *hrow, uint16_t *lrow, int64_t c) {
   store_f16x2_vec4(v, s, s, s, s, hrow, lrow, c);
 }
diff --git a/laser_b200/csrc/tc_launch.h b/laser_b200/csrc/tc_launch.h
--- a/laser_b200/csrc/tc_launch.h
+++ b/laser_b200/csrc/tc_launch.h
@@ -13,6 +13,8 @@
   bool a_mn = false, b_mn = false;
   bool batched = false;
   bool pdl = false;
+  bool prep = false;
+  CUtensorMap sa{}, sb{};
   int dev = 0, sm_count = 0;
   cudaStream_t stream = nullptr;
 };
diff --git a/laser_b200/csrc/tc_launch_impl.cuh b/laser_b200/csrc/tc_launch_impl.cuh
--- a/laser_b200/csrc/tc_launch_impl.cuh
+++ b/laser_b200/csrc/tc_launch_impl.cuh
@@ -11,14 +11,15 @@
 
 namespace lb200 {
 
-template <int ESZ, uint32_t FMT16, int NPASS, typename OutT, bool SCALED, bool A_MN, bool B_MN, bool BATCHED>
+template <int ESZ, uint32_t FMT16, int NPASS, typename OutT, bool SCALED, bool A_MN, bool B_MN, bool BATCHED, bool PREP = false>
 int launch_tc_one(const TcLaunch &l) {
   using Cfg = TcCfg<NPASS>;
+  constexpr int SMEM_BYTES = Cfg::SMEM_BYTES + (PREP ? TC_EPI_WARPS * TC_PREP_BOX * 4 : 0);
   const int64_t units_total = tc_units(l.p);
   cudaLaunchConfig_t cfg{};
   cfg.gridDim = dim3(static_cast<int>(units_total < l.sm_count ? units_total : l.sm_count));
   cfg.blockDim = dim3(TC_THREADS);
-  cfg.dynamicSmemBytes = Cfg::SMEM_BYTES;
+  cfg.dynamicSmemBytes = SMEM_BYTES;
   cfg.stream = l.stream;
   cudaLaunchAttribute attr[1];
   if (l.pdl) {
@@ -27,14 +28,18 @@
     cfg.attrs = attr;
     cfg.numAttrs = 1;
   }
-  auto kfn = gemm_tc_kernel<ESZ, FMT16, NPASS, A_MN, B_MN, OutT, SCALED, BATCHED>;
+  auto kfn = [] {
+    if constexpr (PREP) return gemm_tc_prep_kernel<A_MN, B_MN>;
+    else return gemm_tc_kernel<ESZ, FMT16, NPASS, A_MN, B_MN, OutT, SCALED, BATCHED>;
+  }();
   static std::atomic<uint32_t> attr_set{0};
   if (!(attr_set.load(std::memory_order_acquire) & (1u << l.dev))) {
-    const cudaError_t e = cudaFuncSetAttribute(kfn, cudaFuncAttributeMaxDynamicSharedMemorySize, Cfg::SMEM_BYTES);
+    const cudaError_t e = cudaFuncSetAttribute(kfn, cudaFuncAttributeMaxDynamicSharedMemorySize, SMEM_BYTES);
     if (e != cudaSuccess) return static_cast<int>(e);
     attr_set.fetch_or(1u << l.dev, std::memory_order_release);
   }
-  return static_cast<int>(LB200_LAUNCH_EX(&cfg, kfn, l.a0, l.a1, l.b0, l.b1, l.p));
+  if constexpr (PREP) return static_cast<int>(LB200_LAUNCH_EX(&cfg, kfn, l.a0, l.a1, l.b0, l.b1, l.p, l.sa, l.sb));
+  else return static_cast<int>(LB200_LAUNCH_EX(&cfg, kfn, l.a0, l.a1, l.b0, l.b1, l.p));
 }
 
 template <int ESZ, uint32_t FMT16, int NPASS, typename OutT, bool SCALED>
@@ -44,17 +49,19 @@
     if (l.batched) return launch_tc_one<ESZ, FMT16, NPASS, OutT, SCALED, false, false, true>(l);
     return launch_tc_one<ESZ, FMT16, NPASS, OutT, SCALED, false, false, false>(l);
   }
-#define LB200_MAJORS(BATCHED)                                                                                  \
-  do {                                                                                                         \
-    if (!l.a_mn && !l.b_mn) return launch_tc_one<ESZ, FMT16, NPASS, OutT, SCALED, false, false, BATCHED>(l);   \
-    if (!l.a_mn && l.b_mn) return launch_tc_one<ESZ, FMT16, NPASS, OutT, SCALED, false, true, BATCHED>(l);     \
-    if (l.a_mn && !l.b_mn) return launch_tc_one<ESZ, FMT16, NPASS, OutT, SCALED, true, false, BATCHED>(l);     \
-    return launch_tc_one<ESZ, FMT16, NPASS, OutT, SCALED, true, true, BATCHED>(l);                             \
+#define LB200_MAJORS(...)                                                                                          \
+  do {                                                                                                             \
+    if (!l.a_mn && !l.b_mn) return launch_tc_one<ESZ, FMT16, NPASS, OutT, SCALED, false, false, __VA_ARGS__>(l);   \
+    if (!l.a_mn && l.b_mn) return launch_tc_one<ESZ, FMT16, NPASS, OutT, SCALED, false, true, __VA_ARGS__>(l);     \
+    if (l.a_mn && !l.b_mn) return launch_tc_one<ESZ, FMT16, NPASS, OutT, SCALED, true, false, __VA_ARGS__>(l);     \
+    return launch_tc_one<ESZ, FMT16, NPASS, OutT, SCALED, true, true, __VA_ARGS__>(l);                             \
   } while (0)
   if constexpr (ESZ == 2) {
     if constexpr (SCALED) {
       if (l.batched) LB200_MAJORS(true);
+      if (l.prep) LB200_MAJORS(false, true);
     }
+    if (l.prep) return static_cast<int>(cudaErrorNotSupported);
     if (l.batched) return static_cast<int>(cudaErrorNotSupported);
     LB200_MAJORS(false);
   }
diff --git a/laser_b200/csrc/tc_params.h b/laser_b200/csrc/tc_params.h
--- a/laser_b200/csrc/tc_params.h
+++ b/laser_b200/csrc/tc_params.h
@@ -1,6 +1,8 @@
 #pragma once
 
 #include <stdint.h>
+
+#include <vector>
 
 #if defined(__CUDACC__) || defined(LB200_HOST_EMULATION)
 #define LB200_HD __host__ __device__
@@ -59,7 +61,22 @@
   int64_t bsC = 0;
   int64_t amax_bs_a = 0, amax_bs_b = 0;
   int64_t bias_bs = 0;
+  const int *unit_seq = nullptr;
+  uint32_t *ready = nullptr;
+  uint32_t ready_seq = 0;
+  int n_prep = 0;
+  struct PrepOperand {
+    uint16_t *h = nullptr, *l = nullptr;
+    int64_t ld = 0;
+    uint32_t *words = nullptr;
+    int64_t R = 0, Cc = 0;
+    int mn_major = 0;
+  } prep_a, prep_b;
 };
+constexpr int TC_PREP_BOX = 128;
+constexpr int TC_PREP_STRIP = TC_ROW_BYTES / 4;
+constexpr int TC_PREP_STRIPS = TC_PREP_BOX / TC_PREP_STRIP;
+
 
 LB200_HD inline void tile_coords(int t, int num_m, int num_n, int G, int &mb, int &nb) {
   const int per_group = G * num_n;
@@ -124,4 +141,24 @@
   return (tiles - p.n_direct) * p.k_splits * TC_BLOCK_M * TC_BLOCK_N;
 }
 
+inline void tc_prep_sequence(const TcParams &p, int lead, int *seq) {
+  const int units = static_cast<int>(tc_units(p));
+  const int panels = p.num_m_blocks + p.num_n_blocks;
+  std::vector<int> first(panels, -1), order;
+  order.reserve(panels);
+  for (int u = 0; u < units && static_cast<int>(order.size()) < panels; ++u) {
+    const int t = u < p.n_direct ? u : p.n_direct + (u - p.n_direct) / p.k_splits;
+    int mb, nb;
+    tile_coords(t, p.num_m_blocks, p.num_n_blocks, p.raster_g, mb, nb);
+    for (const int i : {mb, p.num_m_blocks + nb})
+      if (first[i] < 0) { first[i] = u; order.push_back(i); }
+  }
+  int k = 0;
+  size_t j = 0;
+  for (int u = 0; u < units; ++u) {
+    while (j < order.size() && first[order[j]] <= u + lead) seq[k++] = -2 - order[j++];
+    seq[k++] = u;
+  }
 }
+
+}
```
